# neross666/xRayTracer

Measured on AMD Instinct MI355X. Metric: Msamples/s (whole node) + wall-clock at 800×600×1024spp, 1/2/4/8 MI355X, higher is better.
Workload: dtype f32

## Files before the change

include/xrt.h:

```cpp
#ifndef XRT_H
#define XRT_H

#include <stddef.h>
#include <stdint.h>

#ifdef __cplusplus
extern "C" {
#endif

#define XRT_ABI_VERSION 14

enum {
    XRT_OK = 0,
    XRT_ERR_INVALID = -1,
    XRT_ERR_HIP = -2,
    XRT_ERR_STATE = -3,
    XRT_ERR_OOM = -4,
    XRT_ERR_UNSUPPORTED = -5,
    XRT_ERR_IO = -6
};

enum { XRT_OBJ_MESH = 0, XRT_OBJ_SPHERE = 1, XRT_OBJ_BOX = 2 };
enum { XRT_LIGHT_QUAD = 0, XRT_LIGHT_TRIANGLE = 1, XRT_LIGHT_SPHERE = 2, XRT_LIGHT_SPHERE_AREA = 3 };
enum { XRT_MAT_NONE = 0, XRT_MAT_LAMBERT = 1, XRT_MAT_METAL = 2, XRT_MAT_GLASS = 3 };

typedef struct {
    int32_t kind;
    int32_t first;
    int32_t count;
    int32_t material;
    float albedo[3];
    int32_t light;
    int32_t medium;
} xrt_object;

typedef struct {
    int32_t kind;
    float v0[3];
    float v1[3];
    float v2[3];
    float center[3];
    float radius;
    float Le[3];
} xrt_light;

typedef struct {
    uint32_t n_objects;
    const xrt_object* objects;
    uint32_t n_tris;
    const float* tri_v;
    const float* tri_n;
    uint32_t n_spheres;
    const float* spheres;
    uint32_t n_boxes;
    const float* boxes;
    uint32_t n_lights;
    const xrt_light* lights;
} xrt_scene_desc;

enum { XRT_DLIGHT_POINT = 0, XRT_DLIGHT_DISTANT = 1 };
typedef struct {
    int32_t kind;
    float pos[3];
    float dir[3];
    float color[3];
    float intensity;
} xrt_delta_light;
#define XRT_MAX_DELTA_LIGHTS 8

enum {
    XRT_MEDIUM_HETEROGENEOUS = 0,
    XRT_MEDIUM_HOMOGENEOUS_MIS = 1,
    XRT_MEDIUM_HOMOGENEOUS_ACHROMATIC = 2,
    XRT_MEDIUM_HOMOGENEOUS_NOMIS = 3
};
typedef struct {
    uint32_t nx, ny, nz;
    const float* density;
    float origin[3];
    float voxel_size;
    float bbox_min[3];
    float bbox_max[3];
    float max_density;
    float g;
    float absorption[3];
    float scattering[3];
    float density_multiplier;
    int32_t kind;
} xrt_medium_desc;

enum {
    XRT_INTEGRATOR_GI = 0,
    XRT_INTEGRATOR_DIRECT = 1,
    XRT_INTEGRATOR_VPT = 2,
    XRT_INTEGRATOR_INDIRECT = 3,
    XRT_INTEGRATOR_NORMAL = 4,
    XRT_INTEGRATOR_VPT_NEE = 5,
    XRT_INTEGRATOR_WHITTED = 6
};
#define XRT_WHITTED_MAX_DEPTH 4
enum {
    XRT_FLAG_TIMING = 1u,
    XRT_FLAG_WAVEFRONT = 2u,
    XRT_FLAG_NO_MERGED = 4u,
    XRT_FLAG_NO_GROUP = 8u,
    XRT_FLAG_DEEP_SINGLE = 32u,
    XRT_FLAG_DEEP_QUAD = 64u,
    XRT_FLAG_NO_PIXEL = 128u,
    XRT_FLAG_NO_SPEC = 256u,
    XRT_FLAG_WHITTED_BVH = 512u,
    XRT_FLAG_NO_OVERLAP = 1024u,
    XRT_FLAG_INTERLEAVE = 2048u,
    XRT_FLAG_NO_INTERLEAVE = 4096u,
    XRT_FLAG_VAR_FUSED = 8192u,
    XRT_FLAG_ACCUMULATE = 16u
};

typedef struct {
    int32_t integrator;
    uint32_t max_depth;
    uint32_t width, height;
    uint32_t spp;
    uint32_t shard_index;
    uint32_t shard_count;
    uint32_t flags;
    uint32_t slots_per_wave;
    uint32_t visits_per_launch;
} xrt_render_params;

enum {
    XRT_K_SEED = 0, XRT_K_TRACE = 1, XRT_K_SHADE = 2, XRT_K_FINISH = 3, XRT_K_STEP = 4, XRT_K_REFILL = 5,
    XRT_K_DEEP = 6, XRT_K_COUNT = 7
};

enum {
    XRT_SCHED_WAVEFRONT = 0, XRT_SCHED_STEP = 1, XRT_SCHED_STEP_TRI = 2, XRT_SCHED_STEP_MERGED = 3,
    XRT_SCHED_STEP_BVH = 4, XRT_SCHED_PIXEL = 5,
    XRT_SCHED_WHITTED = 6,
    XRT_SCHED_WHITTED_BVH = 7,
    XRT_SCHED_AOV = 8
};

typedef struct {
    double wall_ms;
    double kernel_ms[XRT_K_COUNT];
    uint64_t launches[XRT_K_COUNT];
    uint64_t samples;
    uint64_t segments;
    uint64_t shadow_rays;
    uint64_t draws;
    uint64_t rejected;
    uint64_t iterations;
    uint64_t path_slots;
    uint64_t schedule;
    uint64_t stalled;
    uint32_t slots_per_wave;
    uint32_t group_lanes;
    uint32_t partitions;
    uint32_t visits_per_launch;
    uint64_t rng_twists;
    uint64_t layout_launches[5];
    uint64_t pix_windows;
    uint64_t pix_stride4;
    uint64_t pix_frustum;
    uint64_t pix_frustum_overflow;
    uint64_t pix_shadow_list;
    uint64_t pix_shadow_overflow;
    uint64_t pix_flushes;
    uint64_t spec_launches;
    uint64_t whit_rays;
    uint64_t whit_depth_cut;
    uint64_t whit_refract;
    uint64_t whit_tir;
} xrt_stats;

typedef struct xrt_ctx xrt_ctx;

int  xrt_abi_version(void);
int  xrt_create(int device, xrt_ctx** out);
int  xrt_create_multi(const int* devices, int n_devices, xrt_ctx** out);
int  xrt_device_count(const xrt_ctx* ctx);
void xrt_destroy(xrt_ctx* ctx);
const char* xrt_last_error(const xrt_ctx* ctx);

int  xrt_upload_scene(xrt_ctx* ctx, const xrt_scene_desc* scene);
int  xrt_set_camera(xrt_ctx* ctx, const float c2w[16], float scale, float aspect);
int  xrt_set_medium(xrt_ctx* ctx, const xrt_medium_desc* medium);
int  xrt_set_delta_lights(xrt_ctx* ctx, const xrt_delta_light* lights, uint32_t n);
#define XRT_BRICK 8
typedef struct {
    uint32_t nbx, nby, nbz;
    const int32_t* table;
    uint32_t n_bricks;
    const float* bricks;
} xrt_brick_grid;
int  xrt_set_medium_bricks(xrt_ctx* ctx, const xrt_medium_desc* medium, const xrt_brick_grid* grid);

int  xrt_render(xrt_ctx* ctx, const xrt_render_params* p, float* rgb_out, xrt_stats* st);
int  xrt_render_device(xrt_ctx* ctx, const xrt_render_params* p, float* d_rgb_out, xrt_stats* st);
int  xrt_render_device_after(xrt_ctx* ctx, const xrt_render_params* p, float* d_rgb_out, void* hip_stream,
                             xrt_stats* st);

int  xrt_render_var(xrt_ctx* ctx, const xrt_render_params* p, float* rgb_out, float* variance_out, xrt_stats* st);
int  xrt_render_var_device(xrt_ctx* ctx, const xrt_render_params* p, float* d_rgb_out, float* d_variance_out,
                           void* hip_stream, xrt_stats* st);

typedef struct { float* albedo; float* normal; float* depth; float* alpha; int32_t* object; } xrt_aov_buffers;
int  xrt_render_aov(xrt_ctx* ctx, const xrt_render_params* p, const xrt_aov_buffers* host_out, xrt_stats* st);
int  xrt_render_aov_device(xrt_ctx* ctx, const xrt_render_params* p, const xrt_aov_buffers* device_out,
                           void* hip_stream, xrt_stats* st);

#define XRT_DENOISE_MAX_ITERATIONS 6
#define XRT_DENOISE_TILED_ITERATIONS 2
enum {
    XRT_DENOISE_TIMING = 1u,
    XRT_DENOISE_NO_TILE = 2u
};
typedef struct {
    uint32_t width, height, iterations;
    float sigma_color, sigma_normal, sigma_depth, sigma_albedo;
    uint32_t flags;
} xrt_denoise_params;
typedef struct {
    double wall_ms;
    double kernel_ms;
    uint32_t launches;
    uint32_t tiled_iterations, direct_iterations;
    uint32_t reserved;
} xrt_denoise_stats;
int  xrt_denoise(xrt_ctx* ctx, const xrt_denoise_params* p, const float* color, const xrt_aov_buffers* guides,
                 float* out, xrt_denoise_stats* st);
int  xrt_denoise_device(xrt_ctx* ctx, const xrt_denoise_params* p, const float* d_color,
                        const xrt_aov_buffers* d_guides, float* d_out, void* hip_stream, xrt_denoise_stats* st);

#define XRT_DENOISE_VAR_MAX_RADIUS 3
#define XRT_DENOISE_VAR_TILED_ITERATIONS 2
typedef struct {
    uint32_t width, height, iterations;
    float sigma_luminance, sigma_normal, sigma_depth, sigma_albedo;
    uint32_t variance_radius;
    uint32_t flags;
} xrt_denoise_var_params;
int  xrt_denoise_var(xrt_ctx* ctx, const xrt_denoise_var_params* p, const float* color, const float* variance,
                     const xrt_aov_buffers* guides, float* out, float* out_variance, xrt_denoise_stats* st);
int  xrt_denoise_var_device(xrt_ctx* ctx, const xrt_denoise_var_params* p, const float* d_color,
                            const float* d_variance, const xrt_aov_buffers* d_guides, float* d_out,
                            float* d_out_variance, void* hip_stream, xrt_denoise_stats* st);

typedef struct {
    int32_t hit;
    int32_t object;
    int32_t primitive;
    float t;
    float t1;
    float position[3], ng[3], ns[3], dpdu[3], dpdv[3];
    float barycentric[2];
} xrt_hit;
enum { XRT_QUERY_INTERSECT = 0, XRT_QUERY_OCCLUDED = 1 };
int  xrt_query(xrt_ctx* ctx, uint32_t n, const float* rays, const float* tmax, int32_t mode, xrt_hit* out);

int  xrt_tonemap(xrt_ctx* ctx, const float* d_rgb, uint32_t n_pixels, float gamma, uint8_t* rgb8_out);

typedef struct xrt_hscene xrt_hscene;
xrt_hscene* xrt_hscene_create(void);
void xrt_hscene_destroy(xrt_hscene* s);
const char* xrt_hscene_last_error(const xrt_hscene* s);
int xrt_hscene_load_obj(xrt_hscene* s, const char* path);
int xrt_hscene_add_mesh(xrt_hscene* s, const char* name, const float* tri_v, const float* tri_n,
                        uint32_t n_tris, const float albedo[3]);
int xrt_hscene_add_sphere_mesh(xrt_hscene* s, const char* name, const float center[3], float radius,
                               int n_theta, int n_phi, const float albedo[3]);
int xrt_hscene_add_sphere(xrt_hscene* s, const char* name, const float center[3], float radius,
                          const float albedo[3]);
int xrt_hscene_add_quad_light(xrt_hscene* s, const char* name, const float v0[3], const float v1[3],
                              const float v2[3], const float Le[3]);
int xrt_hscene_add_triangle_light(xrt_hscene* s, const char* name, const float v0[3],
                                  const float v1[3], const float v2[3], const float Le[3]);
int xrt_hscene_add_sphere_light(xrt_hscene* s, const char* name, const float center[3], float radius,
                                const float Le[3]);
int xrt_hscene_add_sphere_light_area(xrt_hscene* s, const char* name, const float center[3], float radius,
                                     const float Le[3]);
int xrt_hscene_add_medium_box(xrt_hscene* s, const char* name, const float pmin[3], const float pmax[3]);
int xrt_hscene_add_point_light(xrt_hscene* s, const char* name, const float l2w[16], const float color[3],
                               float intensity);
int xrt_hscene_add_distant_light(xrt_hscene* s, const char* name, const float l2w[16], const float color[3],
                                 float intensity);
int xrt_hscene_delta_lights(xrt_hscene* s, const xrt_delta_light** out, uint32_t* n);
int xrt_hscene_set_material(xrt_hscene* s, const char* object_name, int32_t material);
int xrt_hscene_flatten(xrt_hscene* s, xrt_scene_desc* out);
const char* xrt_hscene_object_name(const xrt_hscene* s, uint32_t i);

float xrt_pinhole_scale(float fov_deg);

int xrt_test_rng(xrt_ctx* ctx, const uint32_t* seeds, uint32_t n_seeds, uint32_t skip, uint32_t n,
                 float* out);
int xrt_test_trig(xrt_ctx* ctx, const float* x, uint32_t n, float* out);
int xrt_test_trig_draw_domain(xrt_ctx* ctx, uint32_t first_bits, uint32_t count, float* out_sin,
                              float* out_cos, float* out_r);
int xrt_test_logexp(xrt_ctx* ctx, const float* x, uint32_t n, float* out);
int xrt_test_powf(xrt_ctx* ctx, const float* x, uint32_t n, float y, float* out);
int xrt_test_fastdiv(xrt_ctx* ctx, uint32_t mode, float c, float rc, uint64_t* n_bad, uint32_t* first_bad16);
int xrt_test_whitted_math(xrt_ctx* ctx, const float* in, uint32_t n, float* out);
int xrt_test_camlist(xrt_ctx* ctx, const xrt_render_params* p, uint32_t* out);
int xrt_test_slot_map(xrt_ctx* ctx, const xrt_render_params* p, uint32_t* out);

#ifdef __cplusplus
}
#endif
#endif
```

xraytracer_amd/abi.py:

```python
from __future__ import annotations

import ctypes as C
import os

import numpy as np

HERE = os.path.dirname(os.path.abspath(__file__))
LIB_PATH = os.path.join(HERE, "libxrt_hip.so")
if os.environ.get("XRT_LIB"):
    _v = os.path.join(HERE, "variants", os.environ["XRT_LIB"])
    LIB_PATH = _v if os.path.exists(_v) else os.path.join(HERE, os.environ["XRT_LIB"])

XRT_ABI_VERSION = 14
XRT_OK = 0
XRT_OBJ_MESH, XRT_OBJ_SPHERE, XRT_OBJ_BOX = 0, 1, 2
XRT_LIGHT_QUAD, XRT_LIGHT_TRIANGLE, XRT_LIGHT_SPHERE, XRT_LIGHT_SPHERE_AREA = 0, 1, 2, 3
XRT_MAT_NONE, XRT_MAT_LAMBERT, XRT_MAT_METAL, XRT_MAT_GLASS = 0, 1, 2, 3
MATERIALS = {"none": XRT_MAT_NONE, "lambert": XRT_MAT_LAMBERT, "metal": XRT_MAT_METAL, "glass": XRT_MAT_GLASS}
XRT_DLIGHT_POINT, XRT_DLIGHT_DISTANT = 0, 1
XRT_MAX_DELTA_LIGHTS = 8
XRT_INTEGRATOR_GI, XRT_INTEGRATOR_DIRECT, XRT_INTEGRATOR_VPT = 0, 1, 2
XRT_INTEGRATOR_INDIRECT, XRT_INTEGRATOR_NORMAL, XRT_INTEGRATOR_VPT_NEE = 3, 4, 5
XRT_INTEGRATOR_WHITTED = 6
XRT_WHITTED_MAX_DEPTH = 4
XRT_ERR_INVALID, XRT_ERR_UNSUPPORTED = -1, -5
XRT_ERR_STATE = -3
XRT_MEDIUM_HETEROGENEOUS, XRT_MEDIUM_HOMOGENEOUS_MIS, XRT_MEDIUM_HOMOGENEOUS_ACHROMATIC, XRT_MEDIUM_HOMOGENEOUS_NOMIS = 0, 1, 2, 3
XRT_FLAG_TIMING, XRT_FLAG_WAVEFRONT, XRT_FLAG_NO_MERGED, XRT_FLAG_NO_GROUP, XRT_FLAG_ACCUMULATE = 1, 2, 4, 8, 16
XRT_FLAG_DEEP_SINGLE, XRT_FLAG_DEEP_QUAD, XRT_FLAG_NO_PIXEL = 32, 64, 128
XRT_FLAG_NO_SPEC = 256
XRT_FLAG_WHITTED_BVH = 512
XRT_FLAG_NO_OVERLAP = 1024
XRT_FLAG_INTERLEAVE, XRT_FLAG_NO_INTERLEAVE = 2048, 4096
XRT_FLAG_VAR_FUSED = 8192
XRT_SCHED_WAVEFRONT, XRT_SCHED_STEP, XRT_SCHED_STEP_TRI, XRT_SCHED_STEP_MERGED, XRT_SCHED_STEP_BVH = 0, 1, 2, 3, 4
XRT_SCHED_PIXEL, XRT_SCHED_WHITTED, XRT_SCHED_WHITTED_BVH = 5, 6, 7
XRT_SCHED_AOV = 8
AOV_PLANES = ("albedo", "normal", "depth", "alpha", "object")
XRT_DENOISE_MAX_ITERATIONS = 6
XRT_DENOISE_TILED_ITERATIONS = 2
XRT_DENOISE_TIMING, XRT_DENOISE_NO_TILE = 1, 2
XRT_DENOISE_VAR_MAX_RADIUS = 3
XRT_DENOISE_VAR_TILED_ITERATIONS = 2
DENOISE_PLANES = ("albedo", "normal", "depth", "object")
SCHEDULE_NAMES = ("wavefront", "step", "step_tri", "step_merged", "step_bvh", "pixel", "whitted", "whitted_bvh",
                  "aov")
XRT_K_SEED, XRT_K_TRACE, XRT_K_SHADE, XRT_K_FINISH, XRT_K_STEP, XRT_K_REFILL, XRT_K_DEEP, XRT_K_COUNT = \
    0, 1, 2, 3, 4, 5, 6, 7
LAYOUTS = (64, 32, 16, 8, 4)
KERNEL_NAMES = ("seed", "trace", "shade", "finish", "step", "refill", "trace_deep4")

INTEGRATORS = {"gi": XRT_INTEGRATOR_GI, "direct": XRT_INTEGRATOR_DIRECT, "vpt": XRT_INTEGRATOR_VPT,
               "indirect": XRT_INTEGRATOR_INDIRECT, "normal": XRT_INTEGRATOR_NORMAL, "vpt_nee": XRT_INTEGRATOR_VPT_NEE,
               "whitted": XRT_INTEGRATOR_WHITTED}

f32p = C.POINTER(C.c_float)
u32p = C.POINTER(C.c_uint32)


class XrtObject(C.Structure):
    _fields_ = [("kind", C.c_int32), ("first", C.c_int32), ("count", C.c_int32),
                ("material", C.c_int32), ("albedo", C.c_float * 3), ("light", C.c_int32),
                ("medium", C.c_int32)]


class XrtLight(C.Structure):
    _fields_ = [("kind", C.c_int32), ("v0", C.c_float * 3), ("v1", C.c_float * 3),
                ("v2", C.c_float * 3), ("center", C.c_float * 3), ("radius", C.c_float),
                ("Le", C.c_float * 3)]


class XrtDeltaLight(C.Structure):
    _fields_ = [("kind", C.c_int32), ("pos", C.c_float * 3), ("dir", C.c_float * 3), ("color", C.c_float * 3),
                ("intensity", C.c_float)]


class XrtSceneDesc(C.Structure):
    _fields_ = [("n_objects", C.c_uint32), ("objects", C.POINTER(XrtObject)),
                ("n_tris", C.c_uint32), ("tri_v", f32p), ("tri_n", f32p),
                ("n_spheres", C.c_uint32), ("spheres", f32p),
                ("n_boxes", C.c_uint32), ("boxes", f32p),
                ("n_lights", C.c_uint32), ("lights", C.POINTER(XrtLight))]


class XrtMediumDesc(C.Structure):
    _fields_ = [("nx", C.c_uint32), ("ny", C.c_uint32), ("nz", C.c_uint32), ("density", f32p),
                ("origin", C.c_float * 3), ("voxel_size", C.c_float),
                ("bbox_min", C.c_float * 3), ("bbox_max", C.c_float * 3),
                ("max_density", C.c_float), ("g", C.c_float),
                ("absorption", C.c_float * 3), ("scattering", C.c_float * 3),
                ("density_multiplier", C.c_float), ("kind", C.c_int32)]


class XrtBrickGrid(C.Structure):
    _fields_ = [("nbx", C.c_uint32), ("nby", C.c_uint32), ("nbz", C.c_uint32), ("table", C.POINTER(C.c_int32)),
                ("n_bricks", C.c_uint32), ("bricks", f32p)]


XRT_BRICK = 8


class XrtRenderParams(C.Structure):
    _fields_ = [("integrator", C.c_int32), ("max_depth", C.c_uint32), ("width", C.c_uint32),
                ("height", C.c_uint32), ("spp", C.c_uint32), ("shard_index", C.c_uint32),
                ("shard_count", C.c_uint32), ("flags", C.c_uint32), ("slots_per_wave", C.c_uint32),
                ("visits_per_launch", C.c_uint32)]


class XrtStats(C.Structure):
    _fields_ = [("wall_ms", C.c_double), ("kernel_ms", C.c_double * XRT_K_COUNT),
                ("launches", C.c_uint64 * XRT_K_COUNT), ("samples", C.c_uint64),
                ("segments", C.c_uint64), ("shadow_rays", C.c_uint64), ("draws", C.c_uint64),
                ("rejected", C.c_uint64), ("iterations", C.c_uint64), ("path_slots", C.c_uint64),
                ("schedule", C.c_uint64), ("stalled", C.c_uint64), ("slots_per_wave", C.c_uint32),
                ("group_lanes", C.c_uint32), ("partitions", C.c_uint32), ("visits_per_launch", C.c_uint32),
                ("rng_twists", C.c_uint64), ("layout_launches", C.c_uint64 * 5),
                ("pix_windows", C.c_uint64), ("pix_stride4", C.c_uint64), ("pix_frustum", C.c_uint64),
                ("pix_frustum_overflow", C.c_uint64), ("pix_shadow_list", C.c_uint64),
                ("pix_shadow_overflow", C.c_uint64), ("pix_flushes", C.c_uint64), ("spec_launches", C.c_uint64),
                ("whit_rays", C.c_uint64), ("whit_depth_cut", C.c_uint64), ("whit_refract", C.c_uint64),
                ("whit_tir", C.c_uint64)]

    def as_dict(self):
        d = {k: getattr(self, k) for k, _ in self._fields_ if k not in ("kernel_ms", "launches", "layout_launches")}
        d["layout_launches"] = dict(zip(LAYOUTS, (int(x) for x in self.layout_launches)))
        d["kernel_ms"] = {n: self.kernel_ms[i] for i, n in enumerate(KERNEL_NAMES)}
        d["launches"] = {n: int(self.launches[i]) for i, n in enumerate(KERNEL_NAMES)}
        return d


class XrtAovBuffers(C.Structure):
    _fields_ = [("albedo", C.c_void_p), ("normal", C.c_void_p), ("depth", C.c_void_p), ("alpha", C.c_void_p),
                ("object", C.c_void_p)]


class XrtDenoiseParams(C.Structure):
    _fields_ = [("width", C.c_uint32), ("height", C.c_uint32), ("iterations", C.c_uint32),
                ("sigma_color", C.c_float), ("sigma_normal", C.c_float), ("sigma_depth", C.c_float),
                ("sigma_albedo", C.c_float), ("flags", C.c_uint32)]


class XrtDenoiseVarParams(C.Structure):
    _fields_ = [("width", C.c_uint32), ("height", C.c_uint32), ("iterations", C.c_uint32),
                ("sigma_luminance", C.c_float), ("sigma_normal", C.c_float), ("sigma_depth", C.c_float),
                ("sigma_albedo", C.c_float), ("variance_radius", C.c_uint32), ("flags", C.c_uint32)]


class XrtDenoiseStats(C.Structure):
    _fields_ = [("wall_ms", C.c_double), ("kernel_ms", C.c_double), ("launches", C.c_uint32),
                ("tiled_iterations", C.c_uint32), ("direct_iterations", C.c_uint32), ("reserved", C.c_uint32)]


class XrtHit(C.Structure):
    _fields_ = [("hit", C.c_int32), ("object", C.c_int32), ("primitive", C.c_int32), ("t", C.c_float),
                ("t1", C.c_float), ("position", C.c_float * 3), ("ng", C.c_float * 3), ("ns", C.c_float * 3),
                ("dpdu", C.c_float * 3), ("dpdv", C.c_float * 3), ("barycentric", C.c_float * 2)]


XRT_QUERY_INTERSECT, XRT_QUERY_OCCLUDED = 0, 1


SIGNATURES = {
    "xrt_abi_version": (C.c_int, []),
    "xrt_create": (C.c_int, [C.c_int, C.POINTER(C.c_void_p)]),
    "xrt_create_multi": (C.c_int, [C.POINTER(C.c_int), C.c_int, C.POINTER(C.c_void_p)]),
    "xrt_device_count": (C.c_int, [C.c_void_p]),
    "xrt_destroy": (None, [C.c_void_p]),
    "xrt_last_error": (C.c_char_p, [C.c_void_p]),
    "xrt_upload_scene": (C.c_int, [C.c_void_p, C.POINTER(XrtSceneDesc)]),
    "xrt_set_camera": (C.c_int, [C.c_void_p, f32p, C.c_float, C.c_float]),
    "xrt_set_medium": (C.c_int, [C.c_void_p, C.POINTER(XrtMediumDesc)]),
    "xrt_set_delta_lights": (C.c_int, [C.c_void_p, C.POINTER(XrtDeltaLight), C.c_uint32]),
    "xrt_set_medium_bricks": (C.c_int, [C.c_void_p, C.POINTER(XrtMediumDesc), C.POINTER(XrtBrickGrid)]),
    "xrt_render": (C.c_int, [C.c_void_p, C.POINTER(XrtRenderParams), f32p, C.POINTER(XrtStats)]),
    "xrt_render_device": (C.c_int, [C.c_void_p, C.POINTER(XrtRenderParams), C.c_void_p, C.POINTER(XrtStats)]),
    "xrt_render_device_after": (C.c_int, [C.c_void_p, C.POINTER(XrtRenderParams), C.c_void_p, C.c_void_p,
                                          C.POINTER(XrtStats)]),
    "xrt_render_var": (C.c_int, [C.c_void_p, C.POINTER(XrtRenderParams), f32p, f32p, C.POINTER(XrtStats)]),
    "xrt_render_var_device": (C.c_int, [C.c_void_p, C.POINTER(XrtRenderParams), C.c_void_p, C.c_void_p, C.c_void_p,
                                        C.POINTER(XrtStats)]),
    "xrt_render_aov": (C.c_int, [C.c_void_p, C.POINTER(XrtRenderParams), C.POINTER(XrtAovBuffers), C.POINTER(XrtStats)]),
    "xrt_render_aov_device": (C.c_int, [C.c_void_p, C.POINTER(XrtRenderParams), C.POINTER(XrtAovBuffers), C.c_void_p,
                                        C.POINTER(XrtStats)]),
    "xrt_denoise": (C.c_int, [C.c_void_p, C.POINTER(XrtDenoiseParams), C.c_void_p, C.POINTER(XrtAovBuffers), C.c_void_p,
                              C.POINTER(XrtDenoiseStats)]),
    "xrt_denoise_device": (C.c_int, [C.c_void_p, C.POINTER(XrtDenoiseParams), C.c_void_p, C.POINTER(XrtAovBuffers),
                                     C.c_void_p, C.c_void_p, C.POINTER(XrtDenoiseStats)]),
    "xrt_denoise_var": (C.c_int, [C.c_void_p, C.POINTER(XrtDenoiseVarParams), C.c_void_p, C.c_void_p,
                                  C.POINTER(XrtAovBuffers), C.c_void_p, C.c_void_p, C.POINTER(XrtDenoiseStats)]),
    "xrt_denoise_var_device": (C.c_int, [C.c_void_p, C.POINTER(XrtDenoiseVarParams), C.c_void_p, C.c_void_p,
                                         C.POINTER(XrtAovBuffers), C.c_void_p, C.c_void_p, C.c_void_p,
                                         C.POINTER(XrtDenoiseStats)]),
    "xrt_hscene_create": (C.c_void_p, []),
    "xrt_hscene_destroy": (None, [C.c_void_p]),
    "xrt_hscene_last_error": (C.c_char_p, [C.c_void_p]),
    "xrt_hscene_load_obj": (C.c_int, [C.c_void_p, C.c_char_p]),
    "xrt_hscene_add_mesh": (C.c_int, [C.c_void_p, C.c_char_p, f32p, f32p, C.c_uint32, f32p]),
    "xrt_hscene_add_sphere_mesh": (C.c_int, [C.c_void_p, C.c_char_p, f32p, C.c_float, C.c_int, C.c_int, f32p]),
    "xrt_hscene_add_sphere": (C.c_int, [C.c_void_p, C.c_char_p, f32p, C.c_float, f32p]),
    "xrt_hscene_add_quad_light": (C.c_int, [C.c_void_p, C.c_char_p, f32p, f32p, f32p, f32p]),
    "xrt_hscene_add_triangle_light": (C.c_int, [C.c_void_p, C.c_char_p, f32p, f32p, f32p, f32p]),
    "xrt_hscene_add_sphere_light": (C.c_int, [C.c_void_p, C.c_char_p, f32p, C.c_float, f32p]),
    "xrt_hscene_add_sphere_light_area": (C.c_int, [C.c_void_p, C.c_char_p, f32p, C.c_float, f32p]),
    "xrt_hscene_add_medium_box": (C.c_int, [C.c_void_p, C.c_char_p, f32p, f32p]),
    "xrt_hscene_add_point_light": (C.c_int, [C.c_void_p, C.c_char_p, f32p, f32p, C.c_float]),
    "xrt_hscene_add_distant_light": (C.c_int, [C.c_void_p, C.c_char_p, f32p, f32p, C.c_float]),
    "xrt_hscene_delta_lights": (C.c_int, [C.c_void_p, C.POINTER(C.POINTER(XrtDeltaLight)), u32p]),
    "xrt_hscene_set_material": (C.c_int, [C.c_void_p, C.c_char_p, C.c_int32]),
    "xrt_hscene_flatten": (C.c_int, [C.c_void_p, C.POINTER(XrtSceneDesc)]),
    "xrt_hscene_object_name": (C.c_char_p, [C.c_void_p, C.c_uint32]),
    "xrt_pinhole_scale": (C.c_float, [C.c_float]),
    "xrt_test_rng": (C.c_int, [C.c_void_p, u32p, C.c_uint32, C.c_uint32, C.c_uint32, f32p]),
    "xrt_test_trig": (C.c_int, [C.c_void_p, f32p, C.c_uint32, f32p]),
    "xrt_test_trig_draw_domain": (C.c_int, [C.c_void_p, C.c_uint32, C.c_uint32, f32p, f32p, f32p]),
    "xrt_test_logexp": (C.c_int, [C.c_void_p, f32p, C.c_uint32, f32p]),
    "xrt_test_powf": (C.c_int, [C.c_void_p, f32p, C.c_uint32, C.c_float, f32p]),
    "xrt_query": (C.c_int, [C.c_void_p, C.c_uint32, f32p, f32p, C.c_int32, C.POINTER(XrtHit)]),
    "xrt_tonemap": (C.c_int, [C.c_void_p, C.c_void_p, C.c_uint32, C.c_float, C.POINTER(C.c_uint8)]),
    "xrt_test_whitted_math": (C.c_int, [C.c_void_p, f32p, C.c_uint32, f32p]),
    "xrt_test_fastdiv": (C.c_int, [C.c_void_p, C.c_uint32, C.c_float, C.c_float, C.POINTER(C.c_uint64), u32p]),
    "xrt_test_camlist": (C.c_int, [C.c_void_p, C.POINTER(XrtRenderParams), u32p]),
    "xrt_test_slot_map": (C.c_int, [C.c_void_p, C.POINTER(XrtRenderParams), u32p]),
}

_lib = None


def lib():
    global _lib
    if _lib is None:
        if not os.path.exists(LIB_PATH):
            raise ImportError(f"{LIB_PATH} is missing: run __graft_entry__.build() "
                              "(the HIP path has no CPU fallback)")
        try:
            import torch
        except Exception as e:
            if not isinstance(e, ImportError):
                import warnings
                warnings.warn(f"torch failed to import ({e!r}); loading libxrt_hip without it")
        l = C.CDLL(LIB_PATH)
        for name, (res, args) in SIGNATURES.items():
            fn = getattr(l, name)
            fn.restype = res
            fn.argtypes = args
        _lib = l
    return _lib


def fptr(a: np.ndarray):
    assert a.dtype == np.float32 and a.flags.c_contiguous
    return a.ctypes.data_as(f32p)


def u32ptr(a: np.ndarray):
    assert a.dtype == np.uint32 and a.flags.c_contiguous
    return a.ctypes.data_as(u32p)


def f3(v):
    return np.ascontiguousarray(np.asarray(v, dtype=np.float32).reshape(3))


class XrtError(RuntimeError):
    pass
```

xraytracer_amd/csrc/api_context.cpp:

```cpp
#include "ctx.h"

namespace xrt {

int set_err(xrt_ctx* c, int code, const std::string& msg) {
    if (c) c->err = msg;
    return code;
}

int hip_err(xrt_ctx* c, hipError_t e, const char* what) {
    return set_err(c, XRT_ERR_HIP, std::string(what) + ": " + hipGetErrorString(e));
}

void free_buf(DevBuf& b) {
    if (b.p) (void)hipFree(b.p);
    b.p = nullptr;
    b.bytes = 0;
}

int ensure(xrt_ctx* c, DevBuf& b, size_t bytes) {
    if (b.bytes >= bytes && b.p) return XRT_OK;
    free_buf(b);
    if (bytes == 0) return XRT_OK;
    hipError_t e = hipMalloc(&b.p, bytes);
    if (e != hipSuccess) {
        b.p = nullptr;
        return set_err(c, XRT_ERR_OOM, std::string("hipMalloc(") + std::to_string(bytes) + "): " + hipGetErrorString(e));
    }
    b.bytes = bytes;
    return XRT_OK;
}

int upload(xrt_ctx* c, DevBuf& b, const void* src, size_t bytes) {
    int rc = ensure(c, b, std::max<size_t>(bytes, 16));
    if (rc) return rc;
    if (bytes) HIPCHK(c, hipMemcpy(b.p, src, bytes, hipMemcpyHostToDevice));
    return XRT_OK;
}

int order_after(xrt_ctx* c, int wait, hipStream_t wait_stream, bool host_blocks) {
    HIPCHK(c, hipSetDevice(c->device));
    if (wait == 1) {
        HIPCHK(c, hipDeviceSynchronize());
    } else if (wait == 2) {
        HIPCHK(c, hipEventRecord(c->wait_ev, wait_stream));
        if (host_blocks)
            HIPCHK(c, hipEventSynchronize(c->wait_ev));
        else
            HIPCHK(c, hipStreamWaitEvent(c->stream, c->wait_ev, 0));
    }
    return XRT_OK;
}

}

using namespace xrt;

extern "C" {

int xrt_abi_version(void) { return XRT_ABI_VERSION; }

int xrt_create(int device, xrt_ctx** out) {
    if (!out) return XRT_ERR_INVALID;
    *out = nullptr;
    int n = 0;
    if (hipGetDeviceCount(&n) != hipSuccess || n == 0) return XRT_ERR_HIP;
    if (device < 0 || device >= n) return XRT_ERR_INVALID;
    xrt_ctx* c = new xrt_ctx();
    c->device = device;
    if (hipSetDevice(device) != hipSuccess || hipStreamCreateWithFlags(&c->stream, hipStreamNonBlocking) != hipSuccess ||
        hipHostMalloc((void**)&c->h_poll, 8 * kMaxStepGroups * kMaxParts * sizeof(uint32_t), hipHostMallocDefault) !=
            hipSuccess ||
        hipEventCreateWithFlags(&c->wait_ev, hipEventDisableTiming) != hipSuccess) {
        xrt_destroy(c);
        return XRT_ERR_HIP;
    }
    for (auto& slot : c->poll_ev)
        for (hipEvent_t& e : slot)
            if (hipEventCreateWithFlags(&e, hipEventDisableTiming) != hipSuccess) {
                xrt_destroy(c);
                return XRT_ERR_HIP;
            }
    int lds = 0;
    if (hipDeviceGetAttribute(&lds, hipDeviceAttributeMaxSharedMemoryPerBlock, device) != hipSuccess || lds <= 0) {
        xrt_destroy(c);
        return XRT_ERR_HIP;
    }
    c->base.lds_max = (uint32_t)lds;
    *out = c;
    return XRT_OK;
}

void xrt_destroy(xrt_ctx* c) {
    if (!c) return;
    for (xrt_ctx* s : c->subs) xrt_destroy(s);
    c->subs.clear();
    (void)hipSetDevice(c->device);
    if (c->stream) (void)hipStreamSynchronize(c->stream);
    for (hipStream_t s : c->group_stream)
        if (s) (void)hipStreamSynchronize(s), (void)hipStreamDestroy(s);
    if (c->fork_ev) (void)hipEventDestroy(c->fork_ev);
    for (hipEvent_t e : c->join_ev)
        if (e) (void)hipEventDestroy(e);
    DevBuf* all[] = {&c->tri, &c->tri_ng, &c->tri_nrm, &c->sph, &c->sph_obj, &c->box, &c->objs, &c->lights,
                     &c->segs, &c->density, &c->obj_box, &c->obj_plane, &c->bvh_node, &c->bvh_tri, &c->snode, &c->ssph, &c->sbk, &c->sblk, &c->ray_o, &c->ray_d, &c->thr, &c->rad, &c->thr_prev, &c->hit,
                     &c->hit2, &c->hit3, &c->sh_o, &c->sh_d, &c->sh_c, &c->med, &c->med2, &c->nee, &c->state,
                     &c->sample_k, &c->depth, &c->occ, &c->rng_c, &c->rng_g, &c->ring, &c->c_seg, &c->c_shadow,
                     &c->c_rej, &c->c_stall, &c->lists, &c->counts, &c->stats, &c->fb, &c->scratch, &c->kparams};
    for (DevBuf* b : all) free_buf(*b);
    free_buf(c->stri), free_buf(c->sbox), free_buf(c->splane), free_buf(c->bvh4), free_buf(c->deep);
    free_buf(c->q_rays), free_buf(c->q_tmax), free_buf(c->q_out);
    free_buf(c->brick_table), free_buf(c->brick_data), free_buf(c->corners), free_buf(c->camlist);
    free_buf(c->dlights), free_buf(c->obj_albedo), free_buf(c->aov), free_buf(c->denoise);
    free_buf(c->mom), free_buf(c->var);
    for (hipEvent_t e : c->events) (void)hipEventDestroy(e);
    for (auto& slot : c->poll_ev)
        for (hipEvent_t e : slot)
            if (e) (void)hipEventDestroy(e);
    if (c->wait_ev) (void)hipEventDestroy(c->wait_ev);
    if (c->h_poll) (void)hipHostFree(c->h_poll);
    if (c->stream) (void)hipStreamDestroy(c->stream);
    delete c;
}

const char* xrt_last_error(const xrt_ctx* c) { return c ? c->err.c_str() : "no context (xrt_create failed: no HIP device?)"; }

}
```

xraytracer_amd/csrc/api_render.cpp:

```cpp
#include <sched.h>

#include <chrono>
#include <cmath>
#include <cstdio>
#include <cstdlib>
#include <cstring>
#include <mutex>
#include <unordered_map>

#include "ctx.h"

namespace xrt {

int setup_deep(xrt_ctx* c, KParams& P) {
    P.deep = nullptr, P.deep_count = nullptr, P.deep_cap = 0;
    if (!P.two_level) return XRT_OK;
    P.deep_cap = P.part_cap * (1u + (uint32_t)std::max(1, P.n_lights));
    const size_t words = (size_t)P.n_part * P.deep_cap + 3 * kMaxParts;
    const int rc = ensure(c, c->deep, words * 4);
    if (rc) return rc;
    P.deep = as<uint32_t>(c->deep);
    P.deep_count = P.deep + (size_t)P.n_part * P.deep_cap;
    return XRT_OK;
}
// ... 23 lines not shown
        for (uint32_t m = (uint32_t)t; m < (1u << 23) && ok; m += (uint32_t)nthreads) {
            const uint32_t xb = 0x3f800000u | m;
            float x;
            std::memcpy(&x, &xb, 4);
            const float q = x * rc;
            ok = std::fma(std::fma(-d, q, x), rc, q) == x / d;
        }
        part[t] = ok;
    });
    bool ok = true;
    for (char p : part) ok &= p != 0;
    cache[key] = ok;
    return ok;
}

int check_render(xrt_ctx* c, const xrt_render_params* p) {
    if (!c || !p) return XRT_ERR_INVALID;
    if (!c->has_scene || !c->has_camera) return set_err(c, XRT_ERR_STATE, "upload a scene and set a camera first");
    if (p->width == 0 || p->height == 0 || p->shard_count == 0 || p->shard_index >= p->shard_count)
        return set_err(c, XRT_ERR_INVALID, "bad image size or shard");
    if (p->integrator < XRT_INTEGRATOR_GI || p->integrator > XRT_INTEGRATOR_WHITTED)
        return set_err(c, XRT_ERR_INVALID, "unknown integrator");
    if (p->integrator != XRT_INTEGRATOR_WHITTED && c->has_mirror)
        return set_err(c, XRT_ERR_UNSUPPORTED,
                       "the scene holds a metal or glass object: only WhittedIntegrator knows those materials");
    if (p->integrator == XRT_INTEGRATOR_WHITTED && c->has_glass && p->max_depth > XRT_WHITTED_MAX_DEPTH)
        return set_err(c, XRT_ERR_UNSUPPORTED, "WhittedIntegrator over a scene with glass: max_depth above " +
                                                   std::to_string(XRT_WHITTED_MAX_DEPTH) + " (XRT_WHITTED_MAX_DEPTH)");
    const bool volumetric = p->integrator == XRT_INTEGRATOR_VPT || p->integrator == XRT_INTEGRATOR_VPT_NEE;
    if (volumetric && !c->has_medium)
        return set_err(c, XRT_ERR_STATE, "VolumePathTracing needs xrt_set_medium first");
    if (p->integrator == XRT_INTEGRATOR_VPT_NEE && c->base.n_lights == 0)
        return set_err(c, XRT_ERR_STATE, "VolumePathTracingNEE needs an area light");
    if (p->slots_per_wave != 0 && p->slots_per_wave != 4 && p->slots_per_wave != 8 && p->slots_per_wave != 16 &&
        p->slots_per_wave != 32 && p->slots_per_wave != 64)
        return set_err(c, XRT_ERR_INVALID, "slots_per_wave must be 0, 4, 8, 16, 32 or 64");
    if (p->visits_per_launch > 128) return set_err(c, XRT_ERR_INVALID, "visits_per_launch must be 0..128");
    return XRT_OK;
}

int check_render_var(xrt_ctx* c, const xrt_render_params* p) {
    if (p->spp < 2) return set_err(c, XRT_ERR_INVALID, "xrt_render_var: spp must be at least 2 (one sample has no variance)");
    if (p->flags & XRT_FLAG_ACCUMULATE)
        return set_err(c, XRT_ERR_UNSUPPORTED,
                       "xrt_render_var: XRT_FLAG_ACCUMULATE (the moments of the earlier calls' samples are unknown)");
    return XRT_OK;
}

int render_empty_shard(xrt_ctx* c, const xrt_render_params* p, float* d_out, float* h_out, float* d_var, xrt_stats* st,
                       std::chrono::steady_clock::time_point t_start) {
    const size_t npix = (size_t)p->width * p->height;
    int rc;
    if (!d_out && (rc = ensure(c, c->fb, npix * 3 * sizeof(float)))) return rc;
    float* fb0 = d_out ? d_out : as<float>(c->fb);
    if (p->flags & XRT_FLAG_ACCUMULATE) return XRT_OK;
    HIPCHK(c, hipMemsetAsync(fb0, 0, npix * 3 * sizeof(float), c->stream));
    if (d_var) HIPCHK(c, hipMemsetAsync(d_var, 0, npix * sizeof(float), c->stream));
    HIPCHK(c, hipStreamSynchronize(c->stream));
    if (h_out) HIPCHK(c, hipMemcpy(h_out, fb0, npix * 3 * sizeof(float), hipMemcpyDeviceToHost));
    if (st) {
        std::memset(st, 0, sizeof(*st));
        st->wall_ms = std::chrono::duration<double, std::milli>(std::chrono::steady_clock::now() - t_start).count();
    }
    return XRT_OK;
}

void bind_slots(xrt_ctx* c, KParams& P) {
    P.ray_o = as<f4>(c->ray_o), P.ray_d = as<f4>(c->ray_d), P.thr = as<f4>(c->thr), P.rad = as<f4>(c->rad);
    P.thr_prev = as<f4>(c->thr_prev), P.hit = as<f4>(c->hit), P.hit2 = as<f4>(c->hit2), P.hit3 = as<f4>(c->hit3);
    P.sh_o = as<f4>(c->sh_o), P.sh_d = as<f4>(c->sh_d), P.sh_c = as<f4>(c->sh_c);
    P.med = as<f4>(c->med), P.med2 = as<f4>(c->med2), P.nee = as<f4>(c->nee);
    P.state = as<uint32_t>(c->state), P.sample_k = as<uint32_t>(c->sample_k), P.depth = as<uint32_t>(c->depth);
    P.occ = as<uint32_t>(c->occ), P.rng_c = as<uint32_t>(c->rng_c), P.rng_g = as<uint32_t>(c->rng_g);
    P.ring = as<uint32_t>(c->ring);
    P.c_seg = as<uint32_t>(c->c_seg), P.c_shadow = as<uint32_t>(c->c_shadow), P.c_rej = as<uint32_t>(c->c_rej);
    P.c_stall = as<uint32_t>(c->c_stall);
    P.stats = as<unsigned long long>(c->stats);
}

}

int grow_slots(xrt_ctx* c, size_t n) {
    int rc;
    if (n > c->cap_slots) {
        const size_t L = kMaxLights;
        if ((rc = ensure(c, c->ray_o, n * 16)) || (rc = ensure(c, c->ray_d, n * 16)) || (rc = ensure(c, c->thr, n * 16)) ||
            (rc = ensure(c, c->rad, n * 16)) || (rc = ensure(c, c->thr_prev, n * 16)) || (rc = ensure(c, c->hit, n * 16)) ||
            (rc = ensure(c, c->hit2, n * 16)) || (rc = ensure(c, c->hit3, n * 16)) ||
            (rc = ensure(c, c->sh_o, L * n * 16)) || (rc = ensure(c, c->sh_d, L * n * 16)) ||
            (rc = ensure(c, c->sh_c, L * n * 16)) || (rc = ensure(c, c->med, n * 16)) || (rc = ensure(c, c->med2, n * 16)) ||
            (rc = ensure(c, c->nee, 4 * n * 16)) ||
            (rc = ensure(c, c->state, n * 4)) || (rc = ensure(c, c->sample_k, n * 4)) || (rc = ensure(c, c->depth, n * 4)) ||
            (rc = ensure(c, c->occ, n * 4)) || (rc = ensure(c, c->rng_c, n * 4)) || (rc = ensure(c, c->rng_g, n * 4)) ||
            (rc = ensure(c, c->ring, n * kRing * 4)) || (rc = ensure(c, c->c_seg, n * 4)) ||
            (rc = ensure(c, c->c_shadow, n * 4)) || (rc = ensure(c, c->c_rej, n * 4)) || (rc = ensure(c, c->c_stall, n * 4)) ||
            (rc = ensure(c, c->lists, 3 * (n + kMaxParts) * 4)))
            return rc;
        c->cap_slots = n;
    }
    if ((rc = ensure(c, c->counts, 5 * kMaxParts * 4)) || (rc = ensure(c, c->stats, 512))) return rc;
    return ensure(c, c->kparams, sizeof(KParams));
}

KParams render_params(xrt_ctx* c, const xrt_render_params* p, size_t n, float* fb) {
    KParams P = c->base;
    P.integrator = p->integrator;
    P.max_depth = p->max_depth, P.width = p->width, P.height = p->height, P.spp = p->spp;
    P.fw = (float)p->width, P.fh = (float)p->height, P.rw = 1.0f / P.fw, P.rh = 1.0f / P.fh;
    P.raspect = 1.0f / P.aspect;
    P.cdiv = (cdiv_exact(c, P.fw) ? 1u : 0u) | (cdiv_exact(c, P.fh) ? 2u : 0u) | (cdiv_exact(c, P.aspect) ? 4u : 0u);
    P.shard_index = p->shard_index, P.shard_count = p->shard_count, P.n_slots = (uint32_t)n;
    P.spw_req = p->slots_per_wave, P.rflags = p->flags;
    const char* dq = exp_env("XRT_DEEP_QUAD");
    P.deep_quad = dq ? std::atoi(dq) : (p->flags & XRT_FLAG_DEEP_SINGLE) ? 0 : 1;
    bind_slots(c, P);
    P.fb = fb;
    P.camlist = nullptr;
    P.slot_mul = 0;
    return P;
}

void LaunchTimer::read_out() {
    if (!timing) return;
    const bool trace = exp_env("XRT_TRACE_LAUNCHES") != nullptr;
    size_t step_idx = 0;
    for (size_t q = 0; q < kids.size(); ++q) {
        float ms = 0.0f;
        if (hipEventElapsedTime(&ms, c->events[2 * q], c->events[2 * q + 1]) == hipSuccess) S.kernel_ms[kids[q]] += ms;
        if (trace) {
            float gap = 0.0f;
            if (q) (void)hipEventElapsedTime(&gap, c->events[2 * q - 1], c->events[2 * q]);
            std::fprintf(stderr, "[xrt] launch %zu kernel %d %.3f ms (gap %.3f)%s", q, kids[q], ms, gap,
                         kids[q] == XRT_K_STEP && q < step_live.size() + 2 ? "" : "\n");
            if (kids[q] == XRT_K_STEP) {
                const size_t si = step_idx++;
                std::fprintf(stderr, " live %llu\n", si < step_live.size() ? (unsigned long long)step_live[si] : 0ull);
            }
        }
    }
}

namespace {

struct RenderPlan {
    int schedule;
    bool volumetric;
    bool pixel, fused, merged, two_level, step_tri, spec, camlist, elide, whitted, whitted_bvh;
    uint32_t n_part, part_cap;
    uint32_t groups;
    uint32_t slot_mul;
    uint32_t step_visits, spec_visits, rng_keep;
    uint64_t poll_every, ahead;
    uint64_t cap_iters;
    float2* mom;
};

static_assert(XRT_STEP_GROUPS >= 1 && XRT_STEP_GROUPS <= (int)kMaxStepGroups, "XRT_STEP_GROUPS: 1..3");

RenderPlan plan_render(const KParams& P, const xrt_render_params* p, float2* mom) {
    RenderPlan R{};
    R.mom = mom;
    const size_t n = P.n_slots;
    R.volumetric = p->integrator == XRT_INTEGRATOR_VPT || p->integrator == XRT_INTEGRATOR_VPT_NEE;
    R.two_level = !(p->flags & (XRT_FLAG_WAVEFRONT | XRT_FLAG_NO_MERGED)) && use_step_bvh(P);
    R.pixel = !R.two_level && !(p->flags & (XRT_FLAG_WAVEFRONT | XRT_FLAG_NO_PIXEL)) && use_pixel(P);
    R.fused = R.two_level || (!(p->flags & XRT_FLAG_WAVEFRONT) && step_lds_bytes(P) != 0);
    R.merged = R.two_level || (R.fused && !(p->flags & XRT_FLAG_NO_MERGED) && use_step_merged(P));
    R.step_tri = R.fused && !R.merged && use_step_tri(P);
    R.spec = R.merged && !R.two_level && !(p->flags & XRT_FLAG_NO_SPEC) && use_step_spec(P);
    R.camlist = R.spec && !exp_env("XRT_NO_CAMLIST");
    R.elide = XRT_CAM_ELIDE && !exp_env("XRT_NO_ELIDE") && R.merged && !R.two_level && !R.pixel &&
              p->integrator == XRT_INTEGRATOR_GI && p->max_depth >= 1 && p->spp >= 1 && P.n_tris <= 64;
    R.whitted = p->integrator == XRT_INTEGRATOR_WHITTED;
    R.whitted_bvh = R.whitted && (p->flags & XRT_FLAG_WHITTED_BVH) && !use_whitted(P) && use_whitted_bvh(P);
    if (R.whitted) R.pixel = true, R.two_level = R.merged = R.step_tri = R.spec = R.camlist = R.elide = false;
    R.schedule = R.whitted_bvh ? XRT_SCHED_WHITTED_BVH
                 : R.whitted   ? XRT_SCHED_WHITTED
                 : R.pixel     ? XRT_SCHED_PIXEL
                 : !R.fused    ? XRT_SCHED_WAVEFRONT
                 : R.two_level ? XRT_SCHED_STEP_BVH
                 : R.merged    ? XRT_SCHED_STEP_MERGED
                 : R.step_tri  ? XRT_SCHED_STEP_TRI
                               : XRT_SCHED_STEP;
    const size_t cap = R.merged ? 256 : kMaxParts, per = R.merged ? 2048 : kPartMinSlots;
    R.n_part = (uint32_t)std::min<size_t>(cap, std::max<size_t>(1, n / per));
    if (R.n_part >= 8) R.n_part &= ~7u;
    R.part_cap = (uint32_t)((n + R.n_part - 1) / R.n_part);
    R.groups = R.merged && !R.two_level && !R.pixel && !R.whitted && !(p->flags & XRT_FLAG_NO_OVERLAP)
                   ? step_groups_for(R.n_part, XRT_STEP_GROUPS)
                   : 1u;
    const bool can_interleave = R.merged && !R.pixel && !R.whitted && !(p->flags & XRT_FLAG_NO_INTERLEAVE);
    const bool auto_interleave = XRT_SLOT_INTERLEAVE && (R.two_level ? n >= kBvhLive64 && step_merged_spw(P, n) == 64
                                                                     : n >= kSlotInterleaveMin);
    const char* ei = exp_env("XRT_INTERLEAVE");
    const bool want_interleave = ei ? std::atoi(ei) != 0 : ((p->flags & XRT_FLAG_INTERLEAVE) || auto_interleave);
    R.slot_mul = can_interleave && want_interleave ? slot_multiplier((uint32_t)n) : 0u;
    const uint32_t draws = step_merged_draws(P);
    const char* ev = exp_env("XRT_VISITS");
    R.step_visits = ev                             ? (uint32_t)std::atoi(ev)
                    : p->visits_per_launch          ? p->visits_per_launch
                    : R.merged                      ? std::min<uint32_t>(kMergedVisits, (kMT - draws) / draws)
                    : (R.volumetric && kVptEvents) ? kVptEventVisits
                                                    : kStepVisits;
    R.spec_visits = !R.spec          ? 0
                    : XRT_SPEC_TWIST ? ((ev || p->visits_per_launch) ? R.step_visits : XRT_SPEC_VISITS)
                                     : std::min<uint32_t>(R.step_visits, (kMT - kSpecDraws) / kSpecDraws);
    R.rng_keep = R.spec && !XRT_SPEC_TWIST
                     ? std::max(R.step_visits * draws + draws, R.spec_visits * kSpecDraws + kSpecDraws)
                 : R.merged                     ? R.step_visits * draws + draws
                 : (R.volumetric && kVptEvents) ? R.step_visits * kVptEventDraws + kRngVisit
                                                : R.step_visits * kVisitDraws + kRngVisit;
    R.poll_every = R.merged ? 1 : R.fused ? 4 : 16;
    R.ahead = R.merged ? 3 : R.fused ? 16 : 64;
    R.cap_iters = R.volumetric ? (uint64_t)p->spp * 100000ull + 1000000ull
                               : (uint64_t)p->spp * (p->max_depth + 2) + 16;
    return R;
}

struct LivePoll {
    xrt_ctx* c;
    uint32_t n_part;
    uint64_t every, ahead;
    bool part_max;
    uint64_t live_hint;
    uint32_t live_part_max;
    bool done = false;
    struct Pending { uint64_t it; int slot; uint32_t groups; };
    std::vector<Pending> pending;
    int issued = 0;

    int after(uint64_t it, const uint32_t* live, uint32_t groups = 1) {
        if (it % every == every - 1) {
            const int ps = issued++ % 8;
            for (uint32_t g = 0; g < groups; ++g) {
                hipStream_t st = groups > 1 ? c->group_stream[g] : c->stream;
                HIPCHK(c, hipMemcpyAsync(c->h_poll + (ps * kMaxStepGroups + g) * kMaxParts, live, n_part * 4,
                                         hipMemcpyDeviceToHost, st));
                HIPCHK(c, hipEventRecord(c->poll_ev[ps][g], st));
            }
            pending.push_back({it, ps, groups});
        }
        while (!pending.empty()) {
            const Pending q = pending.front();
            const bool must_wait = it - q.it >= ahead;
            bool fired = true;
            for (uint32_t g = 0; g < q.groups && fired && !must_wait; ++g)
                fired = hipEventQuery(c->poll_ev[q.slot][g]) == hipSuccess;
            if (!fired) break;
            for (uint32_t g = 0; g < q.groups; ++g) HIPCHK(c, hipEventSynchronize(c->poll_ev[q.slot][g]));
            const uint32_t* h0 = c->h_poll + (size_t)q.slot * kMaxStepGroups * kMaxParts;
            uint64_t alive = 0;
            uint32_t pmax = 0;
            for (uint32_t k = 0; k < n_part; ++k) {
                const uint32_t v = h0[step_group_of(q.groups, k) * kMaxParts + k];
                alive += v, pmax = std::max(pmax, v);
            }
            if (alive == 0) done = true;
            if (alive < live_hint) {
                live_hint = alive;
                if (part_max) live_part_max = std::max(1u, pmax);
            }
            pending.erase(pending.begin());
            if (done) break;
        }
        return XRT_OK;
    }
};

int seed_paths(xrt_ctx* c, const KParams& P, const RenderPlan& R, const LiveLists& L, LaunchTimer& T) {
    HIPCHK(c, T.launch(XRT_K_SEED, [&] { return launch_seed(P, L.list[0], L.counts(0), L.counts(1), L.req(0), c->stream); }));
    if (R.pixel) {
        uint32_t* work = reinterpret_cast<uint32_t*>(P.stats + kStatsWork);
        const hipError_t e = T.launch(XRT_K_STEP, [&] {
            return R.whitted_bvh ? launch_whitted_bvh(P, work, c->stream, R.mom)
                   : R.whitted   ? launch_whitted(P, work, c->stream, R.mom)
                                 : launch_pixel(P, work, c->stream);
        });
        if (e != hipSuccess) return hip_err(c, e, R.whitted_bvh ? "k_whitted_bvh" : R.whitted ? "k_whitted" : "k_pixel");
    } else {
        HIPCHK(c, T.launch(XRT_K_REFILL, [&] {
            return R.merged ? launch_refill_merged(P, L.req(0), L.req(1), c->stream)
                            : launch_refill(P, L.req(0), L.req(1), c->stream);
        }));
        if (R.elide) HIPCHK(c, T.launch(XRT_K_SEED, [&] { return launch_camlist(P, true, c->stream); }));
    }
    HIPCHK(c, hipMemcpyAsync(c->kparams.p, &P, sizeof(KParams), hipMemcpyHostToDevice, c->stream));
    return XRT_OK;
}

class StepGroupStreams {
  public:
    StepGroupStreams(xrt_ctx* c, LaunchTimer& T, uint32_t groups) : c_(c), T_(T), groups_(groups) {}
    ~StepGroupStreams() { (void)join(); }
    bool forked() const { return forked_; }
    int fork() {
        if (forked_) return XRT_OK;
        for (uint32_t g = 0; g < groups_; ++g) {
            if (!c_->group_stream[g]) HIPCHK(c_, hipStreamCreateWithFlags(&c_->group_stream[g], hipStreamNonBlocking));
            if (!c_->join_ev[g]) HIPCHK(c_, hipEventCreateWithFlags(&c_->join_ev[g], hipEventDisableTiming));
        }
        if (!c_->fork_ev) HIPCHK(c_, hipEventCreateWithFlags(&c_->fork_ev, hipEventDisableTiming));
        T_.span_begin(XRT_K_STEP);
        HIPCHK(c_, hipEventRecord(c_->fork_ev, c_->stream));
        forked_ = true;
        for (uint32_t g = 0; g < groups_; ++g) HIPCHK(c_, hipStreamWaitEvent(c_->group_stream[g], c_->fork_ev, 0));
        return XRT_OK;
    }
    int join() {
        if (!forked_) return XRT_OK;
        forked_ = false;
        hipError_t first = hipSuccess;
        for (uint32_t g = 0; g < groups_; ++g) {
            hipError_t e = hipEventRecord(c_->join_ev[g], c_->group_stream[g]);
            if (e == hipSuccess) e = hipStreamWaitEvent(c_->stream, c_->join_ev[g], 0);
            if (first == hipSuccess) first = e;
        }
        T_.span_end();
        return first == hipSuccess ? XRT_OK : hip_err(c_, first, "joining the step group streams");
    }

  private:
    xrt_ctx* c_;
    LaunchTimer& T_;
    uint32_t groups_;
    bool forked_ = false;
};

int run_fused(xrt_ctx* c, const KParams& P, const RenderPlan& R, const LiveLists& L, LaunchTimer& T, LivePoll& poll,
              uint64_t& it) {
    const KParams* dP = as<KParams>(c->kparams);
    const uint32_t blocks = P.n_part * ((P.part_cap + 255) / 256);
    bool camlist_pending = R.camlist && !R.elide;
    StepGroupStreams GS(c, T, R.groups);
    for (it = 0; it < R.cap_iters && !poll.done; ++it) {
        const uint32_t *list = L.list[it & 1], *ci = L.counts(it % 3);
        uint32_t *out = L.list[~it & 1], *co = L.counts((it + 1) % 3), *cz = L.counts((it + 2) % 3);
        const uint32_t spw = R.merged ? step_merged_spw(P, poll.live_hint) : 0;
        const uint32_t groups = spw == 64 ? R.groups : 1u;
        if (groups == 1 || !GS.forked()) T.step_live.push_back(poll.live_hint);
        if (R.merged) T.S.layout_launches[spw == 64 ? 0 : spw == 32 ? 1 : spw == 16 ? 2 : spw == 8 ? 3 : 4] += groups;
        int rc;
        if (groups > 1) {
            if ((rc = GS.fork())) return rc;
            for (uint32_t g = 0; g < groups; ++g) {
                const hipError_t e =
                    R.mom ? launch_step_merged_mom(P, dP, c->step_objs, list, ci, out, co, cz, R.mom, R.step_visits,
                                                   poll.live_hint, poll.live_part_max, groups, g, c->group_stream[g])
                          : launch_step_merged(P, dP, c->step_objs, list, ci, out, co, cz, L.req(1), R.step_visits,
                                               poll.live_hint, poll.live_part_max, groups, g, c->group_stream[g]);
                if (e != hipSuccess) return hip_err(c, e, "k_step");
            }
            T.S.launches[XRT_K_STEP] += groups;
            if ((rc = poll.after(it, co, groups))) return rc;
            continue;
        }
        if ((rc = GS.join())) return rc;
        const bool spec_now = R.spec && P.camlist && (spw == 16 || spw == 8 || (XRT_SPEC_TAIL && spw == 4)) &&
                              step_merged_group(P, spw) * spw == 64;
        if (spec_now) T.S.spec_launches++;
        if (spec_now && camlist_pending) {
            camlist_pending = false;
            HIPCHK(c, T.launch(XRT_K_SEED, [&] { return launch_camlist(P, false, c->stream); }));
        }
        const hipError_t e = T.launch(XRT_K_STEP, [&] {
            if (spec_now)
                return launch_step_spec(P, dP, list, ci, out, co, cz, R.spec_visits, poll.live_part_max, spw, c->stream);
            if (R.merged && R.mom)
                return launch_step_merged_mom(P, dP, c->step_objs, list, ci, out, co, cz, R.mom, R.step_visits,
                                              poll.live_hint, poll.live_part_max, 1, 0, c->stream);
            if (R.merged)
                return launch_step_merged(P, dP, c->step_objs, list, ci, out, co, cz, L.req(1), R.step_visits,
                                          poll.live_hint, poll.live_part_max, 1, 0, c->stream);
            return launch_step(P, dP, list, ci, out, co, cz, L.req(1), R.step_visits, blocks, poll.live_hint, R.step_tri,
                               c->stream, R.mom);
        });
        if (e != hipSuccess) return hip_err(c, e, "k_step");
        if ((rc = poll.after(it, co))) return rc;
    }
    return GS.join();
}

int run_wavefront(xrt_ctx* c, const KParams& P, const RenderPlan& R, const LiveLists& L, LaunchTimer& T, LivePoll& poll,
                  uint64_t& it) {
    const uint32_t blocks = P.n_part * ((P.part_cap + 255) / 256);
    for (it = 0; it < R.cap_iters && !poll.done; ++it) {
        const int cur = (int)(it & 1), nxt = cur ^ 1;
        hipError_t e = T.launch(XRT_K_SHADE, [&] {
            return launch_shade(P, L.list[cur], L.counts(cur), L.list[nxt], L.counts(nxt), L.req(1), blocks, c->stream,
                                R.mom);
        });
        if (e != hipSuccess) return hip_err(c, e, "k_shade");
        e = T.launch(XRT_K_TRACE, [&] {
            return launch_trace(P, L.list[nxt], L.counts(nxt), L.counts(cur), blocks, c->stream, false);
        });
        if (e != hipSuccess) return hip_err(c, e, "k_trace");
        if (P.two_level && P.bvh_node && P.scene_kind == SCN_TRI) {
            e = T.launch(XRT_K_DEEP, [&] { return launch_trace_deep(P, c->stream); });
            if (e != hipSuccess) return hip_err(c, e, "k_trace_deep4");
        }
        const int rc = poll.after(it, L.counts(nxt));
        if (rc) return rc;
    }
    return XRT_OK;
}

int read_stats(xrt_ctx* c, const KParams& P, xrt_stats& S) {
    unsigned long long hs[48] = {0};
    HIPCHK(c, hipMemcpy(hs, P.stats, 48 * sizeof(unsigned long long), hipMemcpyDeviceToHost));
    if (XRT_PHASE_CLOCK)
        std::fprintf(stderr, "[xrt] spec phase cycles head %llu trace %llu candidates %llu end-test %llu shading %llu"
                     " moves %llu cursor+reload %llu launch %llu\n", hs[40], hs[41], hs[42], hs[43], hs[44], hs[45],
                     hs[46], hs[47]);
    if (hs[38])
        std::fprintf(stderr, "[xrt] deep rays %llu node steps %llu wave iterations %llu max wave iterations %llu"
                     " in-wave walks %llu\n", hs[38], hs[39], hs[37], hs[36], hs[35]);
    S.segments = hs[0], S.shadow_rays = hs[1], S.draws = hs[2], S.rejected = hs[3], S.stalled = hs[4];
    S.rng_twists = hs[7];
    S.pix_windows = hs[kStatsPix], S.pix_stride4 = hs[kStatsPix + 1], S.pix_frustum = hs[kStatsPix + 2];
    S.pix_frustum_overflow = hs[kStatsPix + 3], S.pix_shadow_list = hs[kStatsPix + 4];
    S.pix_shadow_overflow = hs[kStatsPix + 5], S.pix_flushes = hs[kStatsPix + 6];
    S.whit_rays = hs[kStatsWhit], S.whit_depth_cut = hs[kStatsWhit + 1], S.whit_refract = hs[kStatsWhit + 2];
    S.whit_tir = hs[kStatsWhit + 3];
    return XRT_OK;
}

}

int render_impl(xrt_ctx* c, const xrt_render_params* p, float* d_out, float* h_out, xrt_stats* st, int wait,
                hipStream_t wait_stream, float* d_var) {
    const auto t_start = std::chrono::steady_clock::now();
    int rc = check_render(c, p);
    if (rc) return rc;
    xrt_render_params forced;
    if (d_var) {
        if ((rc = check_render_var(c, p))) return rc;
        forced = *p;
        if ((p->flags & XRT_FLAG_VAR_FUSED) && !(p->flags & XRT_FLAG_WAVEFRONT) && p->integrator != XRT_INTEGRATOR_WHITTED) {
            forced.flags = (p->flags & ~XRT_FLAG_VAR_FUSED) | XRT_FLAG_NO_SPEC | XRT_FLAG_NO_PIXEL;
        } else {
            forced.flags = (p->flags & (XRT_FLAG_TIMING | XRT_FLAG_WHITTED_BVH)) | XRT_FLAG_WAVEFRONT;
            forced.slots_per_wave = forced.visits_per_launch = 0;
        }
        p = &forced;
    }
    if ((rc = order_after(c, wait, wait_stream, false))) return rc;
    const size_t n = (size_t)shard_rows(p->height, p->shard_index, p->shard_count) * p->width;
    const size_t npix = (size_t)p->width * p->height;
    if (n == 0) return render_empty_shard(c, p, d_out, h_out, d_var, st, t_start);

    if ((rc = grow_slots(c, n)) || (!d_out && (rc = ensure(c, c->fb, npix * 3 * sizeof(float)))) ||
        (d_var && (rc = ensure(c, c->mom, n * sizeof(float2)))))
        return rc;
    float* fb = d_out ? d_out : as<float>(c->fb);
    KParams P = render_params(c, p, n, fb);
    if (p->integrator == XRT_INTEGRATOR_WHITTED && !use_whitted(P)) {
        if (!(p->flags & XRT_FLAG_WHITTED_BVH))
            return set_err(c, XRT_ERR_UNSUPPORTED,
                           "WhittedIntegrator needs a scene that fits the LDS-resident scene carve (not a two-level scene)");
        if (!use_whitted_bvh(P))
            return set_err(c, XRT_ERR_UNSUPPORTED,
                           "WhittedIntegrator with XRT_FLAG_WHITTED_BVH: the scene neither fits the LDS-resident scene "
                           "carve nor has a triangle BVH (a large sphere-only or mixed scene)");
    }
    const RenderPlan R = plan_render(P, p, d_var ? as<float2>(c->mom) : nullptr);
    if (!R.pixel && R.rng_keep > kMT) return set_err(c, XRT_ERR_INVALID, "visits_per_launch too large for the RNG ring");
    P.n_part = R.n_part, P.part_cap = R.part_cap, P.rng_keep = R.rng_keep, P.slot_mul = R.slot_mul;
    const size_t lcap = (size_t)P.n_part * P.part_cap;
    const LiveLists L{{as<uint32_t>(c->lists), as<uint32_t>(c->lists) + lcap}, as<uint32_t>(c->counts)};
    P.req = as<uint32_t>(c->lists) + 2 * lcap;
    if ((rc = setup_deep(c, P))) return rc;
    if (R.camlist) {
        if ((rc = ensure(c, c->camlist, n * sizeof(uint4)))) return rc;
        P.camlist = as<uint4>(c->camlist);
    }
    xrt_stats S{};
    S.path_slots = n;
    S.samples = (uint64_t)n * p->spp;
    LaunchTimer T{c, S, (p->flags & XRT_FLAG_TIMING) != 0, {}, {}};

    if (!(p->flags & XRT_FLAG_ACCUMULATE))
        HIPCHK(c, hipMemsetAsync(fb, 0, npix * 3 * sizeof(float), c->stream));
    else if (h_out)
        HIPCHK(c, hipMemcpyAsync(fb, h_out, npix * 3 * sizeof(float), hipMemcpyHostToDevice, c->stream));
    if (d_var) HIPCHK(c, hipMemsetAsync(d_var, 0, npix * sizeof(float), c->stream));
    HIPCHK(c, hipMemsetAsync(P.stats, 0, 512, c->stream));
    if (R.mom && R.fused && !R.pixel) HIPCHK(c, hipMemsetAsync(R.mom, 0, n * sizeof(float2), c->stream));
    if ((rc = seed_paths(c, P, R, L, T))) return rc;

    LivePoll poll{c, P.n_part, R.poll_every, R.ahead, R.merged && !P.spw_req, n, P.part_cap};
    uint64_t it = 0;
    if (!R.pixel && (rc = R.fused ? run_fused(c, P, R, L, T, poll, it) : run_wavefront(c, P, R, L, T, poll, it)))
        return rc;
    HIPCHK(c, T.launch(XRT_K_FINISH, [&] {
        const hipError_t e = launch_finish(P, c->stream);
        return e != hipSuccess || !R.mom ? e : launch_finish_var(P, R.mom, d_var, c->stream);
    }));
    HIPCHK(c, hipStreamSynchronize(c->stream));
#if XRT_PHASE_CLOCK
    HIPCHK(c, wave_clock_dump(exp_env("XRT_WAVE_CLOCK_OUT"), c->stream));
#endif
    if (!R.pixel && !poll.done) {
        uint32_t left[kMaxParts] = {0};
        HIPCHK(c, hipMemcpy(left, L.counts(R.fused ? it % 3 : it & 1), P.n_part * 4, hipMemcpyDeviceToHost));
        for (uint32_t k = 0; k < P.n_part; ++k)
            if (left[k] != 0) return set_err(c, XRT_ERR_HIP, "iteration cap reached with live paths");
    }

    if ((rc = read_stats(c, P, S))) return rc;
    S.iterations = it;
    S.schedule = (uint64_t)R.schedule;
    S.partitions = P.n_part;
    if (R.fused && !R.pixel) S.visits_per_launch = R.step_visits;
    if (R.merged && !R.pixel) {
        S.slots_per_wave = step_merged_spw(P, n);
        S.group_lanes = step_merged_group(P, S.slots_per_wave);
    }
    T.read_out();
    if (h_out) HIPCHK(c, hipMemcpy(h_out, fb, npix * 3 * sizeof(float), hipMemcpyDeviceToHost));
    S.wall_ms = std::chrono::duration<double, std::milli>(std::chrono::steady_clock::now() - t_start).count();
    if (st) *st = S;
    return XRT_OK;
}

}

using namespace xrt;

extern "C" {

int xrt_render(xrt_ctx* c, const xrt_render_params* p, float* rgb_out, xrt_stats* st) {
    if (!rgb_out) return set_err(c, XRT_ERR_INVALID, "null output");
    if (c && !c->subs.empty()) return render_multi(c, p, nullptr, rgb_out, st, 0, nullptr);
    return render_impl(c, p, nullptr, rgb_out, st);
}

int xrt_render_device(xrt_ctx* c, const xrt_render_params* p, float* d_rgb_out, xrt_stats* st) {
    if (!d_rgb_out) return set_err(c, XRT_ERR_INVALID, "null output");
    if (c && !c->subs.empty()) return render_multi(c, p, d_rgb_out, nullptr, st, 1, nullptr);
    return render_impl(c, p, d_rgb_out, nullptr, st, 1);
}

int xrt_render_device_after(xrt_ctx* c, const xrt_render_params* p, float* d_rgb_out, void* hip_stream,
                            xrt_stats* st) {
    if (!d_rgb_out) return set_err(c, XRT_ERR_INVALID, "null output");
    if (c && !c->subs.empty()) return render_multi(c, p, d_rgb_out, nullptr, st, 2, (hipStream_t)hip_stream);
    return render_impl(c, p, d_rgb_out, nullptr, st, 2, (hipStream_t)hip_stream);
}

int xrt_test_slot_map(xrt_ctx* c, const xrt_render_params* p, uint32_t* out) {
    c = first_device(c);
    if (!c || !p || !out) return XRT_ERR_INVALID;
    int rc = check_render(c, p);
    if (rc) return rc;
    const size_t n = (size_t)shard_rows(p->height, p->shard_index, p->shard_count) * p->width;
    if (n == 0) return XRT_OK;
    HIPCHK(c, hipSetDevice(c->device));
    DevBuf d;
    if ((rc = ensure(c, d, n * sizeof(uint32_t)))) return rc;
    KParams P = render_params(c, p, n, nullptr);
    P.slot_mul = plan_render(P, p, nullptr).slot_mul;
    hipError_t e = launch_test_slot_map(P, as<uint32_t>(d), c->stream);
    if (e == hipSuccess) e = hipMemcpyAsync(out, d.p, n * sizeof(uint32_t), hipMemcpyDeviceToHost, c->stream);
    if (e == hipSuccess) e = hipStreamSynchronize(c->stream);
    free_buf(d);
    return e == hipSuccess ? XRT_OK : hip_err(c, e, "xrt_test_slot_map");
}

static int render_var(xrt_ctx* c, const xrt_render_params* p, float* d_out, float* h_out, float* d_var, float* h_var,
                      xrt_stats* st, int wait, hipStream_t wait_stream) {
    if (!c || !p || !(d_out || h_out) || !(d_var || h_var)) return set_err(c, XRT_ERR_INVALID, "xrt_render_var: null argument");
    xrt_ctx* c0 = first_device(c);
    const size_t npix = (size_t)p->width * p->height;
    int rc;
    if (!d_var) {
        HIPCHK(c, hipSetDevice(c0->device));
        if ((rc = ensure(c0, c0->var, npix * sizeof(float)))) return c0 == c ? rc : multi_fail(c, c0, rc, "variance plane");
        d_var = as<float>(c0->var);
    }
    rc = !c->subs.empty() ? render_multi(c, p, d_out, h_out, st, wait, wait_stream, d_var)
                          : render_impl(c, p, d_out, h_out, st, wait, wait_stream, d_var);
    if (rc) return rc;
    if (h_var) HIPCHK(c, hipMemcpy(h_var, d_var, npix * sizeof(float), hipMemcpyDeviceToHost));
    if (d_out) {
        if ((rc = ensure(c0, c0->fb, npix * 3 * sizeof(float)))) return c0 == c ? rc : multi_fail(c, c0, rc, "framebuffer");
        HIPCHK(c, hipMemcpy(c0->fb.p, d_out, npix * 3 * sizeof(float), hipMemcpyDeviceToDevice));
    }
    return XRT_OK;
}

int xrt_render_var(xrt_ctx* c, const xrt_render_params* p, float* rgb_out, float* variance_out, xrt_stats* st) {
    return render_var(c, p, nullptr, rgb_out, nullptr, variance_out, st, 0, nullptr);
}

int xrt_render_var_device(xrt_ctx* c, const xrt_render_params* p, float* d_rgb_out, float* d_variance_out,
                          void* hip_stream, xrt_stats* st) {
    return render_var(c, p, d_rgb_out, nullptr, d_variance_out, nullptr, st, 2, (hipStream_t)hip_stream);
}

}
```

xraytracer_amd/csrc/ctx.h:

```cpp
#pragma once
#include <hip/hip_runtime.h>

#include <algorithm>
#include <cstdint>
#include <functional>
#include <string>
#include <thread>
#include <vector>

#include "launch.h"
#include "wavefront.h"
#include "xrt.h"

#pragma GCC visibility push(hidden)

namespace xrt {
struct DevBuf {
    void* p = nullptr;
    size_t bytes = 0;
};
}

struct xrt_ctx {
    int device = 0;
    hipStream_t stream = nullptr;
    std::string err;
    xrt::DevBuf tri, tri_ng, tri_nrm, sph, sph_obj, box, objs, lights, segs, density, obj_box, obj_plane, bvh_node,
        bvh_tri, snode, ssph, sbk, sblk, stri, sbox, splane, bvh4;
    xrt::KParams base{};
    xrt::StepObjs step_objs{};
    xrt::StepObjs sstep{};
    bool has_scene = false, has_camera = false, has_medium = false;
    xrt::DevBuf dlights;
    bool has_mirror = false, has_glass = false;
    size_t cap_slots = 0;
    xrt::DevBuf ray_o, ray_d, thr, rad, thr_prev, hit, hit2, hit3, sh_o, sh_d, sh_c, med, med2, nee;
    xrt::DevBuf state, sample_k, depth, occ, rng_c, rng_g, ring, c_seg, c_shadow, c_rej, c_stall, lists, deep, camlist;
    xrt::DevBuf counts, stats, fb, scratch, kparams;
    xrt::DevBuf mom, var;
    uint32_t* h_poll = nullptr;
    std::vector<hipEvent_t> events;
    hipEvent_t poll_ev[8][xrt::kMaxStepGroups] = {};
    hipEvent_t wait_ev = nullptr;
    hipStream_t group_stream[xrt::kMaxStepGroups] = {};
    hipEvent_t fork_ev = nullptr, join_ev[xrt::kMaxStepGroups] = {};
    std::vector<xrt_ctx*> subs;
    std::vector<int> obj_tri_first;
    xrt::DevBuf q_rays, q_tmax, q_out;
    xrt::DevBuf brick_table, brick_data;
    xrt::DevBuf corners;
    xrt::DevBuf obj_albedo, aov;
    xrt::DevBuf denoise;
};

namespace xrt {

int set_err(xrt_ctx* c, int code, const std::string& msg);
int hip_err(xrt_ctx* c, hipError_t e, const char* what);

#define HIPCHK(ctx, expr)                                    \
    do {                                                     \
        hipError_t e_ = (expr);                              \
        if (e_ != hipSuccess) return hip_err(ctx, e_, #expr); \
    } while (0)

void free_buf(DevBuf& b);
int ensure(xrt_ctx* c, DevBuf& b, size_t bytes);
int upload(xrt_ctx* c, DevBuf& b, const void* src, size_t bytes);

template <typename T>
T* as(DevBuf& b) {
    return reinterpret_cast<T*>(b.p);
}

inline uint32_t shard_rows(uint32_t h, uint32_t idx, uint32_t n) { return idx < h ? (h - idx + n - 1) / n : 0; }

template <typename F>
void on_threads(int n, int own, F&& fn) {
    std::vector<std::thread> th;
    for (int t = own; t < n; ++t) th.emplace_back([&fn, t] { fn(t); });
    for (int t = 0; t < own; ++t) fn(t);
    for (auto& t : th) t.join();
}

int order_after(xrt_ctx* c, int wait, hipStream_t wait_stream, bool host_blocks);

struct LaunchTimer {
    xrt_ctx* c;
    xrt_stats& S;
    bool timing;
    std::vector<int> kids;
    std::vector<uint64_t> step_live;

    template <typename F>
    hipError_t launch(int kid, F&& fn) {
        const size_t e = 2 * kids.size();
        bool timed = timing;
        while (timed && c->events.size() < e + 2) {
            hipEvent_t ev;
            if ((timed = hipEventCreate(&ev) == hipSuccess)) c->events.push_back(ev);
        }
        if (timed) kids.push_back(kid);
        if (timed) (void)hipEventRecord(c->events[e], c->stream);
        const hipError_t err = fn();
        if (timed) (void)hipEventRecord(c->events[e + 1], c->stream);
        S.launches[kid]++;
        return err;
    }
    bool span_open = false;
    size_t span_stop = 0;
    void span_begin(int kid) {
        const size_t e = 2 * kids.size();
        bool timed = timing;
        while (timed && c->events.size() < e + 2) {
            hipEvent_t ev;
            if ((timed = hipEventCreate(&ev) == hipSuccess)) c->events.push_back(ev);
        }
        if (!timed) return;
        kids.push_back(kid);
        (void)hipEventRecord(c->events[e], c->stream);
        span_open = true, span_stop = e + 1;
    }
    void span_end() {
        if (span_open) (void)hipEventRecord(c->events[span_stop], c->stream);
        span_open = false;
    }
    void read_out();
};

struct LiveLists {
    uint32_t* list[2];
    uint32_t* cbase;
    uint32_t* counts(uint64_t j) const { return cbase + (size_t)j * kMaxParts; }
    uint32_t* req(int j) const { return counts(3 + j); }
};

int setup_deep(xrt_ctx* c, KParams& P);
int grow_slots(xrt_ctx* c, size_t n);
KParams render_params(xrt_ctx* c, const xrt_render_params* p, size_t n, float* fb);
int render_impl(xrt_ctx* c, const xrt_render_params* p, float* d_out, float* h_out, xrt_stats* st, int wait = 0,
                hipStream_t wait_stream = nullptr, float* d_var = nullptr);

inline xrt_ctx* first_device(xrt_ctx* c) { return c && !c->subs.empty() ? c->subs[0] : c; }

int multi_fail(xrt_ctx* m, xrt_ctx* s, int rc, const char* what);

template <typename F>
int for_each_device(xrt_ctx* c, const char* what, F&& one) {
    if (!c || c->subs.empty()) return one(c);
    for (xrt_ctx* d : c->subs) {
        const int rc = one(d);
        if (rc) return multi_fail(c, d, rc, what);
    }
    return XRT_OK;
}

int fan_out_rows(xrt_ctx* m, const xrt_render_params* p, const char* what,
                 const std::function<int(uint32_t, const xrt_render_params*)>& per_device);

struct RowPlane {
    std::vector<void*> dev;
    size_t pixel_bytes;
};
int gather_rows(xrt_ctx* m, const xrt_render_params* p, const std::vector<RowPlane>& planes);

xrt_stats sum_stats(const std::vector<xrt_stats>& S);

int render_multi(xrt_ctx* m, const xrt_render_params* p, float* d_out, float* h_io, xrt_stats* st, int wait,
                 hipStream_t wait_stream, float* d_var = nullptr);

}

#pragma GCC visibility pop
```

xraytracer_amd/csrc/launch.h:

```cpp
#pragma once
#include <hip/hip_runtime.h>

#include <algorithm>
#include <cstdlib>
#include <cstring>
#include <type_traits>

#include "slot_map.h"
#include "step_groups.h"
#include "wavefront.h"

namespace xrt {
#ifdef XRT_EXPERIMENTS
inline const char* exp_env(const char* name) { return std::getenv(name); }
#else
inline const char* exp_env(const char*) { return nullptr; }
#endif
template <int V, int... Rest, typename F>
auto with_const(int v, F&& fn) {
    if constexpr (sizeof...(Rest) == 0) {
        return fn(std::integral_constant<int, V>{});
    } else {
        if (v == V) return fn(std::integral_constant<int, V>{});
        return with_const<Rest...>(v, fn);
    }
}
template <typename F>
auto with_scene_kind(int kind, F&& fn) {
    return with_const<SCN_TRI, SCN_SPHERE, SCN_MIXED>(kind, fn);
}
template <typename F>
auto with_integrator(int integrator, F&& fn) {
    return with_const<XRT_INTEGRATOR_DIRECT, XRT_INTEGRATOR_VPT, XRT_INTEGRATOR_INDIRECT, XRT_INTEGRATOR_NORMAL,
                      XRT_INTEGRATOR_VPT_NEE, XRT_INTEGRATOR_GI>(integrator, fn);
}
template <typename K>
hipError_t persistent_blocks(K kernel, int block, size_t lds, uint32_t n_slots, uint32_t* blocks) {
    int dev = 0, ncu = 0, per_cu = 0;
    hipError_t e = hipGetDevice(&dev);
    if (e == hipSuccess) e = hipDeviceGetAttribute(&ncu, hipDeviceAttributeMultiprocessorCount, dev);
    if (e == hipSuccess) e = hipOccupancyMaxActiveBlocksPerMultiprocessor(&per_cu, kernel, block, lds);
    if (e != hipSuccess) return e;
    const uint64_t want = ((uint64_t)n_slots + block / 64 - 1) / (block / 64);
    *blocks = (uint32_t)std::max<uint64_t>(1, std::min<uint64_t>((uint64_t)std::max(1, per_cu) * ncu, want));
    return hipSuccess;
}

hipError_t launch_seed(const KParams& P, uint32_t* list, uint32_t* count, uint32_t* count_other,
                       uint32_t* req_count, hipStream_t st);
hipError_t launch_finish(const KParams& P, hipStream_t st);
hipError_t launch_finish_var(const KParams& P, const float2* mom, float* var, hipStream_t st);
hipError_t launch_test_slot_map(const KParams& P, uint32_t* out, hipStream_t st);
hipError_t launch_tonemap(const float* rgb, uint32_t n, float inv_gamma, uint8_t* out, hipStream_t st);

hipError_t launch_trace(const KParams& P, const uint32_t* list, const uint32_t* count, uint32_t* zero,
                        uint32_t blocks, hipStream_t st, bool zero_deep = true);
hipError_t launch_trace_deep(const KParams& P, hipStream_t st);
hipError_t launch_query(const KParams& P, const float* rays, const float* tmax, int mode, uint32_t* list,
                        uint32_t* count, uint32_t* zero, xrt_hit* out, hipStream_t st);

hipError_t launch_shade(const KParams& P, const uint32_t* list, const uint32_t* count, uint32_t* out,
                        uint32_t* out_count, uint32_t* req_count, uint32_t blocks, hipStream_t st, float2* mom = nullptr);

size_t step_lds_bytes(const KParams& P);
bool use_step_tri(const KParams& P);
hipError_t launch_step(const KParams& P, const KParams* dP, const uint32_t* list, const uint32_t* count, uint32_t* out,
                       uint32_t* out_count, uint32_t* zero, uint32_t* req_count, uint32_t visits, uint32_t blocks,
                       uint64_t live, bool tri, hipStream_t st, float2* mom = nullptr);

hipError_t launch_refill(const KParams& P, const uint32_t* count, uint32_t* zero_count, hipStream_t st);
hipError_t launch_refill_merged(const KParams& P, const uint32_t* count, uint32_t* zero_count, hipStream_t st);
hipError_t launch_trace_2a_coop(const KParams& P, const uint32_t* list, const uint32_t* count, uint32_t* zero,
                                uint32_t blocks, hipStream_t st);
bool use_step_merged(const KParams& P);
bool use_step_bvh(const KParams& P);
uint32_t step_merged_draws(const KParams& P);
uint32_t step_merged_spw(const KParams& P, uint64_t live);
uint32_t step_merged_group(const KParams& P, uint32_t spw);
size_t step_merged_lds_bytes(const KParams& P);
hipError_t launch_step_merged(const KParams& P, const KParams* dP, const StepObjs& SO, const uint32_t* list,
                              const uint32_t* count, uint32_t* out, uint32_t* out_count, uint32_t* zero,
                              uint32_t* req_count, uint32_t visits, uint64_t live, uint32_t live_part_max,
                              uint32_t groups, uint32_t group, hipStream_t st);
hipError_t launch_step_merged_mom(const KParams& P, const KParams* dP, const StepObjs& SO, const uint32_t* list,
                                  const uint32_t* count, uint32_t* out, uint32_t* out_count, uint32_t* zero,
                                  float2* mom, uint32_t visits, uint64_t live, uint32_t live_part_max,
                                  uint32_t groups, uint32_t group, hipStream_t st);
#if XRT_PHASE_CLOCK
hipError_t wave_clock_dump(const char* path, hipStream_t st);
#endif

bool use_step_spec(const KParams& P);
constexpr uint32_t kSpecDraws = 11;
hipError_t launch_camlist(const KParams& P, bool retire, hipStream_t st);
hipError_t launch_step_spec(const KParams& P, const KParams* dP, const uint32_t* list, const uint32_t* count,
                            uint32_t* out, uint32_t* out_count, uint32_t* zero, uint32_t visits, uint32_t part_live,
                            uint32_t spw, hipStream_t st);

bool use_pixel(const KParams& P);
size_t pix_lds_bytes(const KParams& P);
hipError_t launch_pixel(const KParams& P, uint32_t* work, hipStream_t st);

bool use_whitted(const KParams& P);
size_t whit_lds_bytes(const KParams& P);
hipError_t launch_whitted(const KParams& P, uint32_t* work, hipStream_t st, float2* mom = nullptr);
bool use_whitted_bvh(const KParams& P);
size_t whit_bvh_lds_bytes(const KParams& P);
hipError_t launch_whitted_bvh(const KParams& P, uint32_t* work, hipStream_t st, float2* mom = nullptr);
hipError_t launch_test_whitted(const float* in, uint32_t n, float* out, hipStream_t st);

struct AovOut {
    float *albedo, *normal, *depth, *alpha;
    int32_t* object;
    const float* obj_albedo;
};
int aov_kernel(const KParams& P);
hipError_t launch_aov(const KParams& P, const AovOut& A, uint32_t* work, hipStream_t st);

enum class DenoiseFilter { Plain, Var };
struct DenoiseK {
    float k0, kn, kz, ka;
};
struct DenoiseIter {
    const f4 *cin, *nrm, *alb;
    f4* cout;
    float *out3, *outv;
    uint32_t width, height;
    int step;
    DenoiseK K;
};
hipError_t launch_denoise_pack(const float* color, const float* variance, const float* albedo, const float* normal,
                               const float* depth, const int32_t* object, size_t npix, f4* col, f4* nrm, f4* alb,
                               hipStream_t st);
hipError_t launch_dnv_estimate(const f4* cin, const f4* nrm, f4* cout, uint32_t width, uint32_t height, int radius,
                               hipStream_t st);
bool denoise_has_tiled(int step);
hipError_t launch_denoise_iter(DenoiseFilter filter, const DenoiseIter& I, bool tiled, hipStream_t st);
constexpr int kDnTileW = 32, kDnTileH = 8;
constexpr int kDnBlock = kDnTileW * kDnTileH;

hipError_t launch_test_rng(const uint32_t* seeds, uint32_t n_seeds, uint32_t skip, uint32_t n, float* out,
                           uint32_t* rings, hipStream_t st);
hipError_t launch_test_trig(const float* x, uint32_t n, float* out, hipStream_t st);
hipError_t launch_test_trig_domain(uint32_t first, uint32_t count, float* s, float* c, float* r, hipStream_t st);
hipError_t launch_test_logexp(const float* x, uint32_t n, float* out, hipStream_t st);
hipError_t launch_test_powf(const float* x, uint32_t n, float y, float* out, hipStream_t st);
hipError_t launch_test_fastdiv(uint32_t mode, float c, float rc, uint32_t first, uint32_t count,
                               unsigned long long* nbad, uint32_t* bad, hipStream_t st);
}
```

xraytracer_amd/csrc/path_common.h:

```cpp
#pragma once
#include <hip/hip_runtime.h>

#include "device_math.h"
#include "slot_map.h"
#include "step_groups.h"
#include "wavefront.h"
#include "xrt.h"

namespace xrt {

constexpr int kBlock = 256;
constexpr int kTriTile = 512;
constexpr int kSphTile = 1024;

__device__ __forceinline__ SlotPixel slot_pixel(const KParams& P, uint32_t s) {
    return slot_pixel_at(s, P.slot_mul, P.n_slots, P.width, P.shard_index, P.shard_count);
}
__device__ __forceinline__ SlotPixel slot_pixel_rowmajor(const KParams& P, uint32_t s) {
    return slot_pixel_at(s, 0u, P.n_slots, P.width, P.shard_index, P.shard_count);
}

__device__ __forceinline__ uint32_t mt_temper(uint32_t y) {
    y ^= (y >> 11);
    y ^= (y << 7) & 0x9d2c5680u;
    y ^= (y << 15) & 0xefc60000u;
    y ^= (y >> 18);
    return y;
}
__device__ __forceinline__ float canonical(uint32_t y) {
    const float f = (float)y * 0x1p-32f;
    return f >= 1.0f ? 0x1.fffffep-1f : f;
}
__device__ __forceinline__ uint32_t mt_mix(uint32_t a, uint32_t b) {
    const uint32_t y = (a & 0x80000000u) | (b & 0x7fffffffu);
    return (y >> 1) ^ ((y & 1u) ? 0x9908b0dfu : 0u);
}

struct Rng {
    const uint32_t* ring;
    uint32_t c;
    uint32_t nb = 0;
    uint32_t b0 = 0, b1 = 0, b2 = 0, b3 = 0, b4 = 0, b5 = 0, b6 = 0, b7 = 0;
    __device__ __forceinline__ void load8() {
        typedef uint32_t u4u __attribute__((ext_vector_type(4), aligned(4)));
        using g4 = __attribute__((address_space(1))) const u4u;
        using g32 = __attribute__((address_space(1))) const uint32_t;
        const uint32_t i = c % kRing;
        if (i <= kRing - 8) {
            const u4u lo = *(g4*)(ring + i), hi = *(g4*)(ring + i + 4);
            b0 = lo.x, b1 = lo.y, b2 = lo.z, b3 = lo.w, b4 = hi.x, b5 = hi.y, b6 = hi.z, b7 = hi.w;
        } else {
            g32* r = (g32*)ring;
            b0 = r[i], b1 = r[(i + 1) % kRing], b2 = r[(i + 2) % kRing], b3 = r[(i + 3) % kRing];
            b4 = r[(i + 4) % kRing], b5 = r[(i + 5) % kRing], b6 = r[(i + 6) % kRing], b7 = r[(i + 7) % kRing];
        }
    }
    __device__ __forceinline__ void prefetch(uint32_t avail) {
        nb = avail < 8u ? avail : 8u;
        load8();
    }
    __device__ __forceinline__ float next() {
        if (!nb) {
            load8();
            nb = 8;
        }
        const uint32_t y = b0;
        b0 = b1, b1 = b2, b2 = b3, b3 = b4, b4 = b5, b5 = b6, b6 = b7;
        --nb;
        ++c;
        return canonical(mt_temper(y));
    }
};

__device__ __forceinline__ void wave_sync() {
    __builtin_amdgcn_fence(__ATOMIC_RELEASE, "wavefront");
    __builtin_amdgcn_wave_barrier();
    __builtin_amdgcn_fence(__ATOMIC_ACQUIRE, "wavefront");
}

__device__ inline void wave_twist(uint32_t* ring, uint32_t g, int lane) {
    const uint32_t h = g % kRing;
    const uint32_t* old = ring + (kMT - h);
    uint32_t* nw = ring + h;
    uint32_t a[4] = {0, 0, 0, 0}, b[4] = {0, 0, 0, 0};
#pragma unroll
    for (int j = 0; j < 4; ++j) {
        const uint32_t m = lane + 64 * j;
        if (m < 227) a[j] = old[m + 397] ^ mt_mix(old[m], old[m + 1]);
    }
    const uint32_t n0 = __shfl(a[0], 0);
#pragma unroll
    for (int j = 0; j < 4; ++j) {
        const uint32_t m = lane + 64 * j;
        if (m < 227) b[j] = a[j] ^ mt_mix(old[227 + m], old[228 + m]);
    }
#pragma unroll
    for (int j = 0; j < 3; ++j) {
        const uint32_t m = lane + 64 * j;
        if (m < 170) nw[454 + m] = b[j] ^ mt_mix(old[454 + m], m + 455 < kMT ? old[455 + m] : n0);
    }
#pragma unroll
    for (int j = 0; j < 4; ++j) {
        const uint32_t m = lane + 64 * j;
        if (m < 227) nw[m] = a[j], nw[227 + m] = b[j];
    }
}

__device__ inline void wave_refill(bool need, uint32_t slot, uint32_t& g, uint32_t* rings, int lane) {
    uint64_t m = __ballot(need);
    if (m == 0) return;
    while (m) {
        const int L = __ffsll((unsigned long long)m) - 1;
        m &= m - 1;
        const uint32_t sl = __shfl(slot, L);
        const uint32_t gl = __shfl(g, L);
        wave_twist(rings + (size_t)sl * kRing, gl, lane);
    }
    if (need) g += kMT;
    __builtin_amdgcn_fence(__ATOMIC_SEQ_CST, "workgroup");
}

typedef uint32_t u32x4 __attribute__((ext_vector_type(4)));
struct Staged { u32x4 v[3]; };

__device__ __forceinline__ Staged load_block(const uint32_t* ring, uint32_t g, int lane) {
    const u32x4* old = reinterpret_cast<const u32x4*>(ring + (kMT - g % kRing));
    Staged r;
#pragma unroll
    for (int k = 0; k < 3; ++k)
        r.v[k] = __builtin_nontemporal_load(old + min((uint32_t)lane + 64u * k, (uint32_t)(kMT / 4 - 1)));
    return r;
}

__device__ __forceinline__ void store_block(const Staged& r, int lane, uint32_t* lds) {
#pragma unroll
    for (int k = 0; k < 3; ++k) {
        const uint32_t q = (uint32_t)lane + 64u * k;
        if (q < kMT / 4) reinterpret_cast<u32x4*>(lds)[q] = r.v[k];
    }
    wave_sync();
}

__device__ __forceinline__ void twist_block(uint32_t* ring, uint32_t g, int lane, uint32_t* buf) {
    const uint32_t* old = buf;
    uint32_t x0[4], x1[4], x397[4], y0[4], y1[4], z0[3], z1[3];
#pragma unroll
    for (int j = 0; j < 4; ++j) {
        const uint32_t m = min((uint32_t)lane + 64u * j, 226u);
        x0[j] = old[m], x1[j] = old[m + 1], x397[j] = old[m + 397];
        y0[j] = old[227 + m], y1[j] = old[228 + m];
    }
#pragma unroll
    for (int j = 0; j < 3; ++j) {
        const uint32_t m = min((uint32_t)lane + 64u * j, 169u);
        z0[j] = old[454 + m], z1[j] = old[min(455 + m, kMT - 1)];
    }
    uint32_t a[4], b[4];
#pragma unroll
    for (int j = 0; j < 4; ++j) a[j] = x397[j] ^ mt_mix(x0[j], x1[j]);
    const uint32_t n0 = __builtin_amdgcn_readfirstlane(a[0]);
#pragma unroll
    for (int j = 0; j < 4; ++j) b[j] = a[j] ^ mt_mix(y0[j], y1[j]);
    wave_sync();
#pragma unroll
    for (int j = 0; j < 3; ++j) {
        const uint32_t m = (uint32_t)lane + 64u * j;
        if (m < 170u) buf[454 + m] = b[j] ^ mt_mix(z0[j], m + 455 < kMT ? z1[j] : n0);
    }
#pragma unroll
    for (int j = 0; j < 4; ++j) {
        const uint32_t m = (uint32_t)lane + 64u * j;
        if (m < 227u) buf[m] = a[j], buf[227 + m] = b[j];
    }
    wave_sync();
    u32x4* nw = reinterpret_cast<u32x4*>(ring + g % kRing);
#pragma unroll
    for (int k = 0; k < 3; ++k) {
        const uint32_t q = (uint32_t)lane + 64u * k;
        if (q < kMT / 4) nw[q] = reinterpret_cast<const u32x4*>(buf)[q];
    }
}

__device__ __forceinline__ void wave_refill(const KParams& P, bool want, uint32_t s, uint32_t g, int lane,
                                            uint32_t* buf) {
    uint64_t rq = __ballot(want);
    if (!rq) return;
    int l = __builtin_ctzll(rq);
    rq &= rq - 1ull;
    uint32_t sc = (uint32_t)__builtin_amdgcn_readlane((int)s, l), gc = (uint32_t)__builtin_amdgcn_readlane((int)g, l);
    Staged blk = load_block(P.ring + (size_t)sc * kRing, gc, lane);
    for (;;) {
        store_block(blk, lane, buf);
        const bool more = rq != 0ull;
        uint32_t sn = sc, gn = gc;
        if (more) {
            l = __builtin_ctzll(rq);
            rq &= rq - 1ull;
            sn = (uint32_t)__builtin_amdgcn_readlane((int)s, l), gn = (uint32_t)__builtin_amdgcn_readlane((int)g, l);
            blk = load_block(P.ring + (size_t)sn * kRing, gn, lane);
        }
        twist_block(P.ring + (size_t)sc * kRing, gc, lane, buf);
        if (lane == 0) P.rng_g[sc] = gc + kMT;
        if (!more) break;
        wave_sync();
        sc = sn, gc = gn;
    }
}

template <int CTRL>
__device__ __forceinline__ uint32_t dpp32(uint32_t x) {
    return (uint32_t)__builtin_amdgcn_mov_dpp((int)x, CTRL, 0xf, 0xf, false);
}
template <int G>
__device__ __forceinline__ uint32_t group_or32(uint32_t x) {
    if (G >= 2) x |= dpp32<0xB1>(x);
    if (G >= 4) x |= dpp32<0x4E>(x);
    if (G >= 8) x |= dpp32<0x141>(x);
    if (G >= 16) x |= dpp32<0x140>(x);
    return x;
}
template <int G>
__device__ __forceinline__ uint64_t group_or64(uint64_t x) {
    return ((uint64_t)group_or32<G>((uint32_t)(x >> 32)) << 32) | group_or32<G>((uint32_t)x);
}
template <int CTRL>
__device__ __forceinline__ uint64_t min64_dpp(uint64_t x) {
    const uint64_t y = ((uint64_t)dpp32<CTRL>((uint32_t)(x >> 32)) << 32) | dpp32<CTRL>((uint32_t)x);
    return y < x ? y : x;
}
template <int G>
__device__ __forceinline__ uint32_t group_min32(uint32_t x) {
    if (G >= 2) x = min(x, dpp32<0xB1>(x));
    if (G >= 4) x = min(x, dpp32<0x4E>(x));
    if (G >= 8) x = min(x, dpp32<0x141>(x));
    if (G >= 16) x = min(x, dpp32<0x140>(x));
    return x;
}
template <int G>
__device__ __forceinline__ uint64_t group_min64(uint64_t x) {
    if (G >= 2) x = min64_dpp<0xB1>(x);
    if (G >= 4) x = min64_dpp<0x4E>(x);
    if (G >= 8) x = min64_dpp<0x141>(x);
    if (G >= 16) x = min64_dpp<0x140>(x);
    return x;
}

__device__ __forceinline__ void wave_append(bool want, uint32_t v, uint32_t* list, uint32_t* cnt, int lane) {
    const uint64_t m = __ballot(want);
    if (!m) return;
    const int leader = __ffsll((unsigned long long)m) - 1;
    uint32_t base = 0;
    if (lane == leader) base = atomicAdd(cnt, (uint32_t)__popcll(m));
    base = __shfl(base, leader);
    if (want) list[base + __popcll(m & ((1ull << lane) - 1ull))] = v;
}

struct PartIter {
    uint32_t p, first, stride, n;
};
__device__ __forceinline__ PartIter part_iter(const KParams& P, const uint32_t* count, uint32_t per_block) {
    PartIter it;
    it.p = blockIdx.x % P.n_part;
    const uint32_t chunk = blockIdx.x / P.n_part, nchunks = gridDim.x / P.n_part;
    it.first = chunk * per_block;
    it.stride = nchunks * per_block;
    it.n = count[it.p];
    return it;
}
__device__ __forceinline__ void zero_parts(const KParams& P, uint32_t* c) {
    if (blockIdx.x == 0)
        for (uint32_t i = threadIdx.x; i < P.n_part; i += kBlock) c[i] = 0;
}
__device__ __forceinline__ PartIter part_iter(const uint32_t* count, uint32_t per_block, uint32_t grp) {
    const uint32_t np = grp >> 8;
    PartIter it;
    auto uni = [](uint32_t x) { return (uint32_t)__builtin_amdgcn_readfirstlane((int)x); };
    it.p = uni(step_group_part((grp >> 4) & 15u, grp & 15u, blockIdx.x % np));
    const uint32_t chunk = blockIdx.x / np, nchunks = gridDim.x / np;
    it.first = uni(chunk * per_block);
    it.stride = uni(nchunks * per_block);
    it.n = uni(count[it.p]);
    return it;
}
__device__ __forceinline__ void zero_parts(uint32_t* c, uint32_t grp) {
    if (blockIdx.x == 0)
        for (uint32_t i = threadIdx.x; i < (grp >> 8); i += kBlock) c[step_group_part((grp >> 4) & 15u, grp & 15u, i)] = 0;
}


__device__ __forceinline__ bool ray_tri(v3 o, v3 d, v3 v0, v3 e1, v3 e2, float& t, float& u, float& v) {
    const v3 pvec = cross(d, e2);
    const float det = dot(e1, pvec);
    if (__builtin_fabsf(det) < kEPSILON) return false;
    const float invDet = rcp_rn(det);
    const v3 tvec = o - v0;
    u = dot(tvec, pvec) * invDet;
    if (u < 0.0f || u > 1.0f) return false;
    const v3 qvec = cross(tvec, e1);
    v = dot(d, qvec) * invDet;
    if (v < 0.0f || u + v > 1.0f) return false;
    t = dot(e2, qvec) * invDet;
    return t > kEPSILON;
}

__device__ __forceinline__ bool sphere_hit(v3 o, v3 d, v3 c, float r, float& tnear) {
    const v3 L = o - c;
    const float a = dot(d, d);
    const float b = 2.0f * dot(d, L);
    const float cc = dot(L, L) - r * r;
    const float discr = b * b - 4.0f * a * cc;
    if (discr < 0.0f) return false;
    const double sq = __builtin_sqrt((double)discr);
    const float q = (float)(-0.5 * ((double)b + (b > 0.0f ? sq : -sq)));
    float t0 = q / a;
    float t1 = cc / q;
    if (discr == 0.0f) t0 = t1 = (float)(-0.5 * (double)b / (double)a);
    const bool sw = t0 > t1;
    const float lo = sw ? t1 : t0, hi = sw ? t0 : t1;
    tnear = lo < 0.0f ? hi : lo;
    return !(lo < 0.0f && hi < 0.0f);
}

__device__ __forceinline__ bool box_hit(v3 o, v3 d, v3 pmin, v3 pmax, float& t0, float& t1) {
    const v3 di = mk(1.0f / d.x, 1.0f / d.y, 1.0f / d.z);
    const v3 tt = di * (pmax - o), tb = di * (pmin - o);
    const v3 tmin = mk(smin(tt.x, tb.x), smin(tt.y, tb.y), smin(tt.z, tb.z));
    const v3 tmax = mk(smax(tt.x, tb.x), smax(tt.y, tb.y), smax(tt.z, tb.z));
    t0 = smax(smax(tmin.x, tmin.y), tmin.z);
    t1 = smin(smin(tmax.x, tmax.y), tmax.z);
    if (t0 > t1 || t1 <= 0.0f) return false;
    t0 = smax(t0, 0.0f);
    return true;
}


__device__ __forceinline__ bool box_overlap(v3 o, v3 inv, const DObjBox& B, float tlim) {
    const float tx0 = (B.bmin[0] - o.x) * inv.x, tx1 = (B.bmax[0] - o.x) * inv.x;
    const float ty0 = (B.bmin[1] - o.y) * inv.y, ty1 = (B.bmax[1] - o.y) * inv.y;
    const float tz0 = (B.bmin[2] - o.z) * inv.z, tz1 = (B.bmax[2] - o.z) * inv.z;
    const float tn = fmaxf(fmaxf(fminf(tx0, tx1), fminf(ty0, ty1)), fmaxf(fminf(tz0, tz1), 0.0f));
    const float tf = fminf(fminf(fmaxf(tx0, tx1), fmaxf(ty0, ty1)), fminf(fmaxf(tz0, tz1), tlim));
    return !(tn > tf);
}
__device__ __forceinline__ float bvh_enter(const f4& mn, const f4& mx, v3 o, v3 inv, float tlim) {
    const float tx0 = (mn.x - o.x) * inv.x, tx1 = (mx.x - o.x) * inv.x;
    const float ty0 = (mn.y - o.y) * inv.y, ty1 = (mx.y - o.y) * inv.y;
    const float tz0 = (mn.z - o.z) * inv.z, tz1 = (mx.z - o.z) * inv.z;
    const float tn = fmaxf(fmaxf(fminf(tx0, tx1), fminf(ty0, ty1)), fmaxf(fminf(tz0, tz1), 0.0f));
    const float tf = fminf(fminf(fmaxf(tx0, tx1), fmaxf(ty0, ty1)), fminf(fmaxf(tz0, tz1), tlim));
    return tn > tf ? __builtin_inff() : tn;
}

__device__ __forceinline__ bool root_overlap(const f4& n0, const f4& n1, const f4& n2, const f4& n3, v3 o, v3 inv,
                                             float tlim) {
    const bool l = __float_as_int(n1.w) >= 0 && bvh_enter(n0, n1, o, inv, tlim) != __builtin_inff();
    const bool r = __float_as_int(n3.w) >= 0 && bvh_enter(n2, n3, o, inv, tlim) != __builtin_inff();
    return l || r;
}

__device__ __forceinline__ float rcpc(float x) {
    return __builtin_amdgcn_fmed3f(__builtin_amdgcn_rcpf(x), -1e30f, 1e30f);
}
__device__ __forceinline__ v3 rcp3c(v3 d) { return mk(rcpc(d.x), rcpc(d.y), rcpc(d.z)); }
__device__ __forceinline__ v3 rcp3(v3 d) {
    return mk(__builtin_amdgcn_rcpf(d.x), __builtin_amdgcn_rcpf(d.y), __builtin_amdgcn_rcpf(d.z));
}


struct Surf {
    v3 pos, ng, ns, dpdu, dpdv;
    int obj;
};

__device__ __forceinline__ v3 tri_ns(const KParams& P, int i, float u, float v) {
    const float w = 1.0f - u - v;
    return xyz(P.tri_nrm[3 * i]) * w + xyz(P.tri_nrm[3 * i + 1]) * u + xyz(P.tri_nrm[3 * i + 2]) * v;
}

template <int SCN>
__device__ __forceinline__ int surface(const KParams& P, uint32_t s, v3 o, v3 d, f4 h, Surf& S, float& t1) {
    const int code = __float_as_int(h.w);
    S.pos = S.ng = S.ns = S.dpdu = S.dpdv = mk(0, 0, 0);
    t1 = kINF;
    if (code < 0) return -1;
    int surf = code, dp = (SCN == SCN_TRI) ? code : -1;
    float st = h.x, su = h.y, sv = h.z, du = h.y, dv = h.z;
    if (SCN == SCN_MIXED) {
        const f4 h2 = P.hit2[s], h3 = P.hit3[s];
        t1 = h2.x;
        surf = __float_as_int(h2.y), dp = __float_as_int(h2.z), st = h2.w;
        su = h3.x, sv = h3.y, du = h3.z, dv = h3.w;
    }
    if (surf >= 0) {
        const int kind = surf >> 28, idx = surf & 0x0fffffff;
        S.pos = ray_at(o, d, st);
        if (kind == SEG_TRI) {
            S.ng = xyz(P.tri_ng[idx]);
            S.ns = tri_ns(P, idx, su, sv);
        } else {
            S.ng = normalize(ray_at(o, d, st) - xyz(P.sph[idx]));
            S.ns = S.ng;
        }
    }
    if (dp >= 0) onb(tri_ns(P, dp & 0x0fffffff, du, dv), S.dpdu, S.dpdv);
    const int kind = code >> 28, idx = code & 0x0fffffff;
    if (kind == SEG_TRI) return __float_as_int(P.tri[3 * idx].w);
    if (kind == SEG_SPHERE) return P.sph_obj[idx] & 0x3fffffff;
    return __float_as_int(P.box[2 * idx].w);
}

__device__ __forceinline__ bool same3(v3 a) {
    return __float_as_uint(a.x) == __float_as_uint(a.y) && __float_as_uint(a.y) == __float_as_uint(a.z);
}
__device__ __forceinline__ v3 div3s(v3 a, float b) {
    if (same3(a)) {
        const float q = a.x / b;
        return mk(q, q, q);
    }
    return a / b;
}
__device__ __forceinline__ v3 div3v(v3 a, v3 b) {
    if (same3(a) && same3(b)) {
        const float q = a.x / b.x;
        return mk(q, q, q);
    }
    return a / b;
}

__device__ __forceinline__ v3 light_Le(const DLight& L, v3 ns, v3 wi) {
    return dot(wi, ns) < 0.0f ? mk(L.Le[0], L.Le[1], L.Le[2]) : mk(0, 0, 0);
}

__device__ __forceinline__ v3 ld3(const float* p) { return mk(p[0], p[1], p[2]); }

template <class RNG>
__device__ inline v3 light_sample(const DLight& L, v3 x, v3& wi, float& pdf, float& tmax, RNG& rng) {
    if (L.kind == 0) {
        const float ra = rng.next();
        const float rb = rng.next();
// ... 243 lines not shown
```

xraytracer_amd/csrc/step_tri.hip:

```cpp
#include <cstdio>
#include <type_traits>
#include <vector>

#include "bvh.h"
#include "launch.h"
#include "merged.h"
#include "path_common.h"
#include "trace_common.h"

namespace xrt {


template <int NL, bool ORIG = false>
__device__ __forceinline__ void merged_trace(const StepObjs& SO, const LScene& L, MergedWave<NL>& W, int lane,
                                             bool ext, v3 o, v3 d, uint32_t shm, const v3 (&so)[NL + 1],
                                             const v3 (&sd)[NL + 1], const float (&stm)[NL + 1],
                                             unsigned long long& best, uint32_t& occ
) {
    constexpr int R = 1 + NL;
    W.best[lane] = ~0ull;
    W.occ[lane] = 0u;
    v3 inv[R], oi[R];
    inv[0] = rcp3c(d);
    oi[0] = o * inv[0];
// ... 184 lines not shown
    }
}

template <int NL, typename SE>
__device__ __forceinline__ void deep_pass(const KParams& P, const f4* top, int ntop, SE* stk, MergedWave<NL>& W,
                                          int lane, const f4 (&root)[4], bool ext, v3 o, v3 d, uint32_t shm,
                                          const v3 (&so)[NL + 1], const v3 (&sd)[NL + 1], const float (&stm)[NL + 1],
                                          unsigned long long& best, uint32_t& occ) {
    constexpr int R = 1 + NL;
    bool need[R];
    const float bt = best == ~0ull ? kINF : __uint_as_float((uint32_t)(best >> 32));
    need[0] = ext && root_overlap(root[0], root[1], root[2], root[3], o, rcp3(d), bt);
#pragma unroll
    for (int l = 0; l < NL; ++l)
        need[1 + l] = ((shm & ~occ) >> l & 1u) && root_overlap(root[0], root[1], root[2], root[3], so[l], rcp3(sd[l]), stm[l]);
    wave_sync();
    uint32_t tot = 0;
#pragma unroll
    for (int q = 0; q < R; ++q) {
        const uint64_t m = __ballot(need[q]);
        if (need[q]) {
            const uint32_t at = tot + lanemask_rank(m);
            const v3 ro = q == 0 ? o : so[q - 1], rd = q == 0 ? d : sd[q - 1];
            W.ro[at] = make_float4(ro.x, ro.y, ro.z, q == 0 ? kINF : stm[q - 1]);
            W.rd[at] = make_float4(rd.x, rd.y, rd.z, __uint_as_float((uint32_t)(q * 64 + lane)));
        }
        tot += (uint32_t)__popcll(m);
    }
    if (tot == 0) return;
    wave_sync();
    wave_deep_walk<SE>(P, top, ntop, stk, W.ro, W.rd, W.best, W.occ, lane, tot);
    wave_sync();
    best = W.best[lane];
    occ = W.occ[lane];
}

constexpr uint32_t kStackWave = 16u * kQs * 2u;
struct BvhStepLayout {
    uint32_t tri, obj, light, top, wave, stack, total;
    int ntop;
};
__host__ __device__ inline BvhStepLayout bvh_step_layout(const KParams& P, uint32_t wave_bytes) {
    BvhStepLayout B;
    B.tri = 0;
    B.obj = 48u * (uint32_t)P.n_stri;
    B.light = B.obj + (uint32_t)sizeof(DObj) * (uint32_t)P.n_objs;
    B.top = (B.light + (uint32_t)sizeof(DLight) * (uint32_t)P.n_lights + 15u) & ~15u;
    const uint32_t rest = B.top + (kBlock / 64) * wave_bytes + (kBlock / 64) * kStackWave;
    const int fit = rest < kStepLds ? (int)((kStepLds - rest) / 128u) : 0;
    B.ntop = P.bvh4_nodes < XRT_BVH_TOP ? P.bvh4_nodes : XRT_BVH_TOP;
    B.ntop = B.ntop < fit ? B.ntop : fit;
    B.wave = B.top + 128u * (uint32_t)B.ntop;
    B.stack = B.wave + (kBlock / 64) * wave_bytes;
    B.total = B.stack + (kBlock / 64) * kStackWave;
    return B;
}

#ifndef XRT_STEP_MOM_UNIT
template <int NL>
__global__ __launch_bounds__(kBlock, XRT_2A_WAVES) void k_trace_2a_coop(KParams P, const StepObjs SO, const uint32_t* __restrict__ list,
                                                          const uint32_t* __restrict__ count, uint32_t* zero_count) {
    extern __shared__ __attribute__((aligned(16))) f4 lds_2c[];
    LScene L;
    L.tri = lds_2c;
    MergedWave<NL>* Wv = reinterpret_cast<MergedWave<NL>*>(lds_2c + 3 * P.n_stri);
    const int tid = threadIdx.x, lane = tid & 63;
    MergedWave<NL>& W = Wv[tid >> 6];
    lds_copy(const_cast<f4*>(L.tri), P.stri, 3 * P.n_stri, tid);
    zero_parts(P, zero_count);
    __syncthreads();
    const PartIter it = part_iter(P, count, kBlock);
    const PhaseA A = phase_a_begin(P, it);
    for (uint32_t base = it.first; base < it.n; base += it.stride) {
        const SlotRays<NL, NL + 1> R = load_slot_rays<NL, NL + 1>(P, list, it, base + tid);
        unsigned long long best;
        SlotHit H;
        merged_trace<NL>(SO, L, W, lane, R.want, R.o, R.d, R.smask, R.so, R.sd, R.stmax, best, H.occ);
        if (R.want && best != ~0ull) {
            const int hk = (int)(uint32_t)best;
            (void)ray_tri(R.o, R.d, xyz(L.tri[3 * hk]), xyz(L.tri[3 * hk + 1]), xyz(L.tri[3 * hk + 2]), H.t, H.u, H.v);
            H.k = __float_as_int(L.tri[3 * hk + 2].w);
        }
        H.occ &= R.smask;
        phase_a_finish(P, A, R, rcp3(R.d), H, lane);
        wave_sync();
    }
}

hipError_t launch_trace_2a_coop(const KParams& P, const uint32_t* list, const uint32_t* count, uint32_t* zero,
                                uint32_t blocks, hipStream_t st) {
    return with_const<1, kMaxLights>(P.n_lights <= 1 ? 1 : kMaxLights, [&](auto nl) {
        constexpr int NL = decltype(nl)::value;
        const size_t lds = (size_t)P.n_stri * 3 * sizeof(f4) + (kBlock / 64) * sizeof(MergedWave<NL>);
        hipLaunchKernelGGL((k_trace_2a_coop<NL>), dim3(blocks), dim3(kBlock), lds, st, P, *P.sstep, list, count, zero);
        return hipGetLastError();
    });
}
#endif




#if XRT_PHASE_CLOCK && !defined(XRT_STEP_MOM_UNIT)
constexpr uint32_t kWaveClockCap = 1u << 20;
struct WaveClockRec {
    uint32_t tag, block;
    unsigned long long wall0, shader0, wall1, shader1;
};
__device__ WaveClockRec g_wave_clock[kWaveClockCap];
__device__ unsigned int g_wave_clock_n;
struct WaveClock {
    uint32_t idx = kWaveClockCap;
    __device__ explicit WaveClock(uint32_t tag) {
        if ((threadIdx.x & 63u) == 0u) {
            idx = atomicAdd(&g_wave_clock_n, 1u);
            if (idx < kWaveClockCap) {
                g_wave_clock[idx].tag = tag, g_wave_clock[idx].block = blockIdx.x;
                g_wave_clock[idx].wall0 = wall_clock64(), g_wave_clock[idx].shader0 = clock64();
            }
        }
    }
    __device__ void end() {
        if (idx < kWaveClockCap) g_wave_clock[idx].wall1 = wall_clock64(), g_wave_clock[idx].shader1 = clock64();
    }
};
hipError_t wave_clock_dump(const char* path, hipStream_t st) {
    unsigned int n = 0, zero = 0;
    int khz = 0, dev = 0;
    hipError_t e = hipStreamSynchronize(st);
    if (e == hipSuccess) e = hipMemcpyFromSymbol(&n, HIP_SYMBOL(g_wave_clock_n), sizeof(n));
    if (e == hipSuccess) e = hipMemcpyToSymbol(HIP_SYMBOL(g_wave_clock_n), &zero, sizeof(zero));
    if (e == hipSuccess) e = hipGetDevice(&dev);
    if (e == hipSuccess) e = hipDeviceGetAttribute(&khz, hipDeviceAttributeWallClockRate, dev);
    if (e != hipSuccess || !path) return e;
    n = std::min(n, kWaveClockCap);
    std::vector<WaveClockRec> rec(n);
    if (n) e = hipMemcpyFromSymbol(rec.data(), HIP_SYMBOL(g_wave_clock), (size_t)n * sizeof(WaveClockRec));
    if (e != hipSuccess) return e;
    if (FILE* f = std::fopen(path, "wb")) {
        const uint32_t head[2] = {n, (uint32_t)khz};
        std::fwrite(head, sizeof(head), 1, f);
        std::fwrite(rec.data(), sizeof(WaveClockRec), n, f);
        std::fclose(f);
    }
    return hipSuccess;
}
#else
struct WaveClock {
    __device__ explicit WaveClock(uint32_t) {}
    __device__ void end() {}
};
#endif

template <int INTEG, int NL, int SPW, int G, bool LANE, bool BVH, bool GROUPED, bool MOM = false>
__device__ __forceinline__ void step_merged_body(
    const KParams* __restrict__ Pp, const StepObjs SO,
    const uint32_t* __restrict__ list,
    const uint32_t* __restrict__ count, uint32_t* __restrict__ out, uint32_t* out_count, uint32_t* zero_count,
    std::conditional_t<MOM, float2*, uint32_t*> req_count, uint32_t visits, uint32_t grp) {
    constexpr int NW = 6 + 2 * NL;
    static_assert(!GROUPED || (SPW == 64 && G == 1 && !LANE && !BVH), "groups: whole waves of one-level scenes");
    WaveClock wclk(GROUPED ? grp : ~0u);
    static_assert(!BVH || (G == 1 && !LANE), "two-level scenes trace by pair passes");
    const KParams& P = *Pp;
    extern __shared__ __attribute__((aligned(16))) f4 lds_m[];
    char* lb = reinterpret_cast<char*>(lds_m);
    const int tid = threadIdx.x, lane = tid & 63;
    LScene L;
    const DObjPlane* lplane = nullptr;
    MergedWave<NL>* Wp;
    const f4* top = nullptr;
    uint16_t* stk = nullptr;
    int ntop = 0;
    f4 root[4];
    if constexpr (BVH) {
        const BvhStepLayout Bl = bvh_step_layout(P, (uint32_t)sizeof(MergedWave<NL>));
        L.tri = reinterpret_cast<const f4*>(lb + Bl.tri);
        L.obj = reinterpret_cast<const DObj*>(lb + Bl.obj);
        L.light = reinterpret_cast<const DLight*>(lb + Bl.light);
        top = reinterpret_cast<const f4*>(lb + Bl.top);
        ntop = Bl.ntop;
        Wp = reinterpret_cast<MergedWave<NL>*>(lb + Bl.wave);
        stk = reinterpret_cast<uint16_t*>(lb + Bl.stack + (tid >> 6) * kStackWave);
        lds_copy(const_cast<f4*>(L.tri), P.stri, 3 * P.n_stri, tid);
        lds_copy(const_cast<DObj*>(L.obj), P.objs, P.n_objs, tid);
        lds_copy(const_cast<DLight*>(L.light), P.lights, P.n_lights, tid);
        lds_copy(const_cast<f4*>(top), P.bvh4, 8 * ntop, tid);
        root[0] = ldg4(P.bvh_node, 0), root[1] = ldg4(P.bvh_node, 1), root[2] = ldg4(P.bvh_node, 2);
        root[3] = ldg4(P.bvh_node, 3);
    } else {
        const StepLayout Lo = step_layout(P);
        L.tri = reinterpret_cast<const f4*>(lb + Lo.tri);
        L.tng = reinterpret_cast<const f4*>(lb + Lo.tng);
        L.nrm = reinterpret_cast<const f4*>(lb + Lo.nrm);
        L.box = reinterpret_cast<const DObjBox*>(lb + Lo.box);
        L.sph = reinterpret_cast<const f4*>(lb + Lo.sph);
        L.bx = reinterpret_cast<const f4*>(lb + Lo.bx);
        L.obj = reinterpret_cast<const DObj*>(lb + Lo.obj);
        L.light = reinterpret_cast<const DLight*>(lb + Lo.light);
        L.sobj = reinterpret_cast<const int*>(lb + Lo.sobj);
        lplane = reinterpret_cast<const DObjPlane*>(lb + merged_plane_off(Lo));
        Wp = reinterpret_cast<MergedWave<NL>*>(lb + merged_wave_off(P, Lo));
        lds_copy(const_cast<f4*>(L.tri), P.tri, 3 * P.n_tris, tid);
        lds_copy(const_cast<f4*>(L.tng), P.tri_ng, P.n_tris, tid);
        lds_copy(const_cast<f4*>(L.nrm), P.tri_nrm, 3 * P.n_tris, tid);
        lds_copy(const_cast<DObj*>(L.obj), P.objs, P.n_objs, tid);
        lds_copy(const_cast<DLight*>(L.light), P.lights, P.n_lights, tid);
        if (LANE) {
            lds_copy(const_cast<DObjBox*>(L.box), P.obj_box, P.n_objs, tid);
            lds_copy(const_cast<DObjPlane*>(lplane), P.obj_plane, P.n_objs, tid);
        }
    }
    MergedWave<NL>& W = Wp[tid >> 6];
    static_assert(sizeof(MergedWave<NL>) >= kMT * 4, "the wave's trace scratch doubles as the refill buffer");
    auto tri_rec = [&](int i) -> f4 {
        if constexpr (BVH) return ldg4(P.tri, i);
        else return L.tri[i];
    };
    auto tri_ng_at = [&](int i) -> v3 {
        if constexpr (BVH) return xyz(ldg4(P.tri_ng, i));
        else return xyz(L.tng[i]);
    };
    auto tri_ns_at = [&](int i, float u, float v) -> v3 {
        if constexpr (BVH) {
            const float w = 1.0f - u - v;
            return xyz(ldg4(P.tri_nrm, 3 * (size_t)i)) * w + xyz(ldg4(P.tri_nrm, 3 * (size_t)i + 1)) * u +
                   xyz(ldg4(P.tri_nrm, 3 * (size_t)i + 2)) * v;
        } else {
            return tri_ns_l(L, i, u, v);
        }
    };
    __syncthreads();
    if constexpr (GROUPED) zero_parts(zero_count, grp);
    else zero_parts(P, zero_count);
    const PartIter it = GROUPED ? part_iter(count, (kBlock / 64) * SPW, grp) : part_iter(P, count, (kBlock / 64) * SPW);
    const uint32_t spp = P.spp, max_depth = P.max_depth, width = P.width;
    for (uint32_t base = it.first; base < it.n; base += it.stride) {
        const uint32_t i = base + (uint32_t)(tid >> 6) * SPW + (uint32_t)lane / G;
        const bool own = lane / G < SPW && i < it.n;
        const bool lead = own && (lane % G) == 0;
        const uint32_t s = own ? list[it.p * P.part_cap + i] : 0;
        uint32_t st = own ? glb<gu32>(P.state)[s] : ST_DONE;
        st &= ~ST_RNGREQ;
        const bool live = !(st & ST_DONE);
        uint32_t g = 0, depth = 0, k = 0, kst = 0;
        RngRegs<NW> rng;
        rng.c = 0;
        const uint32_t* ring = P.ring + (size_t)s * kRing;
        v3 thr = mk(1, 1, 1), rad = mk(0, 0, 0), o = mk(0, 0, 0), d = mk(0, 0, 0), acc = mk(0, 0, 0);
        v3 rad_fin = mk(0, 0, 0), thr_nee = mk(0, 0, 0);
        v3 so[NL + 1], sd[NL + 1], c1[NL + 1], c0[NL + 1];
        constexpr bool kFold = INTEG == XRT_INTEGRATOR_GI && NL == 1;
        constexpr bool kCover = XRT_CAM_COVER && INTEG == XRT_INTEGRATOR_GI && !BVH;
        uint32_t c0z = 0;
        float stm[NL + 1];
#pragma unroll
        for (int l = 0; l <= NL; ++l) so[l] = sd[l] = c1[l] = c0[l] = mk(0, 0, 0), stm[l] = 0.0f;
        uint32_t shm = 0;
        bool ext = false, fin = false;
        float2 msum = make_float2(0.0f, 0.0f);
        const SlotPixel pix = slot_pixel(P, s);
        const uint32_t col = pix.col, row = pix.row;
        float* px = P.fb + 3 * ((size_t)col + (size_t)width * row);
        if (live) {
            g = glb<gu32>(P.rng_g)[s];
            rng.c = glb<gu32>(P.rng_c)[s];
            depth = glb<gu32>(P.depth)[s];
            k = glb<gu32>(P.sample_k)[s];
            kst = k;
            if (!(st & ST_REGEN)) {
                thr = ld3g(P.thr, s), rad = ld3g(P.rad, s);
                o = ld3g(P.ray_o, s), d = ld3g(P.ray_d, s);
                ext = true;
                kst = k + 1;
            }
            gf32* pxg = glb<gf32>(px);
            acc = mk(pxg[0], pxg[1], pxg[2]);
            if constexpr (MOM && XRT_MOM_REGS) msum = req_count[s];
            rng.load(ring);
        }
        uint32_t nseg = 0, nsh = 0, nrej = 0;
        auto finish = [&](v3 r0) {
            const v3 r = r0 / 1.0f;
            if (__builtin_isnan(r.x) || __builtin_isnan(r.y) || __builtin_isnan(r.z) || __builtin_isinf(r.x) ||
                __builtin_isinf(r.y) || __builtin_isinf(r.z) || r.x < 0.0f || r.y < 0.0f || r.z < 0.0f) {
                ++nrej;
            } else {
                acc = acc + r;
                if constexpr (MOM) {
                    const float l = luminance(r);
                    if constexpr (XRT_MOM_REGS) {
                        msum.x = msum.x + l, msum.y = msum.y + l * l;
                    } else if (lead) {
                        float2 m = req_count[s];
                        m.x = m.x + l, m.y = m.y + l * l;
                        req_count[s] = m;
                    }
                }
            }
            ++k;
            if (k >= spp) st = ST_DONE;
        };
        auto start_sample = [&]() {
            const float u = div_w(P, (float)(int)col + rng.next());
            const float v = div_h(P, (float)(int)row + rng.next());
            camera_ray(P, u, v, o, d);
            thr = mk(1, 1, 1), rad = mk(0, 0, 0);
            depth = 0;
            ext = true;
            ++kst;
        };
        auto resolve = [&](uint32_t occ) {
            if (!shm) return;
            v3& tgt = fin ? rad_fin : rad;
            if (INTEG == XRT_INTEGRATOR_DIRECT) {
#pragma unroll
                for (int l = 0; l < NL; ++l)
                    if ((shm >> l) & 1u) tgt = tgt + (((occ >> l) & 1u) ? c0[l] : c1[l]);
            } else if constexpr (kFold) {
                tgt = tgt + ((occ & 1u) ? mk(zdecode(c0z & 3u), zdecode((c0z >> 2) & 3u), zdecode(c0z >> 4)) : c1[0]);
            } else {
                v3 directL = mk(0, 0, 0);
#pragma unroll
                for (int l = 0; l < NL; ++l)
                    if ((shm >> l) & 1u) {
                        const v3 L_light = mk(0, 0, 0) + (((occ >> l) & 1u) ? c0[l] : c1[l]);
                        directL = directL + L_light;
                    }
                tgt = tgt + thr_nee * directL;
            }
            shm = 0;
            if (fin) {
                fin = false;
                finish(rad_fin);
            }
        };
        if (live && !(st & ST_DONE) && g - rng.c >= (uint32_t)NW && (st & ST_REGEN)) {
            st &= ~ST_REGEN;
            start_sample();
        }
        __builtin_amdgcn_s_waitcnt(0);
        bool pf_pending = false;
        for (uint32_t vis = 0; vis < visits; ++vis) {
            const bool act = live && !(st & ST_DONE) && g - rng.c >= (uint32_t)NW;
            if (!__ballot(act || shm)) break;
            const bool ext_now = act && ext;
            const bool ext_tr = ext_now && !(kCover && depth == 0 && (st >> ST_COVER_SHIFT));
            unsigned long long best;
            uint32_t occ;
            if constexpr (BVH) {
                merged_trace<NL, true>(SO, L, W, lane, ext_now, o, d, shm, so, sd, stm, best, occ);
                deep_pass<NL, uint16_t>(P, top, ntop, stk, W, lane, root, ext_now, o, d, shm, so, sd, stm, best, occ);
            } else if constexpr (!LANE) {
                merged_trace<NL>(SO, L, W, lane, ext_tr, o, d, shm, so, sd, stm, best, occ);
            } else {
                group_trace<NL, G>(P.n_objs, L, lplane, lane, ext_tr, o, d, shm, so, sd, stm, best, occ);
            }
            if (kCover && ext_now && depth == 0 && (st >> ST_COVER_SHIFT)) best = (st >> ST_COVER_SHIFT) - 1u;
            resolve(occ);
            if (BVH ? pf_pending : vis > 0) rng.take();
            if (ext_now) {
                ++nseg;
                int hk = -1, obj = -1;
                float ht = kINF, hu = 0.0f, hv = 0.0f;
                if (best != ~0ull) {
                    hk = (int)(uint32_t)best;
                    const f4 ta = tri_rec(3 * hk);
                    (void)ray_tri(o, d, xyz(ta), xyz(tri_rec(3 * hk + 1)), xyz(tri_rec(3 * hk + 2)), ht, hu, hv);
                    obj = __float_as_int(ta.w);
                }
                v3 pos = mk(0, 0, 0), ng = mk(0, 0, 0);
                if (hk >= 0) pos = ray_at(o, d, ht), ng = tri_ng_at(hk);
                bool ended = false, alive = false;
                if (INTEG == XRT_INTEGRATOR_DIRECT) {
                    if (obj < 0) {
                        rad = mk((float)0.18, (float)0.18, (float)0.18);
                        ended = true;
                    } else if (L.obj[obj].light >= 0) {
                        rad = light_Le(L.light[L.obj[obj].light], tri_ns_at(hk, hu, hv), d);
                        ended = true;
                    } else {
                        alive = true;
                    }
                } else {
                    if (obj < 0) {
                        rad = rad + thr * mk(0.0f, 0.0f, 0.0f);
                        ended = true;
                    } else {
                        alive = true;
                        if (depth > 0) {
                            const float pr = smin(div_const(thr.x + thr.y + thr.z, 3.0f, kRcp3), 1.0f);
                            if (rng.next() >= pr) alive = false, ended = true;
                            else thr = thr / mk(pr, pr, pr);
                        }
                        if (alive && L.obj[obj].light >= 0) {
                            if (depth == 0)
                                rad = rad + thr * light_Le(L.light[L.obj[obj].light], tri_ns_at(hk, hu, hv), d);
                            alive = false, ended = true;
                        }
                    }
                }
                if (alive) {
                    const DObj& ob = L.obj[obj];
                    const v3 fr = ob.material == 1 ? mk(ob.fr[0], ob.fr[1], ob.fr[2]) : mk(0, 0, 0);
#pragma unroll
                    for (int l = 0; l < NL; ++l) {
                        v3 wi = mk(0, 0, 0);
                        float tmax = 0.0f, pdf = 0.0f;
                        const v3 Lv = light_sample(L.light[l], pos, wi, pdf, tmax, rng);
                        if (pdf != 0.0f) {
                            ++nsh;
                            shm |= 1u << l;
                            const float bias = 0.01f;
                            so[l] = pos + ng * bias, sd[l] = wi, stm[l] = tmax - bias;
                            const float cosv = smax(0.0f, dot(ng, wi));
                            c1[l] = ((fr * Lv) * cosv) / pdf;
                            const v3 z = ((fr * 0.0f) * Lv) * cosv;
                            c0[l] = pdf == pdf ? z : mk(pdf, pdf, pdf);
                            if constexpr (kFold) {
                                const v3 zero = mk(0, 0, 0);
                                c1[0] = thr * (zero + (zero + c1[0]));
                                const v3 w = thr * (zero + (zero + c0[0]));
                                c0z = zcode(w.x) | (zcode(w.y) << 2) | (zcode(w.z) << 4);
                            }
                        }
                    }
                    if (INTEG == XRT_INTEGRATOR_DIRECT) {
                        ended = true;
                    } else {
                        if (!kFold && shm) thr_nee = thr;
                        else rad = rad + thr * mk(0.0f, 0.0f, 0.0f);
                        v3 nd = mk(0, 0, 0);
                        const bool lamb = ob.material == 1;
                        if (lamb) {
                            v3 dpdu, dpdv;
                            onb(tri_ns_at(hk, hu, hv), dpdu, dpdv);
                            nd = lambert_sample_f(ng, dpdu, dpdv, rng);
                        }
                        const float cosv = smax(0.0f, dot(nd, ng));
                        const v3 fc = fr * cosv;
                        thr = thr * (lamb ? mk(div_const(fc.x, kLambertPdf, kLambertPdfRcp),
                                               div_const(fc.y, kLambertPdf, kLambertPdfRcp),
                                               div_const(fc.z, kLambertPdf, kLambertPdfRcp))
                                          : fc / 1.0f);
                        o = pos + ng * 0.01f;
                        d = nd;
                        ++depth;
                        if (depth >= max_depth) ended = true;
                    }
                }
                if (ended) {
                    ext = false;
                    if (shm) {
                        rad_fin = rad;
                        fin = true;
                    } else {
                        finish(rad);
                    }
                    if (kst < spp) start_sample();
                }
            }
            rng.prefetch(ring);
            pf_pending = true;
        }
        if (__ballot(shm != 0)) {
            unsigned long long best;
            uint32_t occ;
            if constexpr (BVH) {
                merged_trace<NL, true>(SO, L, W, lane, false, o, d, shm, so, sd, stm, best, occ);
                deep_pass<NL, uint16_t>(P, top, ntop, stk, W, lane, root, false, o, d, shm, so, sd, stm, best, occ);
            } else if constexpr (!LANE) {
                merged_trace<NL>(SO, L, W, lane, false, o, d, shm, so, sd, stm, best, occ);
            } else {
                group_trace<NL, G>(P.n_objs, L, lplane, lane, false, o, d, shm, so, sd, stm, best, occ);
            }
            resolve(occ);
        }
        bool want_req = false;
        if (live && lead) {
            px[0] = acc.x, px[1] = acc.y, px[2] = acc.z;
            if constexpr (MOM && XRT_MOM_REGS) req_count[s] = msum;
            want_req = !(st & ST_DONE) && g - rng.c < P.rng_keep;
            P.state[s] = st;
            if (!(st & (ST_DONE | ST_REGEN))) {
                P.depth[s] = depth;
                P.thr[s] = pk(thr);
                P.rad[s] = pk(rad);
                P.ray_o[s] = pk(o);
                P.ray_d[s] = pk(d);
            }
            P.sample_k[s] = k;
            P.rng_c[s] = rng.c;
            if (nseg) P.c_seg[s] += nseg;
            if (nsh) P.c_shadow[s] += nsh;
            if (nrej) P.c_rej[s] += nrej;
        }
        wave_append(live && lead && !(st & ST_DONE), s, out + it.p * P.part_cap, out_count + it.p, lane);
        wave_refill(P, want_req, s, g, lane, reinterpret_cast<uint32_t*>(&W));
    }
    wclk.end();
}

template <int INTEG, int NL, int SPW, int G, bool LANE, bool BVH, int WV = 0, bool MOM = false>
__global__ __launch_bounds__(kBlock, WV ? WV : (BVH ? XRT_BVH_WAVES : XRT_STEP_WAVES)) void k_step_merged(
    const KParams* __restrict__ Pp, const StepObjs SO, const uint32_t* __restrict__ list,
    const uint32_t* __restrict__ count, uint32_t* __restrict__ out, uint32_t* out_count, uint32_t* zero_count,
    std::conditional_t<MOM, float2*, uint32_t*> req_count, uint32_t visits) {
    step_merged_body<INTEG, NL, SPW, G, LANE, BVH, false, MOM>(Pp, SO, list, count, out, out_count, zero_count, req_count, visits, 0u);
}

template <int INTEG, int NL, bool MOM = false>
__global__ __launch_bounds__(kBlock, XRT_STEP_WAVES) void k_step_merged_group(
    const KParams* __restrict__ Pp, const StepObjs SO, const uint32_t* __restrict__ list,
    const uint32_t* __restrict__ count, uint32_t* __restrict__ out, uint32_t* out_count, uint32_t* zero_count,
    std::conditional_t<MOM, float2*, uint32_t*> req_count, uint32_t visits, uint32_t grp) {
    step_merged_body<INTEG, NL, 64, 1, false, false, true, MOM>(Pp, SO, list, count, out, out_count, zero_count, req_count, visits, grp);
}

#ifndef XRT_STEP_MOM_UNIT
template <bool CLEAR>
__global__ __launch_bounds__(kBlock) void k_refill_merged(KParams P, const uint32_t* __restrict__ req,
                                                          const uint32_t* __restrict__ count, uint32_t* zero_count) {
    __shared__ __attribute__((aligned(16))) uint32_t stage[kBlock / 64][2][kMT];
    zero_parts(P, zero_count);
    const PartIter it = part_iter(P, count, kBlock / 64);
    const int lane = threadIdx.x & 63, wv = threadIdx.x >> 6;
    uint32_t i = it.first + wv;
    if (i >= it.n) return;
    const uint32_t* rq = req + it.p * P.part_cap;
    uint32_t s = rq[i];
    uint32_t g = glb<gu32>(P.rng_g)[s];
    store_block(load_block(P.ring + (size_t)s * kRing, g, lane), lane, stage[wv][0]);
    for (int buf = 0;; buf ^= 1) {
        const uint32_t in = i + it.stride;
        const bool more = in < it.n;
        uint32_t sn = s, gn = g;
        Staged nx;
        if (more) {
            sn = rq[in];
            gn = glb<gu32>(P.rng_g)[sn];
            nx = load_block(P.ring + (size_t)sn * kRing, gn, lane);
        }
        twist_block(P.ring + (size_t)s * kRing, g, lane, stage[wv][buf]);
        if (lane == 0) {
            P.rng_g[s] = g + kMT;
            if (CLEAR) P.state[s] &= ~ST_RNGREQ;
        }
        if (!more) break;
        store_block(nx, lane, stage[wv][buf ^ 1]);
        s = sn, g = gn, i = in;
    }
}

hipError_t launch_refill_merged(const KParams& P, const uint32_t* count, uint32_t* zero_count, hipStream_t st) {
    const uint32_t per = std::max<uint32_t>(1u, std::min<uint32_t>((P.part_cap + 3) / 4, 16384u / P.n_part));
    hipLaunchKernelGGL(k_refill_merged<false>, dim3(P.n_part * per), dim3(kBlock), 0, st, P, P.req, count,
                       zero_count);
    return hipGetLastError();
}

hipError_t launch_refill(const KParams& P, const uint32_t* count, uint32_t* zero_count, hipStream_t st) {
    const uint32_t per = std::max<uint32_t>(1u, std::min<uint32_t>((P.part_cap + 3) / 4, 16384u / P.n_part));
    hipLaunchKernelGGL(k_refill_merged<true>, dim3(P.n_part * per), dim3(kBlock), 0, st, P, P.req, count, zero_count);
    return hipGetLastError();
}

bool use_step_merged(const KParams& P) {
    return P.scene_kind == SCN_TRI && P.small_tri && P.det_bounded && P.n_objs <= kMergedMaxObjs && P.n_lights <= kMaxLights &&
           (P.integrator == XRT_INTEGRATOR_DIRECT || (P.integrator == XRT_INTEGRATOR_GI && P.max_depth > 0)) &&
           !exp_env("XRT_NO_MERGED") && step_merged_lds_bytes(P) <= kStepLds;
}

bool use_step_bvh(const KParams& P) {
    return P.scene_kind == SCN_TRI && P.two_level && P.sstep && P.det_bounded && P.bvh4 && P.bvh_node &&
           P.bvh4_nodes <= 0x10000 && P.bvh4_stack > 0 && P.bvh4_stack <= kBvh4Stack && P.n_lights >= 1 &&
           P.n_lights <= 2 &&
           (P.integrator == XRT_INTEGRATOR_DIRECT || (P.integrator == XRT_INTEGRATOR_GI && P.max_depth > 0)) &&
           !exp_env("XRT_NO_STEP_BVH") && step_merged_lds_bytes(P) <= kStepLds;
}

uint32_t step_merged_draws(const KParams& P) { return 6u + 2u * (uint32_t)P.n_lights; }

static size_t merged_wave_bytes(int n_lights) {
    return with_const<0, 1, 2, 3, 4>(n_lights, [](auto nl) { return sizeof(MergedWave<decltype(nl)::value>); });
}

size_t step_merged_lds_bytes(const KParams& P) {
    const size_t w = merged_wave_bytes(P.n_lights);
    if (P.two_level) return bvh_step_layout(P, (uint32_t)w).total;
    return merged_wave_off(P, step_layout(P)) + (kBlock / 64) * w;
}
#endif

template <bool MOM, int INTEG, int SPW, int G, bool LANE, bool BVH = false, int WV = 0>
static void launch_merged_i(const KParams& P, const KParams* dP, const StepObjs& SO, const uint32_t* list,
                            const uint32_t* count, uint32_t* out, uint32_t* out_count, uint32_t* zero,
                            std::conditional_t<MOM, float2*, uint32_t*> req_count, uint32_t visits, uint32_t part_live, size_t lds, uint32_t grp,
                            hipStream_t st) {
    const uint32_t per_block = (kBlock / 64) * SPW;
    const uint32_t blocks = (grp >> 8) * ((std::min(part_live, P.part_cap) + per_block - 1) / per_block);
    auto go = [&](auto nl) {
        constexpr int NL = decltype(nl)::value;
        if constexpr (SPW == 64 && G == 1 && !LANE && !BVH) {
            if (((grp >> 4) & 15u) > 1u) {
                hipLaunchKernelGGL((k_step_merged_group<INTEG, NL, MOM>), dim3(blocks), dim3(kBlock), lds, st, dP, SO, list, count,
                                   out, out_count, zero, req_count, visits, grp);
                return;
            }
        }
        hipLaunchKernelGGL((k_step_merged<INTEG, NL, SPW, G, LANE, BVH, WV, MOM>), dim3(blocks), dim3(kBlock), lds, st, dP, SO,
                           list, count, out, out_count, zero, req_count, visits);
    };
    if constexpr (BVH) with_const<1, 2>(P.n_lights, go);
    else with_const<0, 1, 2, 3, 4>(P.n_lights, go);
}

#ifndef XRT_STEP_MOM_UNIT
uint32_t step_merged_spw(const KParams& P, uint64_t live) {
    const bool group = P.n_tris <= 64 && !(P.rflags & XRT_FLAG_NO_GROUP);
    if (P.spw_req == 4) return group ? 4u : 16u;
    if (P.spw_req == 8) return group ? 8u : 16u;
    if (P.spw_req == 16 || P.spw_req == 32 || P.spw_req == 64) return P.spw_req;
    if (P.two_level) return live >= kBvhLive64 ? 64u : live >= kBvhLive32 ? 32u : 16u;
    if (live >= kMergedLive64) return 64;
    if (live >= kMergedLive32) return 32;
    if (!group) return 16u;
    if (live < kMergedLive16) return 4u;
    return live < XRT_LIVE8 ? 8u : 16u;
}

uint32_t step_merged_group(const KParams& P, uint32_t spw) {
    const bool group = P.n_tris <= 64 && !(P.rflags & XRT_FLAG_NO_GROUP);
    return spw < 64 && group ? 64u / spw : 1u;
}
#endif

template <bool MOM, int INTEG>
static void launch_merged_spw(const KParams& P, const KParams* dP, const StepObjs& SO, const uint32_t* list,
                              const uint32_t* count, uint32_t* out, uint32_t* out_count, uint32_t* zero,
                              std::conditional_t<MOM, float2*, uint32_t*> req_count, uint32_t visits, uint64_t live, uint32_t part_live, size_t lds,
                              uint32_t grp, hipStream_t st) {
    const bool group = P.n_tris <= 64 && !(P.rflags & XRT_FLAG_NO_GROUP);
    const bool lane64 = group && exp_env("XRT_LANE_TRACE");
    (void)lane64;
    if (P.two_level) {
#define XRT_BVH_CASE(SPWV) \
    launch_merged_i<MOM, INTEG, SPWV, 1, false, true>(P, dP, *P.sstep, list, count, out, out_count, zero, req_count, visits, \
                                                 part_live, lds, grp, st)
        switch (step_merged_spw(P, live)) {
            case 64: XRT_BVH_CASE(64); break;
            case 32: XRT_BVH_CASE(32); break;
            default:
                if (live < XRT_BVH_LOW_LIVE)
                    launch_merged_i<MOM, INTEG, 16, 1, false, true, XRT_BVH_LOW_WAVES>(
                        P, dP, *P.sstep, list, count, out, out_count, zero, req_count, visits, part_live, lds, grp, st);
                else
                    XRT_BVH_CASE(16);
                break;
        }
#undef XRT_BVH_CASE
        return;
    }
#define XRT_MERGED_CASE(SPWV, GV, LV) \
    launch_merged_i<MOM, INTEG, SPWV, GV, LV>(P, dP, SO, list, count, out, out_count, zero, req_count, visits, part_live, lds, grp, st)
    switch (step_merged_spw(P, live)) {
        case 64:
            if constexpr (!MOM) {
                if (lane64) {
                    XRT_MERGED_CASE(64, 1, true);
                    break;
                }
            }
// ... 37 lines not shown
```

xraytracer_amd/csrc/tuning.h:

```cpp
#pragma once

#ifndef XRT_MAX_PARTS
#define XRT_MAX_PARTS 1024
#endif
#ifndef XRT_PART_MIN
#define XRT_PART_MIN 512
#endif

#ifndef XRT_LIVE32
#define XRT_LIVE32 90000
#endif
#ifndef XRT_LIVE8
#define XRT_LIVE8 0
#endif
#ifndef XRT_LIVE16
#define XRT_LIVE16 20000
#endif
#ifndef XRT_MOM_REGS
#define XRT_MOM_REGS 1
#endif
#ifndef XRT_TRACE_TLIM
#define XRT_TRACE_TLIM 1
#endif
#ifndef XRT_TRACE_CLASSES
#define XRT_TRACE_CLASSES 1
#endif
#ifndef XRT_STEP_WAVES
#define XRT_STEP_WAVES 4
#endif
#ifndef XRT_STEP_GROUPS
#define XRT_STEP_GROUPS 2
#endif
#ifndef XRT_SLOT_INTERLEAVE
#define XRT_SLOT_INTERLEAVE 1
#endif
#ifndef XRT_SLOT_INTERLEAVE_MIN
#define XRT_SLOT_INTERLEAVE_MIN 60000
#endif
#ifndef XRT_KSTEP_LDS_REFILL
#define XRT_KSTEP_LDS_REFILL 2
#endif
#ifndef XRT_KSTEP_512
#define XRT_KSTEP_512 0
#endif
#ifndef XRT_KSTEP_WAVES
#define XRT_KSTEP_WAVES XRT_STEP_WAVES
#endif

#ifndef XRT_PIX_BLOCK
#define XRT_PIX_BLOCK 512
#endif
#ifndef XRT_PIX_STRIDE4
#define XRT_PIX_STRIDE4 1
#endif
#ifndef XRT_PIX_GLOBAL_BVH
#define XRT_PIX_GLOBAL_BVH 1
#endif
#ifndef XRT_PIX_DEFER_BLOCK
#define XRT_PIX_DEFER_BLOCK 1024
#endif
#ifndef XRT_PIX_WAVES
#define XRT_PIX_WAVES 4
#endif
#ifndef XRT_PIX_FRUSTUM_MAX
#define XRT_PIX_FRUSTUM_MAX 8192
#endif
#ifndef XRT_PIX_DEFER
#define XRT_PIX_DEFER 1
#endif
#ifndef XRT_PIX_SHADOW_LIST
#define XRT_PIX_SHADOW_LIST 1
#endif
#ifndef XRT_PIX_BLOCKS
#define XRT_PIX_BLOCKS 1
#endif
#ifndef XRT_PIX_PACKET
#define XRT_PIX_PACKET 1
#endif

#ifndef XRT_BVH_WAVES
#define XRT_BVH_WAVES 4
#endif
#ifndef XRT_BVH_LIVE64
#define XRT_BVH_LIVE64 750000
#endif
#ifndef XRT_BVH_LIVE32
#define XRT_BVH_LIVE32 250000
#endif
#ifndef XRT_BVH_LEAF
#define XRT_BVH_LEAF 4
#endif
#ifndef XRT_BVH_LOW_LIVE
#define XRT_BVH_LOW_LIVE 0
#endif
#ifndef XRT_BVH_LOW_WAVES
#define XRT_BVH_LOW_WAVES 3
#endif
#ifndef XRT_BVH_TOP
#define XRT_BVH_TOP 64
#endif
#ifndef XRT_DEEP_LEAF_BATCH
#define XRT_DEEP_LEAF_BATCH 1
#endif
#ifndef XRT_DEEP_SPREAD
#define XRT_DEEP_SPREAD 1
#endif

#ifndef XRT_SHADE_WAVES
#define XRT_SHADE_WAVES 1
#endif
#ifndef XRT_DEEP_WAVES
#define XRT_DEEP_WAVES 1
#endif
#ifndef XRT_2A_WAVES
#define XRT_2A_WAVES 1
#endif

#ifndef XRT_SPEC_TWIST
#define XRT_SPEC_TWIST 1
#endif
#ifndef XRT_SPEC_VISITS
#define XRT_SPEC_VISITS 80
#endif
#ifndef XRT_SPEC_TAIL
#define XRT_SPEC_TAIL 1
#endif
#ifndef XRT_CAM_ELIDE
#define XRT_CAM_ELIDE 1
#endif
#ifndef XRT_CAM_COVER
#define XRT_CAM_COVER 1
#endif

#ifndef XRT_PHASE_CLOCK
#define XRT_PHASE_CLOCK 0
#endif

#ifndef XRT_VPT_EVENTS
#define XRT_VPT_EVENTS 1
#endif
#ifndef XRT_VPT_EV_VISITS
#define XRT_VPT_EV_VISITS 128
#endif
#ifndef XRT_VPT_EV_DRAWS
#define XRT_VPT_EV_DRAWS 4
#endif
#ifndef XRT_VPT_LOW_LIVE
#define XRT_VPT_LOW_LIVE 131072
#endif
#ifndef XRT_VPT_EV_PF
#define XRT_VPT_EV_PF 4
#endif
#ifndef XRT_CORNER_GRID
#define XRT_CORNER_GRID 1
#endif
```

xraytracer_amd/renderer.py:

```python
from __future__ import annotations

import ctypes as C

import numpy as np

from . import abi
from .scenes import SceneBundle


class HipRenderer:
    def __init__(self, spp: int, device: int = 0, devices=None):
        self.spp = int(spp)
        self._lib = abi.lib()
        ctx = C.c_void_p()
        if devices is not None:
            devs = (C.c_int * len(devices))(*[int(d) for d in devices])
            rc = self._lib.xrt_create_multi(devs, len(devices), C.byref(ctx))
            what = f"xrt_create_multi(devices={list(devices)})"
        else:
            rc = self._lib.xrt_create(int(device), C.byref(ctx))
            what = f"xrt_create(device={device})"
        if rc != 0:
            raise abi.XrtError(f"{what} failed ({rc}): {self._lib.xrt_last_error(None).decode()}")
        self.ctx = ctx
        self.stats = None
        self._uploaded = None

    def close(self):
        ctx, self.ctx = getattr(self, "ctx", None), None
        if ctx:
            self._lib.xrt_destroy(ctx)

    __del__ = close

    def _check(self, rc, what):
        if rc != 0:
            raise abi.XrtError(f"{what} failed ({rc}): {self._lib.xrt_last_error(self.ctx).decode()}")

    def upload(self, scene: SceneBundle):
        self._check(self._lib.xrt_upload_scene(self.ctx, C.byref(scene.desc)), "xrt_upload_scene")
        cam = scene.camera
        self._check(self._lib.xrt_set_camera(self.ctx, abi.fptr(cam.c2w), C.c_float(cam.scale),
                                             C.c_float(cam.aspect)), "xrt_set_camera")
        dl, ndl = scene.delta_lights()
        self._check(self._lib.xrt_set_delta_lights(self.ctx, dl, ndl), "xrt_set_delta_lights")
        if scene.medium is not None:
            md = scene.medium.desc()
            if getattr(scene.medium, "sparse", False):
                table, bricks = scene.medium.bricks()
                self._bricks = (table, bricks)
                nbz, nby, nbx = table.shape
                bg = abi.XrtBrickGrid(nbx, nby, nbz, table.ctypes.data_as(C.POINTER(C.c_int32)), len(bricks),
                                      abi.fptr(bricks.reshape(-1)))
                self._check(self._lib.xrt_set_medium_bricks(self.ctx, C.byref(md), C.byref(bg)),
                            "xrt_set_medium_bricks")
            else:
                self._check(self._lib.xrt_set_medium(self.ctx, C.byref(md)), "xrt_set_medium")
        self._uploaded = scene

    def params(self, scene, width, height, shard_index=0, shard_count=1, timing=False, integrator=None,
               max_depth=None, schedule="auto", slots_per_wave=0, visits_per_launch=0, group=True,
               accumulate=False, deep="auto", spec=True, whitted_bvh=False, overlap=True, interleave=None,
               fused_var=False):
        if schedule not in ("auto", "step", "wavefront", "step_tri"):
            raise ValueError(f"unknown schedule {schedule!r}")
        if deep not in ("auto", "single", "quad"):
            raise ValueError(f"unknown deep walk {deep!r}")
        p = abi.XrtRenderParams()
        p.integrator = abi.INTEGRATORS[integrator or scene.integrator]
        p.max_depth = scene.max_depth if max_depth is None else max_depth
        p.width, p.height, p.spp = width, height, self.spp
        p.shard_index, p.shard_count = shard_index, shard_count
        p.flags = ((abi.XRT_FLAG_TIMING if timing else 0) | (abi.XRT_FLAG_WAVEFRONT if schedule == "wavefront" else 0) |
                   (abi.XRT_FLAG_NO_MERGED if schedule == "step_tri" else 0) | (0 if group else abi.XRT_FLAG_NO_GROUP) |
                   (abi.XRT_FLAG_NO_PIXEL if schedule in ("step", "step_tri") else 0) |
                   (abi.XRT_FLAG_ACCUMULATE if accumulate else 0) | (0 if spec else abi.XRT_FLAG_NO_SPEC) |
                   (abi.XRT_FLAG_WHITTED_BVH if whitted_bvh else 0) | (0 if overlap else abi.XRT_FLAG_NO_OVERLAP) |
                   (0 if interleave is None else abi.XRT_FLAG_INTERLEAVE if interleave else abi.XRT_FLAG_NO_INTERLEAVE) |
                   (abi.XRT_FLAG_VAR_FUSED if fused_var else 0) |
                   {"auto": 0, "single": abi.XRT_FLAG_DEEP_SINGLE, "quad": abi.XRT_FLAG_DEEP_QUAD}[deep])
        p.slots_per_wave, p.visits_per_launch = slots_per_wave, visits_per_launch
        return p

    def render(self, scene: SceneBundle, width: int, height: int, initial=None, **kw) -> np.ndarray:
        if self._uploaded is not scene:
            self.upload(scene)
        p = self.params(scene, width, height, accumulate=initial is not None, **kw)
        img = np.zeros((height, width, 3), np.float32)
        if initial is not None:
            img[...] = initial
        st = abi.XrtStats()
        self._check(self._lib.xrt_render(self.ctx, C.byref(p), abi.fptr(img), C.byref(st)), "xrt_render")
        self.stats = st
        return img

    def render_var(self, scene: SceneBundle, width: int, height: int, **kw):
        if self._uploaded is not scene:
            self.upload(scene)
        p = self.params(scene, width, height, **kw)
        img = np.zeros((height, width, 3), np.float32)
        var = np.zeros((height, width), np.float32)
        st = abi.XrtStats()
        self._check(self._lib.xrt_render_var(self.ctx, C.byref(p), abi.fptr(img), abi.fptr(var), C.byref(st)),
                    "xrt_render_var")
        self.stats = st
        return img, var

    def render_var_device(self, scene: SceneBundle, width: int, height: int, out_ptr: int, var_ptr: int,
                          after_stream=None, **kw):
        if self._uploaded is not scene:
            self.upload(scene)
        p = self.params(scene, width, height, **kw)
        st = abi.XrtStats()
        self._check(self._lib.xrt_render_var_device(self.ctx, C.byref(p), C.c_void_p(out_ptr or None),
                                                    C.c_void_p(var_ptr or None), C.c_void_p(after_stream or None),
                                                    C.byref(st)), "xrt_render_var_device")
        self.stats = st
        return st

    _AOV_SHAPES = {"albedo": (3,), "normal": (3,), "depth": (), "alpha": (), "object": ()}

    def render_aov(self, scene: SceneBundle, width: int, height: int,
                   planes=("albedo", "normal", "depth", "alpha", "object"), **kw) -> dict:
        planes = tuple(planes)
        bad = [n for n in planes if n not in self._AOV_SHAPES]
        if bad:
            raise ValueError(f"unknown guide planes {bad}")
        if self._uploaded is not scene:
            self.upload(scene)
        p = self.params(scene, width, height, **kw)
        out = {n: np.zeros((height, width) + self._AOV_SHAPES[n], np.int32 if n == "object" else np.float32)
               for n in planes}
        bufs = abi.XrtAovBuffers(**{n: a.ctypes.data for n, a in out.items()})
        st = abi.XrtStats()
        self._check(self._lib.xrt_render_aov(self.ctx, C.byref(p), C.byref(bufs), C.byref(st)), "xrt_render_aov")
        self.stats = st
        return out

    def render_aov_device(self, scene: SceneBundle, width: int, height: int, ptrs: dict, after_stream=None, **kw):
        bad = [n for n in ptrs if n not in self._AOV_SHAPES]
        if bad:
            raise ValueError(f"unknown guide planes {bad}")
        if self._uploaded is not scene:
            self.upload(scene)
        p = self.params(scene, width, height, **kw)
        bufs = abi.XrtAovBuffers(**{n: int(v) for n, v in ptrs.items() if v})
        st = abi.XrtStats()
        self._check(self._lib.xrt_render_aov_device(self.ctx, C.byref(p), C.byref(bufs), C.c_void_p(after_stream or None),
                                                    C.byref(st)), "xrt_render_aov_device")
        self.stats = st
        return st

    def _filter_inputs(self, color, guides, width, height):
        bad = [n for n in guides if n not in self._AOV_SHAPES]
        if bad:
            raise ValueError(f"unknown guide planes {bad}")
        if color is not None:
            assert color.dtype == np.float32 and color.flags.c_contiguous and color.ndim == 3 and color.shape[2] == 3
            height, width = color.shape[:2]
        for n in abi.DENOISE_PLANES:
            a = guides.get(n)
            if a is not None:
                assert a.dtype == (np.int32 if n == "object" else np.float32) and a.flags.c_contiguous
                assert a.shape == (height, width) + self._AOV_SHAPES[n], n
        return width, height, abi.XrtAovBuffers(**{n: guides[n].ctypes.data for n in abi.DENOISE_PLANES
                                                   if guides.get(n) is not None})

    def _filter_inputs_device(self, guide_ptrs):
        bad = [n for n in guide_ptrs if n not in self._AOV_SHAPES]
        if bad:
            raise ValueError(f"unknown guide planes {bad}")
        return abi.XrtAovBuffers(**{n: int(guide_ptrs[n]) for n in abi.DENOISE_PLANES if guide_ptrs.get(n)})

    @staticmethod
    def _denoise_params(width, height, iterations, sigma_color, sigma_normal, sigma_depth, sigma_albedo, tile, timing):
        return abi.XrtDenoiseParams(width, height, iterations, sigma_color, sigma_normal, sigma_depth, sigma_albedo,
                                    (abi.XRT_DENOISE_TIMING if timing else 0) | (0 if tile else abi.XRT_DENOISE_NO_TILE))

    def denoise(self, color, guides: dict, iterations=3, sigma_color=2.0, sigma_normal=0.5, sigma_depth=0.0,
                sigma_albedo=0.2, tile=True, timing=False, out=None, width=None, height=None) -> np.ndarray:
        width, height, bufs = self._filter_inputs(color, guides, width, height)
        if out is None:
            out = np.empty((height, width, 3), np.float32)
        assert out.dtype == np.float32 and out.flags.c_contiguous and out.shape == (height, width, 3)
        p = self._denoise_params(width, height, iterations, sigma_color, sigma_normal, sigma_depth, sigma_albedo, tile, timing)
        st = abi.XrtDenoiseStats()
        self._check(self._lib.xrt_denoise(self.ctx, C.byref(p), C.c_void_p(color.ctypes.data if color is not None else None),
                                          C.byref(bufs), C.c_void_p(out.ctypes.data), C.byref(st)), "xrt_denoise")
        self.denoise_stats = st
        return out

    def denoise_device(self, color_ptr, guide_ptrs: dict, out_ptr, width, height, after_stream=None, iterations=3,
                       sigma_color=2.0, sigma_normal=0.5, sigma_depth=0.0, sigma_albedo=0.2, tile=True, timing=False):
        bufs = self._filter_inputs_device(guide_ptrs)
        p = self._denoise_params(width, height, iterations, sigma_color, sigma_normal, sigma_depth, sigma_albedo, tile, timing)
        st = abi.XrtDenoiseStats()
        self._check(self._lib.xrt_denoise_device(self.ctx, C.byref(p), C.c_void_p(color_ptr or None), C.byref(bufs),
                                                 C.c_void_p(out_ptr or None), C.c_void_p(after_stream or None),
                                                 C.byref(st)), "xrt_denoise_device")
        self.denoise_stats = st
        return st

    @staticmethod
    def _denoise_var_params(width, height, iterations, sigma_luminance, sigma_normal, sigma_depth, sigma_albedo,
                            variance_radius, tile, timing):
        return abi.XrtDenoiseVarParams(width, height, iterations, sigma_luminance, sigma_normal, sigma_depth, sigma_albedo,
                                       variance_radius,
                                       (abi.XRT_DENOISE_TIMING if timing else 0) | (0 if tile else abi.XRT_DENOISE_NO_TILE))

    def denoise_var(self, color, guides: dict, variance=None, iterations=4, sigma_luminance=4.0, sigma_normal=0.5,
                    sigma_depth=0.0, sigma_albedo=0.2, variance_radius=3, tile=True, timing=False, out=None,
                    out_variance=None, want_variance=True, width=None, height=None):
        width, height, bufs = self._filter_inputs(color, guides, width, height)
        if variance is not None:
            assert variance.dtype == np.float32 and variance.flags.c_contiguous and variance.shape == (height, width)
        if out is None:
            out = np.empty((height, width, 3), np.float32)
        assert out.dtype == np.float32 and out.flags.c_contiguous and out.shape == (height, width, 3)
        if out_variance is None and want_variance:
            out_variance = np.empty((height, width), np.float32)
        if out_variance is not None:
            assert out_variance.dtype == np.float32 and out_variance.flags.c_contiguous and out_variance.shape == (height, width)
        p = self._denoise_var_params(width, height, iterations, sigma_luminance, sigma_normal, sigma_depth, sigma_albedo,
                                     variance_radius, tile, timing)
        st = abi.XrtDenoiseStats()
        self._check(self._lib.xrt_denoise_var(
            self.ctx, C.byref(p), C.c_void_p(color.ctypes.data if color is not None else None),
            C.c_void_p(variance.ctypes.data if variance is not None else None), C.byref(bufs), C.c_void_p(out.ctypes.data),
            C.c_void_p(out_variance.ctypes.data if out_variance is not None else None), C.byref(st)), "xrt_denoise_var")
        self.denoise_stats = st
        return out, out_variance

    def denoise_var_device(self, color_ptr, guide_ptrs: dict, out_ptr, width, height, variance_ptr=0, out_variance_ptr=0,
                           after_stream=None, iterations=4, sigma_luminance=4.0, sigma_normal=0.5, sigma_depth=0.0,
                           sigma_albedo=0.2, variance_radius=3, tile=True, timing=False):
        bufs = self._filter_inputs_device(guide_ptrs)
        p = self._denoise_var_params(width, height, iterations, sigma_luminance, sigma_normal, sigma_depth, sigma_albedo,
                                     variance_radius, tile, timing)
        st = abi.XrtDenoiseStats()
        self._check(self._lib.xrt_denoise_var_device(
            self.ctx, C.byref(p), C.c_void_p(color_ptr or None), C.c_void_p(variance_ptr or None), C.byref(bufs),
            C.c_void_p(out_ptr or None), C.c_void_p(out_variance_ptr or None), C.c_void_p(after_stream or None), C.byref(st)),
            "xrt_denoise_var_device")
        self.denoise_stats = st
        return st

    def query(self, scene: SceneBundle, rays: np.ndarray, tmax=None, occluded: bool = False):
        if self._uploaded is not scene:
            self.upload(scene)
        r = np.ascontiguousarray(rays, dtype=np.float32).reshape(-1, 6)
        n = len(r)
        out = (abi.XrtHit * max(1, n))()
        tm = None if tmax is None else np.ascontiguousarray(np.broadcast_to(np.asarray(tmax, np.float32), (n,)))
        self._check(self._lib.xrt_query(self.ctx, n, abi.fptr(r), abi.fptr(tm) if tm is not None else None,
                                        abi.XRT_QUERY_OCCLUDED if occluded else abi.XRT_QUERY_INTERSECT, out),
                    "xrt_query")
        return out[:n]

    def camlist(self, scene: SceneBundle, width: int, height: int, shard_index: int = 0, shard_count: int = 1):
        if self._uploaded is not scene:
            self.upload(scene)
        p = self.params(scene, width, height, shard_index=shard_index, shard_count=shard_count)
        out = np.zeros((len(range(shard_index, height, shard_count)) * width, 4), np.uint32)
        self._check(self._lib.xrt_test_camlist(self.ctx, C.byref(p), abi.u32ptr(out)), "xrt_test_camlist")
        return out

    def slot_map(self, scene: SceneBundle, width: int, height: int, **kw) -> np.ndarray:
        if self._uploaded is not scene:
            self.upload(scene)
        p = self.params(scene, width, height, **kw)
        out = np.zeros(len(range(p.shard_index, height, p.shard_count)) * width, np.uint32)
        self._check(self._lib.xrt_test_slot_map(self.ctx, C.byref(p), abi.u32ptr(out)), "xrt_test_slot_map")
        return out

    def tonemap(self, width: int, height: int, gamma: float, device_ptr: int = 0) -> np.ndarray:
        out = np.empty((height, width, 3), np.uint8)
        self._check(self._lib.xrt_tonemap(self.ctx, C.c_void_p(device_ptr or None), width * height, C.c_float(gamma),
                                          out.ctypes.data_as(C.POINTER(C.c_uint8))), "xrt_tonemap")
        return out

    @staticmethod
    def write_ppm(path: str, rgb8: np.ndarray):
        h, w, _ = rgb8.shape
        with open(path, "w") as f:
            f.write(f"P3\n{w} {h}\n255\n")
            f.write("".join(f"{r} {g} {b}\n" for r, g, b in rgb8.reshape(-1, 3).tolist()))

    def render_device(self, scene: SceneBundle, width: int, height: int, out_ptr: int, after_stream=None, **kw):
        if self._uploaded is not scene:
            self.upload(scene)
        p = self.params(scene, width, height, **kw)
        st = abi.XrtStats()
        if after_stream is None:
            rc = self._lib.xrt_render_device(self.ctx, C.byref(p), C.c_void_p(out_ptr), C.byref(st))
        else:
            rc = self._lib.xrt_render_device_after(self.ctx, C.byref(p), C.c_void_p(out_ptr),
                                                   C.c_void_p(after_stream or None), C.byref(st))
        self._check(rc, "xrt_render_device")
        self.stats = st
        return st
```

Baseline: 10790.

## Add chunked persistent step phase for early merged-step iterations

Adds a chunk-based scheduling phase that compacts live paths into fixed-size chunks per partition class. It then runs a persistent merged-step kernel that handles several passes per launch over those chunks, and scatters survivors back into the per-partition live lists once the live count falls below a threshold. The aim is to cut per-iteration launch, poll and list-compaction overhead while many paths are still alive. In exchange it adds a synchronous host readback during setup, new build and scatter kernels, and extra device memory. It is gated by heuristics on integrator mode, interleave and spp, plus env/flag overrides and a test probe entry point.

New measurement: 11420, median of 6. 1.06x the previous value.

```diff
diff --git a/include/xrt.h b/include/xrt.h
--- a/include/xrt.h
+++ b/include/xrt.h
@@ -113,6 +113,8 @@
     XRT_FLAG_INTERLEAVE = 2048u,
     XRT_FLAG_NO_INTERLEAVE = 4096u,
     XRT_FLAG_VAR_FUSED = 8192u,
+    XRT_FLAG_CHUNKS = 16384u,
+    XRT_FLAG_NO_CHUNKS = 32768u,
     XRT_FLAG_ACCUMULATE = 16u
 };
 
@@ -303,6 +305,7 @@
 int xrt_test_whitted_math(xrt_ctx* ctx, const float* in, uint32_t n, float* out);
 int xrt_test_camlist(xrt_ctx* ctx, const xrt_render_params* p, uint32_t* out);
 int xrt_test_slot_map(xrt_ctx* ctx, const xrt_render_params* p, uint32_t* out);
+int xrt_test_chunk_plan(xrt_ctx* ctx, const xrt_render_params* p, uint32_t plan[5], uint32_t* sizes, uint32_t n_sizes);
 
 #ifdef __cplusplus
 }
diff --git a/xraytracer_amd/abi.py b/xraytracer_amd/abi.py
--- a/xraytracer_amd/abi.py
+++ b/xraytracer_amd/abi.py
@@ -32,6 +32,7 @@
 XRT_FLAG_WHITTED_BVH = 512
 XRT_FLAG_NO_OVERLAP = 1024
 XRT_FLAG_INTERLEAVE, XRT_FLAG_NO_INTERLEAVE = 2048, 4096
+XRT_FLAG_CHUNKS, XRT_FLAG_NO_CHUNKS = 16384, 32768
 XRT_FLAG_VAR_FUSED = 8192
 XRT_SCHED_WAVEFRONT, XRT_SCHED_STEP, XRT_SCHED_STEP_TRI, XRT_SCHED_STEP_MERGED, XRT_SCHED_STEP_BVH = 0, 1, 2, 3, 4
 XRT_SCHED_PIXEL, XRT_SCHED_WHITTED, XRT_SCHED_WHITTED_BVH = 5, 6, 7
@@ -221,6 +222,7 @@
     "xrt_test_fastdiv": (C.c_int, [C.c_void_p, C.c_uint32, C.c_float, C.c_float, C.POINTER(C.c_uint64), u32p]),
     "xrt_test_camlist": (C.c_int, [C.c_void_p, C.POINTER(XrtRenderParams), u32p]),
     "xrt_test_slot_map": (C.c_int, [C.c_void_p, C.POINTER(XrtRenderParams), u32p]),
+    "xrt_test_chunk_plan": (C.c_int, [C.c_void_p, C.POINTER(XrtRenderParams), u32p, u32p, C.c_uint32]),
 }
 
 _lib = None
diff --git a/xraytracer_amd/csrc/api_context.cpp b/xraytracer_amd/csrc/api_context.cpp
--- a/xraytracer_amd/csrc/api_context.cpp
+++ b/xraytracer_amd/csrc/api_context.cpp
@@ -111,7 +111,7 @@
     free_buf(c->q_rays), free_buf(c->q_tmax), free_buf(c->q_out);
     free_buf(c->brick_table), free_buf(c->brick_data), free_buf(c->corners), free_buf(c->camlist);
     free_buf(c->dlights), free_buf(c->obj_albedo), free_buf(c->aov), free_buf(c->denoise);
-    free_buf(c->mom), free_buf(c->var);
+    free_buf(c->mom), free_buf(c->var), free_buf(c->chunks);
     for (hipEvent_t e : c->events) (void)hipEventDestroy(e);
     for (auto& slot : c->poll_ev)
         for (hipEvent_t e : slot)
diff --git a/xraytracer_amd/csrc/api_render.cpp b/xraytracer_amd/csrc/api_render.cpp
--- a/xraytracer_amd/csrc/api_render.cpp
+++ b/xraytracer_amd/csrc/api_render.cpp
@@ -199,6 +199,8 @@
     uint32_t step_visits, spec_visits, rng_keep;
     uint64_t poll_every, ahead;
     uint64_t cap_iters;
+    uint32_t chunk_passes, chunk_class_cap;
+    bool chunk_forced;
     float2* mom;
 };
 
@@ -249,6 +251,22 @@
                     : R.merged                      ? std::min<uint32_t>(kMergedVisits, (kMT - draws) / draws)
                     : (R.volumetric && kVptEvents) ? kVptEventVisits
                                                     : kStepVisits;
+    {
+        ChunkRule cr{};
+        cr.one_level_merged = R.merged && !R.two_level && !R.pixel && !R.whitted && !R.mom && !exp_env("XRT_LANE_TRACE") &&
+                              R.step_visits >= 1 && R.step_visits <= 255;
+        cr.starts_whole_waves = cr.one_level_merged && step_merged_spw(P, n) == 64;
+        cr.interleaved = can_interleave && auto_interleave && R.slot_mul != 0;
+        cr.force = (p->flags & XRT_FLAG_CHUNKS) != 0, cr.forbid = (p->flags & XRT_FLAG_NO_CHUNKS) != 0;
+        cr.visits_req = ev ? 1u : p->visits_per_launch, cr.spw_req = p->slots_per_wave;
+        cr.spp = p->spp, cr.max_depth = p->max_depth, cr.visits = R.step_visits;
+        cr.class_cap = chunk_class_cap(R.n_part, R.part_cap);
+        const char* eq = exp_env("XRT_CHUNK_Q");
+        cr.pass_cap = eq ? (uint32_t)std::min(255, std::max(1, std::atoi(eq))) : XRT_CHUNK_PASSES;
+        R.chunk_passes = chunk_plan(cr);
+        R.chunk_class_cap = cr.class_cap;
+        R.chunk_forced = cr.force;
+    }
     R.spec_visits = !R.spec          ? 0
                     : XRT_SPEC_TWIST ? ((ev || p->visits_per_launch) ? R.step_visits : XRT_SPEC_VISITS)
                                      : std::min<uint32_t>(R.step_visits, (kMT - kSpecDraws) / kSpecDraws);
@@ -272,7 +290,8 @@
     uint64_t live_hint;
     uint32_t live_part_max;
     bool done = false;
-    struct Pending { uint64_t it; int slot; uint32_t groups; };
+    uint64_t retired = 0;
+    struct Pending { uint64_t it; int slot; uint32_t groups; bool parts; };
     std::vector<Pending> pending;
     int issued = 0;
 
@@ -285,7 +304,7 @@
                                          hipMemcpyDeviceToHost, st));
                 HIPCHK(c, hipEventRecord(c->poll_ev[ps][g], st));
             }
-            pending.push_back({it, ps, groups});
+            pending.push_back({it, ps, groups, part_max});
         }
         while (!pending.empty()) {
             const Pending q = pending.front();
@@ -302,10 +321,11 @@
                 const uint32_t v = h0[step_group_of(q.groups, k) * kMaxParts + k];
                 alive += v, pmax = std::max(pmax, v);
             }
+            ++retired;
             if (alive == 0) done = true;
             if (alive < live_hint) {
                 live_hint = alive;
-                if (part_max) live_part_max = std::max(1u, pmax);
+                if (part_max && q.parts) live_part_max = std::max(1u, pmax);
             }
             pending.erase(pending.begin());
             if (done) break;
@@ -373,13 +393,62 @@
     bool forked_ = false;
 };
 
-int run_fused(xrt_ctx* c, const KParams& P, const RenderPlan& R, const LiveLists& L, LaunchTimer& T, LivePoll& poll,
-              uint64_t& it) {
+int build_chunks(xrt_ctx* c, const KParams& P, const RenderPlan& R, const LiveLists& L, LaunchTimer& T, ChunkBufs& B) {
+    const size_t chunks = 8u * (size_t)R.chunk_class_cap, head = kChunkHdrWords + kMaxParts + 2 * chunks;
+    const int rc = ensure(c, c->chunks, (head + 2 * chunks * kChunkSlots) * sizeof(uint32_t));
+    if (rc) return rc;
+    B.hdr = as<uint32_t>(c->chunks), B.part_live = B.hdr + kChunkHdrWords, B.cnt = B.part_live + kMaxParts;
+    B.seg = B.hdr + head, B.class_cap = R.chunk_class_cap;
+    HIPCHK(c, hipMemsetAsync(B.hdr, 0, head * sizeof(uint32_t), c->stream));
+    HIPCHK(c, T.launch(XRT_K_SEED, [&] { return launch_chunks_build(P, B, L.list[0], L.counts(0), c->stream); }));
+    uint32_t head_words[kChunkHdrWords];
+    HIPCHK(c, hipStreamSynchronize(c->stream));
+    HIPCHK(c, hipMemcpy(head_words, B.hdr, sizeof(head_words), hipMemcpyDeviceToHost));
+    uint32_t max_nx = 0;
+    B.chunks = 0;
+    for (uint32_t x = 0; x < 8; ++x) B.chunks += head_words[x], max_nx = std::max(max_nx, head_words[x]);
+    B.blocks = 8u * chunk_class_blocks(max_nx);
+    if (!R.chunk_forced && max_nx > kChunkClassBlocks) B.blocks = 0;
+    return XRT_OK;
+}
+
+int run_chunks(xrt_ctx* c, const KParams& P, const RenderPlan& R, const LiveLists& L, const ChunkBufs& B, LaunchTimer& T,
+               LivePoll& poll, uint64_t& it) {
+    const KParams* dP = as<KParams>(c->kparams);
+    const bool part_max = poll.part_max;
+    const uint64_t ahead = poll.ahead;
+    poll.part_max = false, poll.ahead = 1;
+    int rc = XRT_OK;
+    for (it = 0; it < R.cap_iters && !poll.done; ++it) {
+        if (poll.retired && poll.live_hint < kMergedLive64) break;
+        T.step_live.push_back(poll.live_hint);
+        T.S.layout_launches[0]++;
+        const hipError_t e = T.launch(XRT_K_STEP, [&] {
+            return launch_step_merged_chunks(P, dP, c->step_objs, B, L.counts((it + 1) % 3), L.counts((it + 2) % 3),
+                                             R.step_visits, R.chunk_passes, (uint32_t)it, c->stream);
+        });
+        if (e != hipSuccess) return hip_err(c, e, "k_step_merged_chunks");
+        if ((rc = poll.after(it, L.counts((it + 1) % 3)))) break;
+    }
+    poll.part_max = part_max, poll.ahead = ahead;
+    if (rc || poll.done) return rc;
+    HIPCHK(c, hipMemsetAsync(L.counts(it % 3), 0, P.n_part * sizeof(uint32_t), c->stream));
+    HIPCHK(c, T.launch(XRT_K_SEED, [&] { return launch_chunks_scatter(P, B, L.list[it & 1], L.counts(it % 3), c->stream); }));
+    return XRT_OK;
+}
+
+int run_fused(xrt_ctx* c, const KParams& P, const RenderPlan& R, const LiveLists& L, const ChunkBufs& B, LaunchTimer& T,
+              LivePoll& poll, uint64_t& it) {
     const KParams* dP = as<KParams>(c->kparams);
     const uint32_t blocks = P.n_part * ((P.part_cap + 255) / 256);
     bool camlist_pending = R.camlist && !R.elide;
     StepGroupStreams GS(c, T, R.groups);
-    for (it = 0; it < R.cap_iters && !poll.done; ++it) {
+    it = 0;
+    if (R.chunk_passes && B.blocks) {
+        const int rc = run_chunks(c, P, R, L, B, T, poll, it);
+        if (rc) return rc;
+    }
+    for (; it < R.cap_iters && !poll.done; ++it) {
         const uint32_t *list = L.list[it & 1], *ci = L.counts(it % 3);
         uint32_t *out = L.list[~it & 1], *co = L.counts((it + 1) % 3), *cz = L.counts((it + 2) % 3);
         const uint32_t spw = R.merged ? step_merged_spw(P, poll.live_hint) : 0;
@@ -474,7 +543,7 @@
 }
 
 int render_impl(xrt_ctx* c, const xrt_render_params* p, float* d_out, float* h_out, xrt_stats* st, int wait,
-                hipStream_t wait_stream, float* d_var) {
+                hipStream_t wait_stream, float* d_var, ChunkProbe* probe) {
     const auto t_start = std::chrono::steady_clock::now();
     int rc = check_render(c, p);
     if (rc) return rc;
@@ -511,6 +580,10 @@
     }
     const RenderPlan R = plan_render(P, p, d_var ? as<float2>(c->mom) : nullptr);
     if (!R.pixel && R.rng_keep > kMT) return set_err(c, XRT_ERR_INVALID, "visits_per_launch too large for the RNG ring");
+    if (probe) {
+        probe->passes = R.chunk_passes;
+        if (!R.chunk_passes) return XRT_OK;
+    }
     P.n_part = R.n_part, P.part_cap = R.part_cap, P.rng_keep = R.rng_keep, P.slot_mul = R.slot_mul;
     const size_t lcap = (size_t)P.n_part * P.part_cap;
     const LiveLists L{{as<uint32_t>(c->lists), as<uint32_t>(c->lists) + lcap}, as<uint32_t>(c->counts)};
@@ -533,10 +606,20 @@
     HIPCHK(c, hipMemsetAsync(P.stats, 0, 512, c->stream));
     if (R.mom && R.fused && !R.pixel) HIPCHK(c, hipMemsetAsync(R.mom, 0, n * sizeof(float2), c->stream));
     if ((rc = seed_paths(c, P, R, L, T))) return rc;
+    ChunkBufs CB{};
+    if (R.chunk_passes && (rc = build_chunks(c, P, R, L, T, CB))) return rc;
+    if (probe) {
+        const uint32_t cap = 8u * CB.class_cap;
+        std::vector<uint32_t> cnt(2 * (size_t)cap);
+        HIPCHK(c, hipMemcpy(cnt.data(), CB.cnt, cnt.size() * 4, hipMemcpyDeviceToHost));
+        probe->chunks = CB.chunks, probe->blocks = CB.blocks, probe->cap = cap;
+        for (uint32_t q = 0; q < cap && q < probe->n_sizes; ++q) probe->sizes[q] = cnt[2 * q] + cnt[2 * q + 1];
+        return XRT_OK;
+    }
 
     LivePoll poll{c, P.n_part, R.poll_every, R.ahead, R.merged && !P.spw_req, n, P.part_cap};
     uint64_t it = 0;
-    if (!R.pixel && (rc = R.fused ? run_fused(c, P, R, L, T, poll, it) : run_wavefront(c, P, R, L, T, poll, it)))
+    if (!R.pixel && (rc = R.fused ? run_fused(c, P, R, L, CB, T, poll, it) : run_wavefront(c, P, R, L, T, poll, it)))
         return rc;
     HIPCHK(c, T.launch(XRT_K_FINISH, [&] {
         const hipError_t e = launch_finish(P, c->stream);
@@ -613,6 +696,20 @@
     return e == hipSuccess ? XRT_OK : hip_err(c, e, "xrt_test_slot_map");
 }
 
+int xrt_test_chunk_plan(xrt_ctx* c, const xrt_render_params* p, uint32_t plan[5], uint32_t* sizes, uint32_t n_sizes) {
+    c = first_device(c);
+    if (!c || !p || !plan || (!sizes && n_sizes)) return XRT_ERR_INVALID;
+    ChunkProbe probe{0, 0, 0, 0, sizes, n_sizes};
+    std::memset(plan, 0, 5 * sizeof(uint32_t));
+    if ((size_t)shard_rows(p->height, p->shard_index, p->shard_count) * p->width == 0) return check_render(c, p);
+    xrt_render_params q = *p;
+    q.flags &= ~(uint32_t)XRT_FLAG_ACCUMULATE;
+    const int rc = render_impl(c, &q, nullptr, nullptr, nullptr, 0, nullptr, nullptr, &probe);
+    if (rc) return rc;
+    plan[0] = probe.passes != 0 && probe.blocks != 0, plan[1] = probe.passes, plan[2] = probe.chunks, plan[3] = probe.blocks, plan[4] = probe.cap;
+    return XRT_OK;
+}
+
 static int render_var(xrt_ctx* c, const xrt_render_params* p, float* d_out, float* h_out, float* d_var, float* h_var,
                       xrt_stats* st, int wait, hipStream_t wait_stream) {
     if (!c || !p || !(d_out || h_out) || !(d_var || h_var)) return set_err(c, XRT_ERR_INVALID, "xrt_render_var: null argument");
diff --git a/xraytracer_amd/csrc/ctx.h b/xraytracer_amd/csrc/ctx.h
--- a/xraytracer_amd/csrc/ctx.h
+++ b/xraytracer_amd/csrc/ctx.h
@@ -38,6 +38,7 @@
     xrt::DevBuf state, sample_k, depth, occ, rng_c, rng_g, ring, c_seg, c_shadow, c_rej, c_stall, lists, deep, camlist;
     xrt::DevBuf counts, stats, fb, scratch, kparams;
     xrt::DevBuf mom, var;
+    xrt::DevBuf chunks;
     uint32_t* h_poll = nullptr;
     std::vector<hipEvent_t> events;
     hipEvent_t poll_ev[8][xrt::kMaxStepGroups] = {};
@@ -138,8 +139,13 @@
 int setup_deep(xrt_ctx* c, KParams& P);
 int grow_slots(xrt_ctx* c, size_t n);
 KParams render_params(xrt_ctx* c, const xrt_render_params* p, size_t n, float* fb);
+struct ChunkProbe {
+    uint32_t passes, chunks, blocks, cap;
+    uint32_t* sizes;
+    uint32_t n_sizes;
+};
 int render_impl(xrt_ctx* c, const xrt_render_params* p, float* d_out, float* h_out, xrt_stats* st, int wait = 0,
-                hipStream_t wait_stream = nullptr, float* d_var = nullptr);
+                hipStream_t wait_stream = nullptr, float* d_var = nullptr, ChunkProbe* probe = nullptr);
 
 inline xrt_ctx* first_device(xrt_ctx* c) { return c && !c->subs.empty() ? c->subs[0] : c; }
 
diff --git a/xraytracer_amd/csrc/host/step_chunks.cpp b/xraytracer_amd/csrc/host/step_chunks.cpp
--- /dev/null
+++ b/xraytracer_amd/csrc/host/step_chunks.cpp
@@ -0,0 +1,31 @@
+#include "../step_chunks.h"
+
+namespace xrt {
+
+uint32_t chunk_class_cap(uint32_t n_part, uint32_t part_cap) {
+    const uint32_t per_class = (n_part + 7u) / 8u;
+    return (uint32_t)(((uint64_t)per_class * part_cap + kChunkSlots - 1u) / kChunkSlots);
+}
+
+uint32_t chunk_blocks(uint32_t C) {
+    const uint32_t most = 8u * kChunkClassBlocks;
+    const uint32_t nb = (C < most ? C : most) + 7u;
+    return nb & ~7u;
+}
+
+uint32_t chunk_passes(uint32_t cap, uint32_t spp, uint32_t max_depth, uint32_t visits) {
+    if (visits == 0u) return 0u;
+    const uint64_t quarter = (uint64_t)spp * ((uint64_t)max_depth + 2u) / (2ull * visits * 4ull);
+    return (uint32_t)(quarter < cap ? quarter : cap);
+}
+
+uint32_t chunk_plan(const ChunkRule& r) {
+    if (r.forbid || !r.one_level_merged || !r.starts_whole_waves) return 0u;
+    if (r.class_cap > kChunkOwnMax * kChunkClassBlocks) return 0u;
+    if (r.force) return r.pass_cap >= 1u ? r.pass_cap : 1u;
+    if (!r.interleaved || r.visits_req || r.spw_req) return 0u;
+    const uint32_t Q = chunk_passes(r.pass_cap, r.spp, r.max_depth, r.visits);
+    return Q >= 2u && Q == r.pass_cap ? Q : 0u;
+}
+
+}
diff --git a/xraytracer_amd/csrc/launch.h b/xraytracer_amd/csrc/launch.h
--- a/xraytracer_amd/csrc/launch.h
+++ b/xraytracer_amd/csrc/launch.h
@@ -7,6 +7,7 @@
 #include <type_traits>
 
 #include "slot_map.h"
+#include "step_chunks.h"
 #include "step_groups.h"
 #include "wavefront.h"
 
@@ -86,6 +87,17 @@
                                   const uint32_t* count, uint32_t* out, uint32_t* out_count, uint32_t* zero,
                                   float2* mom, uint32_t visits, uint64_t live, uint32_t live_part_max,
                                   uint32_t groups, uint32_t group, hipStream_t st);
+struct ChunkBufs {
+    uint32_t *hdr, *part_live, *cnt, *seg;
+    uint32_t class_cap;
+    uint32_t chunks, blocks;
+};
+hipError_t launch_chunks_build(const KParams& P, const ChunkBufs& B, const uint32_t* list, const uint32_t* count,
+                               hipStream_t st);
+hipError_t launch_step_merged_chunks(const KParams& P, const KParams* dP, const StepObjs& SO, const ChunkBufs& B,
+                                     uint32_t* live_count, uint32_t* zero, uint32_t visits, uint32_t passes, uint32_t rot,
+                                     hipStream_t st);
+hipError_t launch_chunks_scatter(const KParams& P, const ChunkBufs& B, uint32_t* out, uint32_t* out_count, hipStream_t st);
 #if XRT_PHASE_CLOCK
 hipError_t wave_clock_dump(const char* path, hipStream_t st);
 #endif
diff --git a/xraytracer_amd/csrc/path_common.h b/xraytracer_amd/csrc/path_common.h
--- a/xraytracer_amd/csrc/path_common.h
+++ b/xraytracer_amd/csrc/path_common.h
@@ -3,6 +3,7 @@
 
 #include "device_math.h"
 #include "slot_map.h"
+#include "step_chunks.h"
 #include "step_groups.h"
 #include "wavefront.h"
 #include "xrt.h"
@@ -285,6 +286,82 @@
 __device__ __forceinline__ void zero_parts(uint32_t* c, uint32_t grp) {
     if (blockIdx.x == 0)
         for (uint32_t i = threadIdx.x; i < (grp >> 8); i += kBlock) c[step_group_part((grp >> 4) & 15u, grp & 15u, i)] = 0;
+}
+
+struct ChunkIter {
+    uint32_t *seg, *cnt;
+    uint32_t* tab;
+    uint32_t x, bj, nx, m, rot, T;
+    uint32_t t, left;
+    uint32_t c, h, n;
+};
+__device__ __forceinline__ uint32_t* chunk_table() {
+    __shared__ uint32_t tab[kChunkOwnMax + kBlock / 64];
+    return tab;
+}
+__device__ __forceinline__ uint32_t chunk_uni(uint32_t x) { return (uint32_t)__builtin_amdgcn_readfirstlane((int)x); }
+__device__ __forceinline__ ChunkIter chunk_iter(const uint32_t* hdr, uint32_t* cnt, uint32_t* seg, uint32_t rot,
+                                                uint32_t passes) {
+    ChunkIter K;
+    K.seg = seg, K.cnt = cnt, K.tab = chunk_table();
+    uint32_t max_nx = 0;
+    for (uint32_t x = 0; x < 8u; ++x) max_nx = max(max_nx, hdr[x]);
+    K.x = blockIdx.x & 7u, K.bj = blockIdx.x >> 3;
+    K.nx = chunk_uni(hdr[K.x]);
+    K.m = chunk_uni(min(chunk_class_blocks(max_nx), gridDim.x >> 3));
+    K.rot = rot;
+    K.T = chunk_uni(min(K.nx ? chunk_owned(K.bj, K.nx, K.m) : 0u, kChunkOwnMax));
+    K.t = K.T ? rot % K.T : 0u, K.left = passes, K.c = K.h = K.n = 0;
+    for (uint32_t t = threadIdx.x; t < K.T; t += kBlock) {
+        const uint32_t c = 8u * chunk_owned_at(K.bj, t, K.nx, K.m, rot) + K.x;
+        const uint32_t n0 = cnt[2u * c], n1 = cnt[2u * c + 1u];
+        K.tab[t] = n0 ? n0 : (n1 | 1u << 16);
+    }
+    __syncthreads();
+    return K;
+}
+__device__ __forceinline__ bool chunk_next(ChunkIter& K) {
+    if (K.left == 0u) return false;
+    for (uint32_t k = 0; k < K.T; ++k) {
+        uint32_t t = K.t + k;
+        t = t >= K.T ? t - K.T : t;
+        const uint32_t v = chunk_uni(K.tab[t]);
+        if (v & 0xffffu) {
+            K.c = 8u * chunk_uni(chunk_owned_at(K.bj, t, K.nx, K.m, K.rot)) + K.x;
+            K.h = v >> 16, K.n = v & 0xffffu;
+            K.t = t;
+            --K.left;
+            return true;
+        }
+    }
+    return false;
+}
+__device__ __forceinline__ void chunk_append(ChunkIter& K, bool want, uint32_t v, int lane, int tid) {
+    uint32_t* wcnt = K.tab + kChunkOwnMax;
+    const uint64_t m = __ballot(want);
+    if (lane == 0) wcnt[tid >> 6] = (uint32_t)__popcll(m);
+    __syncthreads();
+    uint32_t before = 0, total = 0;
+#pragma unroll
+    for (int w = 0; w < kBlock / 64; ++w) {
+        const uint32_t q = wcnt[w];
+        before += w < (tid >> 6) ? q : 0u;
+        total += q;
+    }
+    uint32_t* out = K.seg + (size_t)(2u * K.c + (K.h ^ 1u)) * kChunkSlots;
+    if (want) out[before + (uint32_t)__popcll(m & ((1ull << lane) - 1ull))] = v;
+    if (tid == 0) {
+        K.cnt[2u * K.c + K.h] = 0u;
+        K.cnt[2u * K.c + (K.h ^ 1u)] = total;
+        K.tab[K.t] = total | (K.h ^ 1u) << 16;
+    }
+    K.t = K.t + 1u >= K.T ? 0u : K.t + 1u;
+}
+__device__ __forceinline__ void chunk_pass_end() { __syncthreads(); }
+__device__ __forceinline__ uint32_t chunk_live(const ChunkIter& K) {
+    uint32_t sum = 0;
+    for (uint32_t t = 0; t < K.T; ++t) sum += K.tab[t] & 0xffffu;
+    return sum;
 }
 
 
diff --git a/xraytracer_amd/csrc/step_chunks.h b/xraytracer_amd/csrc/step_chunks.h
--- /dev/null
+++ b/xraytracer_amd/csrc/step_chunks.h
@@ -0,0 +1,54 @@
+#pragma once
+#include <stdint.h>
+
+#ifdef __HIPCC__
+#define XRT_CHUNKS_FN __host__ __device__ inline
+#else
+#define XRT_CHUNKS_FN inline
+#endif
+
+namespace xrt {
+
+constexpr uint32_t kChunkSlots = 256;
+constexpr uint32_t kChunkClassBlocks = 128;
+constexpr uint32_t kChunkOwnMax = 32;
+constexpr uint32_t kChunkHdrWords = 16;
+
+XRT_CHUNKS_FN uint32_t chunk_class_count(uint32_t C, uint32_t x) { return (C + 7u - x) / 8u; }
+XRT_CHUNKS_FN uint32_t chunk_class_blocks(uint32_t max_nx) { return max_nx < kChunkClassBlocks ? max_nx : kChunkClassBlocks; }
+XRT_CHUNKS_FN uint32_t chunk_owner(uint32_t j, uint32_t x, uint32_t nx, uint32_t m, uint32_t rot) {
+    return 8u * (((j + rot % nx) % nx) % m) + x;
+}
+XRT_CHUNKS_FN uint32_t chunk_owned(uint32_t bj, uint32_t nx, uint32_t m) { return bj < nx && bj < m ? (nx - bj + m - 1u) / m : 0u; }
+XRT_CHUNKS_FN uint32_t chunk_owned_at(uint32_t bj, uint32_t t, uint32_t nx, uint32_t m, uint32_t rot) {
+    return (bj + t * m + nx - rot % nx) % nx;
+}
+
+XRT_CHUNKS_FN uint32_t chunk_dense_offset(const uint32_t* part_live, uint32_t p) {
+    uint32_t off = 0;
+    for (uint32_t q = p & 7u; q < p; q += 8u) off += part_live[q];
+    return off;
+}
+XRT_CHUNKS_FN uint32_t chunk_class_live(const uint32_t* part_live, uint32_t n_part, uint32_t x) {
+    uint32_t tot = 0;
+    for (uint32_t q = x; q < n_part; q += 8u) tot += part_live[q];
+    return tot;
+}
+XRT_CHUNKS_FN uint32_t chunks_for(uint32_t live) { return (live + kChunkSlots - 1u) / kChunkSlots; }
+
+uint32_t chunk_class_cap(uint32_t n_part, uint32_t part_cap);
+uint32_t chunk_blocks(uint32_t C);
+uint32_t chunk_passes(uint32_t cap, uint32_t spp, uint32_t max_depth, uint32_t visits);
+struct ChunkRule {
+    bool one_level_merged;
+    bool starts_whole_waves;
+    bool interleaved;
+    bool force, forbid;
+    uint32_t visits_req, spw_req;
+    uint32_t spp, max_depth, visits;
+    uint32_t class_cap;
+    uint32_t pass_cap;
+};
+uint32_t chunk_plan(const ChunkRule& r);
+
+}
diff --git a/xraytracer_amd/csrc/step_tri.hip b/xraytracer_amd/csrc/step_tri.hip
--- a/xraytracer_amd/csrc/step_tri.hip
+++ b/xraytracer_amd/csrc/step_tri.hip
@@ -360,7 +360,7 @@
 };
 #endif
 
-template <int INTEG, int NL, int SPW, int G, bool LANE, bool BVH, bool GROUPED, bool MOM = false>
+template <int INTEG, int NL, int SPW, int G, bool LANE, bool BVH, bool GROUPED, bool MOM = false, bool CHUNKS = false>
 __device__ __forceinline__ void step_merged_body(
     const KParams* __restrict__ Pp, const StepObjs SO,
     const uint32_t* __restrict__ list,
@@ -370,6 +370,7 @@
     static_assert(!GROUPED || (SPW == 64 && G == 1 && !LANE && !BVH), "groups: whole waves of one-level scenes");
     WaveClock wclk(GROUPED ? grp : ~0u);
     static_assert(!BVH || (G == 1 && !LANE), "two-level scenes trace by pair passes");
+    static_assert(!CHUNKS || (SPW == 64 && G == 1 && !LANE && !BVH && !GROUPED && !MOM), "chunks: whole waves of one-level scenes");
     const KParams& P = *Pp;
     extern __shared__ __attribute__((aligned(16))) f4 lds_m[];
     char* lb = reinterpret_cast<char*>(lds_m);
@@ -441,13 +442,21 @@
     __syncthreads();
     if constexpr (GROUPED) zero_parts(zero_count, grp);
     else zero_parts(P, zero_count);
-    const PartIter it = GROUPED ? part_iter(count, (kBlock / 64) * SPW, grp) : part_iter(P, count, (kBlock / 64) * SPW);
+    ChunkIter ck;
+    if constexpr (CHUNKS) {
+        ck = chunk_iter(count, req_count, out, grp, visits >> 8);
+        visits &= 255u;
+    }
+    const PartIter it = CHUNKS    ? PartIter{0u, 0u, 0u, 0u}
+                        : GROUPED ? part_iter(count, (kBlock / 64) * SPW, grp)
+                                  : part_iter(P, count, (kBlock / 64) * SPW);
     const uint32_t spp = P.spp, max_depth = P.max_depth, width = P.width;
-    for (uint32_t base = it.first; base < it.n; base += it.stride) {
+    for (uint32_t base = it.first; CHUNKS ? chunk_next(ck) : base < it.n; base += it.stride) {
+        const uint32_t n_in = CHUNKS ? ck.n : it.n;
         const uint32_t i = base + (uint32_t)(tid >> 6) * SPW + (uint32_t)lane / G;
-        const bool own = lane / G < SPW && i < it.n;
+        const bool own = lane / G < SPW && i < n_in;
         const bool lead = own && (lane % G) == 0;
-        const uint32_t s = own ? list[it.p * P.part_cap + i] : 0;
+        const uint32_t s = own ? (CHUNKS ? glb<gu32>(ck.seg + (size_t)(2u * ck.c + ck.h) * kChunkSlots)[i] : list[it.p * P.part_cap + i]) : 0;
         uint32_t st = own ? glb<gu32>(P.state)[s] : ST_DONE;
         st &= ~ST_RNGREQ;
         const bool live = !(st & ST_DONE);
@@ -703,8 +712,16 @@
             if (nsh) P.c_shadow[s] += nsh;
             if (nrej) P.c_rej[s] += nrej;
         }
-        wave_append(live && lead && !(st & ST_DONE), s, out + it.p * P.part_cap, out_count + it.p, lane);
+        if constexpr (CHUNKS) chunk_append(ck, live && lead && !(st & ST_DONE), s, lane, tid);
+        else wave_append(live && lead && !(st & ST_DONE), s, out + it.p * P.part_cap, out_count + it.p, lane);
         wave_refill(P, want_req, s, g, lane, reinterpret_cast<uint32_t*>(&W));
+        if constexpr (CHUNKS) chunk_pass_end();
+    }
+    if constexpr (CHUNKS) {
+        if (tid == 0) {
+            const uint32_t left = chunk_live(ck);
+            if (left) atomicAdd(out_count + blockIdx.x % P.n_part, left);
+        }
     }
     wclk.end();
 }
@@ -726,6 +743,110 @@
 }
 
 #ifndef XRT_STEP_MOM_UNIT
+template <int INTEG, int NL>
+__global__ __launch_bounds__(kBlock, XRT_STEP_WAVES) void k_step_merged_chunks(
+    const KParams* __restrict__ Pp, const StepObjs SO, const uint32_t* __restrict__ hdr, uint32_t* cnt, uint32_t* seg,
+    uint32_t* live_count, uint32_t* zero_count, uint32_t visits, uint32_t passes, uint32_t rot) {
+    step_merged_body<INTEG, NL, 64, 1, false, false, false, false, true>(Pp, SO, nullptr, hdr, seg, live_count, zero_count, cnt,
+                                                                          visits | passes << 8, rot);
+}
+
+__global__ __launch_bounds__(kBlock) void k_chunks_count(KParams P, const uint32_t* __restrict__ list,
+                                                         const uint32_t* __restrict__ count, uint32_t* part_live) {
+    __shared__ uint32_t red[kBlock / 64];
+    const uint32_t p = blockIdx.x, n = min(count[p], P.part_cap);
+    const int lane = threadIdx.x & 63, wv = threadIdx.x >> 6;
+    uint32_t keep = 0;
+    for (uint32_t i = threadIdx.x; i < n; i += kBlock) keep += (P.state[list[(size_t)p * P.part_cap + i]] & ST_DONE) ? 0u : 1u;
+    for (int off = 32; off > 0; off >>= 1) keep += __shfl_down(keep, off);
+    if (lane == 0) red[wv] = keep;
+    __syncthreads();
+    if (threadIdx.x == 0) {
+        uint32_t tot = 0;
+        for (int w = 0; w < kBlock / 64; ++w) tot += red[w];
+        part_live[p] = tot;
+    }
+}
+__global__ __launch_bounds__(kBlock) void k_chunks_build(KParams P, const uint32_t* __restrict__ list,
+                                                         const uint32_t* __restrict__ count,
+                                                         const uint32_t* __restrict__ part_live, uint32_t* hdr, uint32_t* cnt,
+                                                         uint32_t* seg, uint32_t class_cap) {
+    __shared__ uint32_t wc[kBlock / 64];
+    const uint32_t p = blockIdx.x, x = p & 7u, n = min(count[p], P.part_cap);
+    const int tid = threadIdx.x, lane = tid & 63, wv = tid >> 6;
+    uint32_t run = chunk_dense_offset(part_live, p);
+    for (uint32_t base = 0; base < n; base += kBlock) {
+        const uint32_t i = base + (uint32_t)tid;
+        const uint32_t s = i < n ? list[(size_t)p * P.part_cap + i] : 0u;
+        const bool keep = i < n && !(P.state[s] & ST_DONE);
+        const uint64_t m = __ballot(keep);
+        if (lane == 0) wc[wv] = (uint32_t)__popcll(m);
+        __syncthreads();
+        uint32_t before = 0, total = 0;
+        for (int w = 0; w < kBlock / 64; ++w) before += w < wv ? wc[w] : 0u, total += wc[w];
+        const uint32_t pos = run + before + (uint32_t)__popcll(m & ((1ull << lane) - 1ull));
+        const uint32_t j = pos / kChunkSlots;
+        if (keep && j < class_cap) seg[(size_t)(2u * (8u * j + x)) * kChunkSlots + pos % kChunkSlots] = s;
+        run += total;
+        __syncthreads();
+    }
+    if (p < 8u) {
+        const uint32_t tot = chunk_class_live(part_live, P.n_part, x);
+        if (tid == 0) hdr[x] = min(chunks_for(tot), class_cap), hdr[8u + x] = tot;
+        for (uint32_t j = tid; j < class_cap; j += kBlock) {
+            const uint32_t lo = j * kChunkSlots;
+            cnt[2u * (8u * j + x)] = tot > lo ? min(kChunkSlots, tot - lo) : 0u;
+            cnt[2u * (8u * j + x) + 1u] = 0u;
+        }
+    }
+}
+__global__ __launch_bounds__(kBlock) void k_chunks_scatter(KParams P, const uint32_t* __restrict__ cnt,
+                                                           const uint32_t* __restrict__ seg, uint32_t* out, uint32_t* out_count) {
+    const uint32_t c = blockIdx.x, n0 = cnt[2u * c], n1 = cnt[2u * c + 1u];
+    const uint32_t h = n0 ? 0u : 1u, n = min(n0 | n1, kChunkSlots);
+    const int lane = threadIdx.x & 63;
+    const bool have = threadIdx.x < n;
+    const uint32_t s = have ? seg[(size_t)(2u * c + h) * kChunkSlots + threadIdx.x] : 0u;
+    const uint32_t p = min(s / P.part_cap, P.n_part - 1u);
+    uint64_t todo = __ballot(have);
+    while (todo) {
+        const uint32_t pl = (uint32_t)__builtin_amdgcn_readlane((int)p, __builtin_ctzll(todo));
+        const bool mine = have && p == pl;
+        wave_append(mine, s, out + (size_t)pl * P.part_cap, out_count + pl, lane);
+        todo &= ~__ballot(mine);
+    }
+}
+
+hipError_t launch_chunks_build(const KParams& P, const ChunkBufs& B, const uint32_t* list, const uint32_t* count,
+                               hipStream_t st) {
+    hipLaunchKernelGGL(k_chunks_count, dim3(P.n_part), dim3(kBlock), 0, st, P, list, count, B.part_live);
+    hipLaunchKernelGGL(k_chunks_build, dim3(P.n_part), dim3(kBlock), 0, st, P, list, count, B.part_live, B.hdr, B.cnt, B.seg,
+                       B.class_cap);
+    return hipGetLastError();
+}
+
+hipError_t launch_chunks_scatter(const KParams& P, const ChunkBufs& B, uint32_t* out, uint32_t* out_count, hipStream_t st) {
+    hipLaunchKernelGGL(k_chunks_scatter, dim3(8u * B.class_cap), dim3(kBlock), 0, st, P, B.cnt, B.seg, out, out_count);
+    return hipGetLastError();
+}
+
+hipError_t launch_step_merged_chunks(const KParams& P, const KParams* dP, const StepObjs& SO, const ChunkBufs& B,
+                                     uint32_t* live_count, uint32_t* zero, uint32_t visits, uint32_t passes, uint32_t rot,
+                                     hipStream_t st) {
+    if (P.two_level || visits == 0 || visits > 255u || passes == 0 || passes > 255u || B.blocks == 0 ||
+        B.blocks % 8u || B.blocks > 8u * kChunkClassBlocks)
+        return hipErrorInvalidValue;
+    const uint32_t blocks = B.blocks;
+    const size_t lds = step_merged_lds_bytes(P);
+    with_const<XRT_INTEGRATOR_DIRECT, XRT_INTEGRATOR_GI>(P.integrator, [&](auto integ) {
+        with_const<0, 1, 2, 3, 4>(P.n_lights, [&](auto nl) {
+            hipLaunchKernelGGL((k_step_merged_chunks<decltype(integ)::value, decltype(nl)::value>), dim3(blocks), dim3(kBlock),
+                               lds, st, dP, SO, B.hdr, B.cnt, B.seg, live_count, zero, visits, passes, rot);
+        });
+    });
+    return hipGetLastError();
+}
+
 template <bool CLEAR>
 __global__ __launch_bounds__(kBlock) void k_refill_merged(KParams P, const uint32_t* __restrict__ req,
                                                           const uint32_t* __restrict__ count, uint32_t* zero_count) {
diff --git a/xraytracer_amd/csrc/tuning.h b/xraytracer_amd/csrc/tuning.h
--- a/xraytracer_amd/csrc/tuning.h
+++ b/xraytracer_amd/csrc/tuning.h
@@ -30,6 +30,9 @@
 #endif
 #ifndef XRT_STEP_GROUPS
 #define XRT_STEP_GROUPS 2
+#endif
+#ifndef XRT_CHUNK_PASSES
+#define XRT_CHUNK_PASSES 4
 #endif
 #ifndef XRT_SLOT_INTERLEAVE
 #define XRT_SLOT_INTERLEAVE 1
diff --git a/xraytracer_amd/renderer.py b/xraytracer_amd/renderer.py
--- a/xraytracer_amd/renderer.py
+++ b/xraytracer_amd/renderer.py
@@ -61,7 +61,7 @@
     def params(self, scene, width, height, shard_index=0, shard_count=1, timing=False, integrator=None,
                max_depth=None, schedule="auto", slots_per_wave=0, visits_per_launch=0, group=True,
                accumulate=False, deep="auto", spec=True, whitted_bvh=False, overlap=True, interleave=None,
-               fused_var=False):
+               fused_var=False, chunks=None):
         if schedule not in ("auto", "step", "wavefront", "step_tri"):
             raise ValueError(f"unknown schedule {schedule!r}")
         if deep not in ("auto", "single", "quad"):
@@ -78,6 +78,7 @@
                    (abi.XRT_FLAG_WHITTED_BVH if whitted_bvh else 0) | (0 if overlap else abi.XRT_FLAG_NO_OVERLAP) |
                    (0 if interleave is None else abi.XRT_FLAG_INTERLEAVE if interleave else abi.XRT_FLAG_NO_INTERLEAVE) |
                    (abi.XRT_FLAG_VAR_FUSED if fused_var else 0) |
+                   (0 if chunks is None else abi.XRT_FLAG_CHUNKS if chunks else abi.XRT_FLAG_NO_CHUNKS) |
                    {"auto": 0, "single": abi.XRT_FLAG_DEEP_SINGLE, "quad": abi.XRT_FLAG_DEEP_QUAD}[deep])
         p.slots_per_wave, p.visits_per_launch = slots_per_wave, visits_per_launch
         return p
@@ -273,6 +274,18 @@
         self._check(self._lib.xrt_test_slot_map(self.ctx, C.byref(p), abi.u32ptr(out)), "xrt_test_slot_map")
         return out
 
+    def chunk_plan(self, scene: SceneBundle, width: int, height: int, **kw) -> dict:
+        if self._uploaded is not scene:
+            self.upload(scene)
+        p = self.params(scene, width, height, **kw)
+        n = len(range(p.shard_index, height, p.shard_count)) * width
+        sizes = np.zeros(8 * (n // 256 + 2), np.uint32)
+        plan = np.zeros(5, np.uint32)
+        self._check(self._lib.xrt_test_chunk_plan(self.ctx, C.byref(p), abi.u32ptr(plan), abi.u32ptr(sizes), len(sizes)),
+                    "xrt_test_chunk_plan")
+        return dict(chunks=bool(plan[0]), passes=int(plan[1]), C=int(plan[2]), blocks=int(plan[3]),
+                    sizes=sizes[:min(len(sizes), int(plan[4]))].copy())
+
     def tonemap(self, width: int, height: int, gamma: float, device_ptr: int = 0) -> np.ndarray:
         out = np.empty((height, width, 3), np.uint8)
         self._check(self._lib.xrt_tonemap(self.ctx, C.c_void_p(device_ptr or None), width * height, C.c_float(gamma),
```
